# at-cg/PHI

Measured on AMD Instinct MI355X. Metric: read Gbases/s scored (49-hap MHC graph stand-in synMHC-49); reads resident in HBM, parsing and H2D excluded, higher is better.
Workload: dtype u64

## Files before the change

### include/phi_amd.h

```cpp
#ifndef PHI_AMD_H
#define PHI_AMD_H

#include <stddef.h>
#include <stdint.h>

#ifdef __cplusplus
extern "C" {
#endif

typedef struct phi_ctx phi_ctx;

typedef enum {
    PHI_OK = 0,
    PHI_ERR_INVALID = -1,
    PHI_ERR_NOMEM = -2,
    PHI_ERR_DEVICE = -3,
    PHI_ERR_STATE = -4,
    PHI_ERR_UNSUPPORTED = -5,
    PHI_ERR_WALK = -6,
    PHI_ERR_OVERFLOW = -7
} phi_status;

const char *phi_strerror(int status);
const char *phi_last_error(const phi_ctx *ctx);
// ... 44 lines not shown
int phi_panel_stats(phi_ctx *ctx, phi_panel_info *out);
int phi_panel_release(phi_ctx *ctx);
#define PHI_PANEL_KEEP_READS 2u

typedef struct {
    int32_t n_blocks, n_walks;
    int64_t n_classes_flagged;
    int64_t n_nonzero;
    double record_gpu_ms, class_gpu_ms, entry_gpu_ms;
    double walk_sum_gpu_ms;
} phi_scout_info;
int phi_scout_graph(phi_ctx *ctx, int32_t n_vtx, const char *seq_concat, const int64_t *seq_off,
                    const int64_t *adj_off, const int32_t *adj, int32_t n_walks,
                    const int64_t *walk_off, const int32_t *walk_vtx, const int32_t *topo_rank);
int phi_scout_scores(phi_ctx *ctx, int32_t n_blocks, int32_t *scores, phi_scout_info *info);
int phi_scout_choose(phi_ctx *ctx, const uint8_t *always, int32_t n_want, uint8_t *keep, int32_t *round_of);

typedef struct {
    int64_t text_bytes;
    int64_t n_records;
    int32_t n_samples;
    int64_t n_flagged;
    int64_t n_units, n_entries;
    double genotype_gpu_ms, walks_gpu_ms;
} phi_vcf_info;
int phi_vcf_genotypes(phi_ctx *ctx, const char *text, int64_t n_text, const int64_t *text_off, const int32_t *gt_index, int64_t n_records,
                      int32_t n_samples, uint16_t *gt, int32_t *ploidy, uint8_t *flagged);
int phi_vcf_walks(phi_ctx *ctx, const int32_t *unit_first, int64_t n_units, const int32_t *site_backbone, const int32_t *site_allele0,
                  int64_t n_sites, const int32_t *choice, int32_t n_haps, int64_t *walk_off_out);
int phi_vcf_walks_wide(phi_ctx *ctx, const int32_t *unit_first, int64_t n_units, const int32_t *site_backbone, const int32_t *site_allele0,
                       int64_t n_sites, const int32_t *choice, int32_t n_haps, int64_t *walk_off_out);
int phi_vcf_stats(phi_ctx *ctx, phi_vcf_info *out);

int phi_add_reads(phi_ctx *ctx, const char *bases, const int64_t *read_off, int64_t n_reads);
int phi_add_reads_device(phi_ctx *ctx, const void *d_bases, const void *d_read_off, int64_t n_reads,
                         int64_t n_bases);
int phi_reads_text_begin(phi_ctx *ctx, int64_t max_chunk_bytes);
int phi_add_reads_text(phi_ctx *ctx, const char *text, int64_t n_bytes, int32_t *irregular);
int phi_reads_text_end(phi_ctx *ctx, const char **pending, int64_t *n_pending, int64_t *n_taken);
typedef struct phi_text_park phi_text_park;
int phi_text_park_create(int32_t device, phi_text_park **out);
int phi_text_park_pin(phi_text_park *park, void *host, size_t bytes);
int phi_text_park_add(phi_text_park *park, const char *text, int64_t n, int32_t *index);
int phi_text_park_add_async(phi_text_park *park, const char *text, int64_t n, int32_t *index);
int phi_text_park_wait(phi_text_park *park, int32_t index);
int64_t phi_text_park_bytes(phi_text_park *park, int32_t index);
int phi_text_park_fetch(phi_text_park *park, int32_t index, char *out, int64_t cap);
int phi_text_park_release(phi_text_park *park, int32_t index);
void phi_text_park_destroy(phi_text_park *park);
int phi_add_reads_text_parked(phi_ctx *ctx, phi_text_park *park, int32_t index, int32_t *irregular);
int phi_reads_text_last_batch(phi_ctx *ctx, char *bases, int64_t cap_bases, int64_t *off, int64_t cap_reads, int64_t *n_reads,
                              int64_t *n_bases);
int phi_reads_text_detach_carry(phi_ctx *ctx, const char **bytes, int64_t *n);
int phi_reset_reads(phi_ctx *ctx);
int phi_reads_stats(phi_ctx *ctx, int64_t *n_reads, int64_t *n_bases, int64_t *n_emitted, int64_t *n_distinct);

int phi_hits_buffer(phi_ctx *ctx, void **d_hits, int64_t *n);
int phi_read_table(phi_ctx *ctx, void **d_table, int64_t *n_buckets);
int phi_spectrum_export(phi_ctx *ctx, void **d_hashes, int64_t *n);
int phi_spectrum_import(phi_ctx *ctx, const void *d_hashes, int64_t n);
int phi_spectrum_set_size(phi_ctx *ctx, int64_t global_size);

#define PHI_COMM_ID_BYTES 128
int phi_comm_unique_id(void *id_out, size_t cap);
int phi_comm_init(phi_ctx *ctx, const void *id, int32_t rank, int32_t n_ranks);
int phi_comm_info(const phi_ctx *ctx, int32_t *rank, int32_t *n_ranks);
int phi_comm_allreduce_hits(phi_ctx *ctx);
int phi_comm_exchange(phi_ctx *ctx);
int phi_comm_destroy(phi_ctx *ctx);

int phi_peers_create(int32_t n_ranks, void **group);
int phi_peers_join(phi_ctx *ctx, void *group, int32_t rank);
int phi_peers_allreduce_hits(phi_ctx *ctx);
int phi_peers_exchange(phi_ctx *ctx);
int phi_peers_destroy(void *group);

int phi_ipc_unique_id(void *id_out, size_t cap);
int phi_ipc_init(phi_ctx *ctx, const void *id, int32_t rank, int32_t n_ranks);
int phi_ipc_info(const phi_ctx *ctx, int32_t *rank, int32_t *n_ranks);
int phi_ipc_allreduce_hits(phi_ctx *ctx);
int phi_ipc_flush(phi_ctx *ctx);
int phi_ipc_exchange(phi_ctx *ctx);
int phi_ipc_check(phi_ctx *ctx);
int phi_ipc_destroy(phi_ctx *ctx);

typedef struct {
    int64_t objective;
    int64_t upper_bound;
    int32_t optimal;
    int32_t n_dp_runs;
    int64_t n_covered;
    int64_t n_path;
    const int32_t *path_vtx;
    const int32_t *path_hap;
    int32_t recombination_count;
    int32_t n_switches;
    int64_t hap_len;
    int32_t n_walks;
    const int64_t *n_minimizers;
    const int64_t *n_anchors;
    int64_t spectrum_size;
    int64_t filtered;
    int64_t retained;
    int64_t n_in_model;
} phi_result;

int phi_set_solve_budget(phi_ctx *ctx, int64_t max_dp_runs);

int phi_solve(phi_ctx *ctx, phi_result *out);

int phi_path_sequence(phi_ctx *ctx, char *buf, int64_t cap);

int phi_sketch(phi_ctx *ctx, const char *bases, const int64_t *seq_off, int64_t n_seq, int32_t k,
               int32_t w, uint64_t *out_hash, int64_t *out_pos, int32_t *out_seq, int64_t cap,
               int64_t *n_out);
typedef struct {
    int64_t n_entries, walk_bases;
    int64_t n_classes, class_bases, n_class_records;
    int64_t n_walk_minimizers, n_distinct_minimizers;
    double sketch_gpu_ms;
} phi_index_info;
int phi_index_stats(phi_ctx *ctx, phi_index_info *out);

typedef struct {
    int64_t n_dp_anchors, n_events;
    int32_t n_steps, n_blocks, dp_mode, max_classes;
    double mean_classes;
} phi_solve_info;
int phi_solve_stats(phi_ctx *ctx, phi_solve_info *out);

int phi_walk_minimizers(phi_ctx *ctx, int32_t walk, uint64_t *out_hash, int64_t *out_pos,
                        int64_t cap, int64_t *n_out);
int phi_walk_sharing(phi_ctx *ctx, int64_t *hist, int32_t cap, int64_t *n_distinct);

int phi_kept_anchors(phi_ctx *ctx, uint64_t *out_hash, int32_t *out_walk, int32_t *out_t0,
                     int32_t *out_t1, int64_t cap, int64_t *n_out);

int phi_host_register(phi_ctx *ctx, void *p, size_t bytes);
int phi_host_unregister(phi_ctx *ctx, void *p);

int phi_prof_enable(phi_ctx *ctx, int on);
int phi_prof_read(phi_ctx *ctx, int64_t *n_launches, double *total_ms, int64_t *total_bases);

typedef struct { const char *text; int64_t n; } phi_walk_text;
int phi_walk_text_upload(phi_ctx *ctx, const phi_walk_text *walks, int32_t n_walks);
int phi_walk_text_resolve(phi_ctx *ctx, const char *prefix, int32_t prefix_n, const int32_t *num2id, int64_t n_num, int32_t n_seg,
                          int64_t *walk_off_out, uint32_t *irregular);
int phi_walk_entries(phi_ctx *ctx, int32_t *out, int64_t cap, int64_t *n);

int phi_device_synchronize(phi_ctx *ctx);

int phi_prefix_sums(phi_ctx *ctx, int32_t kind, const void *d_in, int64_t n, void *d_out);

int phi_edit_distances(phi_ctx *ctx, const char *a, const int64_t *a_off, const char *b, const int64_t *b_off,
                       int64_t n_pairs, int64_t max_distance, int64_t *out);

int phi_edit_alignments(phi_ctx *ctx, const char *a, const int64_t *a_off, const char *b, const int64_t *b_off,
                        int64_t n_pairs, const int64_t *dist, int64_t *counts, char *cigar, const int64_t *cigar_off);


#define PHI_INFLATE_CHUNK_DEFAULT (64 << 10)
#define PHI_INFLATE_NO_FINDER 1
typedef struct {
    int64_t in_bytes;
    int64_t out_bytes;
    int64_t members;
    int64_t chunks;
    int64_t confirmed;
    int64_t redecoded;
    int64_t marker_bytes;
    double device_ms;
    char detail[192];
} phi_inflate_info;
int phi_inflate(int32_t device, const void *in, int64_t n, void *out, int64_t cap, int64_t chunk_bytes, int32_t flags,
                int64_t *out_size, phi_inflate_info *info);
int phi_inflate_alloc(int32_t device, const void *in, int64_t n, int64_t chunk_bytes, int32_t flags, void **out, int64_t *out_size,
                      phi_inflate_info *info);
void phi_inflate_free(void *p);
int phi_text_park_gzip_begin(phi_text_park *park, int64_t piece_bytes);
int phi_text_park_gzip_add(phi_text_park *park, const void *data, int64_t n);
int phi_text_park_gzip_end(phi_text_park *park, int32_t *first, int32_t *count, phi_inflate_info *info);
int phi_gzip_header(const void *data, int64_t n, int64_t pos, int64_t *deflate_start);
uint32_t phi_crc32_combine(uint32_t crc_a, uint32_t crc_b, int64_t len_b);

typedef struct {
    int64_t text_bytes;
    int64_t host_bytes;
    int64_t walk_bytes;
    int32_t n_walks;
    phi_inflate_info inflate;
} phi_gfa_gzip_info;
int phi_gfa_gzip_split(phi_ctx *ctx, const void *gz, int64_t n, int64_t chunk_bytes, char **host_text, int64_t *host_n,
                       phi_gfa_gzip_info *info);
void phi_gfa_gzip_free(char *host_text);

#define PHI_LADDER_MAX_LEVELS 16
typedef struct {
    int32_t n_levels;
    int32_t one_length;
    int64_t n_reads, n_bases;
    int64_t n_kept_reads, n_kept_bases;
    int64_t band_reads[PHI_LADDER_MAX_LEVELS], band_bases[PHI_LADDER_MAX_LEVELS];
    uint64_t threshold[PHI_LADDER_MAX_LEVELS];
    double count_gpu_ms, scan_gpu_ms, scatter_gpu_ms, copy_gpu_ms;
} phi_ladder_info;
int phi_reads_collect_begin(phi_ctx *ctx, int64_t first_ordinal);
int phi_reads_collect_end(phi_ctx *ctx, int64_t *n_reads, int64_t *n_bases);
int phi_reads_collect_release(phi_ctx *ctx);
int phi_reads_collect_score(phi_ctx *ctx);
int phi_ladder_plan(phi_ctx *ctx, uint64_t seed, const double *fractions, int32_t n_levels, phi_ladder_info *info);
int phi_ladder_advance(phi_ctx *ctx, int32_t level);
int phi_ladder_band(phi_ctx *ctx, int32_t band, int64_t *ordinals_out, int64_t cap, int64_t *n,
                    char *bases_out, int64_t bases_cap, int64_t *offsets_out, int64_t *n_bases);

typedef struct {
    int64_t n_records;
    int64_t n_kept;
    int64_t n_secondary_supplementary;
    int64_t n_empty;
    int64_t n_reverse;
    int64_t n_bases;
    int64_t header_bytes;
    int64_t tiles, tiles_confirmed, tiles_rewalked;
    int64_t batches, batches_without_offsets;
    int32_t n_ref;
    int32_t one_length;
} phi_bam_info;
int phi_reads_bam_begin(phi_ctx *ctx, int64_t max_chunk_bytes, int64_t tile_bytes);
int phi_add_reads_bam(phi_ctx *ctx, const void *bytes, int64_t n);
int phi_add_reads_bam_parked(phi_ctx *ctx, phi_text_park *park, int32_t index);
int phi_reads_bam_end(phi_ctx *ctx, phi_bam_info *info);
int phi_reads_bam_last_batch(phi_ctx *ctx, char *bases, int64_t cap_bases, int64_t *off, int64_t cap_reads, int64_t *n_reads, int64_t *n_bases);

typedef struct {
    int64_t n_calls;
    const int64_t *pos;
    const int64_t *ref_off, *alt_off;
    const char *ref_bytes, *alt_bytes;
    const int32_t *anchor;
    int64_t n_shared, n_query, n_ref;
    int64_t ref_span[2], query_span[2];
    double gpu_ms;
} phi_calls;
typedef struct {
    int64_t n_query, n_ref, n_shared, n_pairs, n_calls;
    int64_t ref_bytes, alt_bytes;
    int64_t ref_bases, query_bases;
    int64_t bytes_moved;
    double table_gpu_ms, shared_gpu_ms, pairs_gpu_ms, fill_gpu_ms, gpu_ms;
} phi_calls_info;
int phi_calls_path(phi_ctx *ctx, int32_t ref_walk, phi_calls *out);
int phi_calls_walk(phi_ctx *ctx, int32_t walk, int32_t ref_walk, phi_calls *out);
int phi_calls_stats(phi_ctx *ctx, phi_calls_info *out);

#ifdef __cplusplus
}
#endif
#endif
```

### phi_amd/_capi.py

```python
import ctypes as C
import os

_HERE = os.path.dirname(os.path.abspath(__file__))
LIB_PATH = os.environ.get("PHI_AMD_LIB") or os.path.join(_HERE, "libphi_amd.so")

PHI_OK = 0
PHI_ERR_INVALID, PHI_ERR_NOMEM, PHI_ERR_DEVICE, PHI_ERR_STATE = -1, -2, -3, -4
PHI_ERR_UNSUPPORTED, PHI_ERR_WALK, PHI_ERR_OVERFLOW = -5, -6, -7
PHI_FLAG_QCLP, PHI_FLAG_MIXED = 1, 2
PHI_COMM_ID_BYTES = 128

SYMBOLS = [
    "phi_strerror", "phi_last_error", "phi_ctx_create", "phi_ctx_destroy", "phi_set_stream", "phi_set_params",
    "phi_set_graph", "phi_add_reads", "phi_add_reads_device", "phi_reset_reads", "phi_reads_stats", "phi_hits_buffer", "phi_read_table",
    "phi_spectrum_export", "phi_spectrum_import", "phi_spectrum_set_size", "phi_solve", "phi_path_sequence",
    "phi_sketch", "phi_walk_minimizers", "phi_walk_sharing", "phi_kept_anchors", "phi_prof_enable", "phi_prof_read",
    "phi_host_register", "phi_host_unregister", "phi_set_solve_budget", "phi_device_synchronize", "phi_walk_text_upload", "phi_walk_text_resolve", "phi_walk_entries",
    "phi_index_stats", "phi_solve_stats", "phi_comm_unique_id", "phi_comm_init", "phi_comm_info", "phi_comm_allreduce_hits", "phi_comm_exchange", "phi_comm_destroy",
    "phi_reads_text_begin", "phi_add_reads_text", "phi_reads_text_end", "phi_reads_text_detach_carry", "phi_reads_text_last_batch",
    "phi_text_park_create", "phi_text_park_pin", "phi_text_park_add", "phi_text_park_add_async", "phi_text_park_wait", "phi_text_park_bytes", "phi_text_park_fetch", "phi_text_park_release", "phi_text_park_destroy",
    "phi_add_reads_text_parked",
    "phi_peers_create", "phi_peers_join", "phi_peers_allreduce_hits", "phi_peers_exchange", "phi_peers_destroy",
    "phi_ipc_unique_id", "phi_ipc_init", "phi_ipc_info", "phi_ipc_allreduce_hits", "phi_ipc_flush", "phi_ipc_exchange", "phi_ipc_check", "phi_ipc_destroy",
    "phi_edit_distances", "phi_edit_alignments",
    "phi_inflate", "phi_inflate_alloc", "phi_inflate_free", "phi_gzip_header", "phi_crc32_combine",
    "phi_text_park_gzip_begin", "phi_text_park_gzip_add", "phi_text_park_gzip_end",
    "phi_gfa_gzip_split", "phi_gfa_gzip_free",
    "phi_set_graph_chopped", "phi_chop_origin", "phi_chop_stats",
    "phi_vcf_genotypes", "phi_vcf_walks", "phi_vcf_stats",
    "phi_reads_collect_begin", "phi_reads_collect_end", "phi_reads_collect_release", "phi_ladder_plan", "phi_ladder_advance", "phi_ladder_band",
    "phi_set_graph_panel", "phi_panel_origin", "phi_panel_walks", "phi_panel_stats", "phi_panel_release",
    "phi_scout_graph", "phi_scout_scores", "phi_scout_choose", "phi_reads_collect_score", "phi_vcf_walks_wide",
    "phi_prefix_sums",
    "phi_reads_bam_begin", "phi_add_reads_bam", "phi_add_reads_bam_parked", "phi_reads_bam_end", "phi_reads_bam_last_batch",
    "phi_calls_path", "phi_calls_walk", "phi_calls_stats",
]
PHI_PANEL_RETAIN = 1
PHI_PANEL_KEEP_READS = 2
PHI_SCOUT_MAX_WALKS = 65535
PHI_LADDER_MAX_LEVELS = 16
PHI_INFLATE_NO_FINDER = 1
PHI_INFLATE_CHUNK_DEFAULT = 64 << 10


class PhiIndexInfo(C.Structure):
    _fields_ = [(n, C.c_int64) for n in ("n_entries", "walk_bases", "n_classes", "class_bases", "n_class_records",
                                         "n_walk_minimizers", "n_distinct_minimizers")] + [("sketch_gpu_ms", C.c_double)]


class PhiSolveInfo(C.Structure):
    _fields_ = [("n_dp_anchors", C.c_int64), ("n_events", C.c_int64), ("n_steps", C.c_int32), ("n_blocks", C.c_int32),
                ("dp_mode", C.c_int32), ("max_classes", C.c_int32), ("mean_classes", C.c_double)]


class PhiChopInfo(C.Structure):
    _fields_ = [("n_vtx_in", C.c_int64), ("n_vtx_out", C.c_int64), ("n_entries_in", C.c_int64), ("n_entries_out", C.c_int64),
                ("max_len", C.c_int32), ("expand_gpu_ms", C.c_double)]


class PhiPanelInfo(C.Structure):
    _fields_ = [("n_walks_in", C.c_int32), ("n_walks_out", C.c_int32), ("n_vtx_in", C.c_int64), ("n_vtx_out", C.c_int64),
                ("n_edges_in", C.c_int64), ("n_edges_out", C.c_int64), ("n_entries_in", C.c_int64), ("n_entries_out", C.c_int64),
                ("mark_gpu_ms", C.c_double), ("scan_gpu_ms", C.c_double), ("remap_gpu_ms", C.c_double),
                ("reduce_host_s", C.c_double), ("kahn_host_s", C.c_double)]


class PhiScoutInfo(C.Structure):
    _fields_ = [("n_blocks", C.c_int32), ("n_walks", C.c_int32), ("n_classes_flagged", C.c_int64), ("n_nonzero", C.c_int64),
                ("record_gpu_ms", C.c_double), ("class_gpu_ms", C.c_double), ("entry_gpu_ms", C.c_double), ("walk_sum_gpu_ms", C.c_double)]


class PhiVcfInfo(C.Structure):
    _fields_ = [("text_bytes", C.c_int64), ("n_records", C.c_int64), ("n_samples", C.c_int32), ("n_flagged", C.c_int64),
                ("n_units", C.c_int64), ("n_entries", C.c_int64), ("genotype_gpu_ms", C.c_double), ("walks_gpu_ms", C.c_double)]


class PhiLadderInfo(C.Structure):
    _fields_ = [("n_levels", C.c_int32), ("one_length", C.c_int32), ("n_reads", C.c_int64), ("n_bases", C.c_int64),
                ("n_kept_reads", C.c_int64), ("n_kept_bases", C.c_int64),
                ("band_reads", C.c_int64 * PHI_LADDER_MAX_LEVELS), ("band_bases", C.c_int64 * PHI_LADDER_MAX_LEVELS),
                ("threshold", C.c_uint64 * PHI_LADDER_MAX_LEVELS),
                ("count_gpu_ms", C.c_double), ("scan_gpu_ms", C.c_double), ("scatter_gpu_ms", C.c_double), ("copy_gpu_ms", C.c_double)]


class PhiBamInfo(C.Structure):
    _fields_ = [(n, C.c_int64) for n in ("n_records", "n_kept", "n_secondary_supplementary", "n_empty", "n_reverse", "n_bases", "header_bytes",
                                         "tiles", "tiles_confirmed", "tiles_rewalked", "batches", "batches_without_offsets")] + [
        ("n_ref", C.c_int32), ("one_length", C.c_int32)]


class PhiCalls(C.Structure):
    _fields_ = [("n_calls", C.c_int64), ("pos", C.POINTER(C.c_int64)), ("ref_off", C.POINTER(C.c_int64)), ("alt_off", C.POINTER(C.c_int64)),
                ("ref_bytes", C.c_void_p), ("alt_bytes", C.c_void_p), ("anchor", C.POINTER(C.c_int32)),
                ("n_shared", C.c_int64), ("n_query", C.c_int64), ("n_ref", C.c_int64),
                ("ref_span", C.c_int64 * 2), ("query_span", C.c_int64 * 2), ("gpu_ms", C.c_double)]


class PhiCallsInfo(C.Structure):
    _fields_ = [(n, C.c_int64) for n in ("n_query", "n_ref", "n_shared", "n_pairs", "n_calls", "ref_bytes", "alt_bytes", "ref_bases", "query_bases", "bytes_moved")] + [
        (n, C.c_double) for n in ("table_gpu_ms", "shared_gpu_ms", "pairs_gpu_ms", "fill_gpu_ms", "gpu_ms")]


class PhiResult(C.Structure):
    _fields_ = [
        ("objective", C.c_int64), ("upper_bound", C.c_int64), ("optimal", C.c_int32), ("n_dp_runs", C.c_int32),
        ("n_covered", C.c_int64),
        ("n_path", C.c_int64), ("path_vtx", C.POINTER(C.c_int32)), ("path_hap", C.POINTER(C.c_int32)),
        ("recombination_count", C.c_int32), ("n_switches", C.c_int32), ("hap_len", C.c_int64),
        ("n_walks", C.c_int32), ("n_minimizers", C.POINTER(C.c_int64)), ("n_anchors", C.POINTER(C.c_int64)),
        ("spectrum_size", C.c_int64), ("filtered", C.c_int64), ("retained", C.c_int64), ("n_in_model", C.c_int64),
    ]


class PhiInflateInfo(C.Structure):
    _fields_ = [(n, C.c_int64) for n in ("in_bytes", "out_bytes", "members", "chunks", "confirmed", "redecoded", "marker_bytes")] + [
        ("device_ms", C.c_double), ("detail", C.c_char * 192)]


class PhiGfaGzipInfo(C.Structure):
    _fields_ = [("text_bytes", C.c_int64), ("host_bytes", C.c_int64), ("walk_bytes", C.c_int64), ("n_walks", C.c_int32),
                ("inflate", PhiInflateInfo)]


_lib = None


def load():
    global _lib
    if _lib is not None:
        return _lib
    if not os.path.exists(LIB_PATH):
        raise RuntimeError(f"{LIB_PATH} is missing: build it with `python -m phi_amd.build` "
                           "(hipcc --offload-arch=gfx950); there is no CPU fallback")
    L = C.CDLL(LIB_PATH)
    vp, i32, i64 = C.c_void_p, C.c_int32, C.c_int64
    L.phi_strerror.restype = C.c_char_p
    L.phi_strerror.argtypes = [C.c_int]
    L.phi_last_error.restype = C.c_char_p
    L.phi_last_error.argtypes = [vp]
    L.phi_ctx_create.argtypes = [C.c_int, C.POINTER(vp)]
    L.phi_ctx_destroy.restype = None
    L.phi_ctx_destroy.argtypes = [vp]
    L.phi_set_stream.argtypes = [vp, vp]
    L.phi_set_params.argtypes = [vp, i32, i32, C.c_float, i32, C.c_uint32]
    L.phi_set_graph.argtypes = [vp, i32, vp, vp, vp, vp, i32, vp, vp, vp]
    L.phi_set_graph_chopped.argtypes = [vp, i32, vp, vp, vp, vp, i32, vp, vp, vp, i32, vp]
    L.phi_chop_origin.argtypes = [vp, vp, i64, vp, vp]
    L.phi_chop_stats.argtypes = [vp, C.POINTER(PhiChopInfo)]
    L.phi_set_graph_panel.argtypes = [vp, i32, vp, vp, vp, vp, i32, vp, vp, vp, i32, C.c_uint32, vp]
    L.phi_panel_origin.argtypes = [vp, vp, i64, vp]
    L.phi_panel_walks.argtypes = [vp, vp, i32, C.POINTER(i32)]
    L.phi_panel_stats.argtypes = [vp, C.POINTER(PhiPanelInfo)]
    L.phi_panel_release.argtypes = [vp]
    L.phi_scout_graph.argtypes = [vp, i32, vp, vp, vp, vp, i32, vp, vp, vp]
    L.phi_scout_scores.argtypes = [vp, i32, vp, C.POINTER(PhiScoutInfo)]
    L.phi_scout_choose.argtypes = [vp, vp, i32, vp, vp]
    L.phi_reads_collect_score.argtypes = [vp]
    L.phi_vcf_walks_wide.argtypes = [vp, vp, i64, vp, vp, i64, vp, i32, vp]
    L.phi_vcf_genotypes.argtypes = [vp, vp, i64, vp, vp, i64, i32, vp, vp, vp]
    L.phi_vcf_walks.argtypes = [vp, vp, i64, vp, vp, i64, vp, i32, vp]
    L.phi_vcf_stats.argtypes = [vp, C.POINTER(PhiVcfInfo)]
    L.phi_reads_collect_begin.argtypes = [vp, i64]
    L.phi_reads_collect_end.argtypes = [vp, C.POINTER(i64), C.POINTER(i64)]
    L.phi_reads_collect_release.argtypes = [vp]
    L.phi_ladder_plan.argtypes = [vp, C.c_uint64, C.POINTER(C.c_double), i32, C.POINTER(PhiLadderInfo)]
    L.phi_ladder_advance.argtypes = [vp, i32]
    L.phi_ladder_band.argtypes = [vp, i32, vp, i64, C.POINTER(i64), vp, i64, vp, C.POINTER(i64)]
    L.phi_add_reads.argtypes = [vp, vp, vp, i64]
    L.phi_add_reads_device.argtypes = [vp, vp, vp, i64, i64]
    L.phi_reset_reads.argtypes = [vp]
    L.phi_reads_text_begin.argtypes = [vp, i64]
    L.phi_add_reads_text.argtypes = [vp, vp, i64, C.POINTER(i32)]
    L.phi_reads_text_end.argtypes = [vp, C.POINTER(vp), C.POINTER(i64), C.POINTER(i64)]
    L.phi_reads_text_detach_carry.argtypes = [vp, C.POINTER(vp), C.POINTER(i64)]
    L.phi_reads_text_last_batch.argtypes = [vp, vp, i64, vp, i64, C.POINTER(i64), C.POINTER(i64)]
    L.phi_text_park_create.argtypes = [i32, C.POINTER(vp)]
    L.phi_text_park_pin.argtypes = [vp, vp, C.c_size_t]
    L.phi_text_park_add.argtypes = [vp, vp, i64, C.POINTER(i32)]
    L.phi_text_park_add_async.argtypes = [vp, vp, i64, C.POINTER(i32)]
    L.phi_text_park_wait.argtypes = [vp, i32]
    L.phi_text_park_bytes.argtypes = [vp, i32]
    L.phi_text_park_bytes.restype = i64
    L.phi_text_park_fetch.argtypes = [vp, i32, vp, i64]
    L.phi_text_park_release.argtypes = [vp, i32]
    L.phi_text_park_destroy.argtypes = [vp]
    L.phi_text_park_destroy.restype = None
    L.phi_add_reads_text_parked.argtypes = [vp, vp, i32, C.POINTER(i32)]
    L.phi_reads_bam_begin.argtypes = [vp, i64, i64]
    L.phi_add_reads_bam.argtypes = [vp, vp, i64]
    L.phi_add_reads_bam_parked.argtypes = [vp, vp, i32]
    L.phi_reads_bam_end.argtypes = [vp, C.POINTER(PhiBamInfo)]
    L.phi_reads_bam_last_batch.argtypes = [vp, vp, i64, vp, i64, C.POINTER(i64), C.POINTER(i64)]
    L.phi_calls_path.argtypes = [vp, i32, C.POINTER(PhiCalls)]
    L.phi_calls_walk.argtypes = [vp, i32, i32, C.POINTER(PhiCalls)]
    L.phi_calls_stats.argtypes = [vp, C.POINTER(PhiCallsInfo)]
    L.phi_reads_stats.argtypes = [vp, C.POINTER(i64), C.POINTER(i64), C.POINTER(i64), C.POINTER(i64)]
    L.phi_hits_buffer.argtypes = [vp, C.POINTER(vp), C.POINTER(i64)]
    L.phi_read_table.argtypes = [vp, C.POINTER(vp), C.POINTER(i64)]
    L.phi_spectrum_export.argtypes = [vp, C.POINTER(vp), C.POINTER(i64)]
    L.phi_spectrum_import.argtypes = [vp, vp, i64]
    L.phi_spectrum_set_size.argtypes = [vp, i64]
    L.phi_solve.argtypes = [vp, C.POINTER(PhiResult)]
    L.phi_set_solve_budget.argtypes = [vp, i64]
    L.phi_index_stats.argtypes = [vp, C.POINTER(PhiIndexInfo)]
    L.phi_solve_stats.argtypes = [vp, C.POINTER(PhiSolveInfo)]
    L.phi_comm_unique_id.argtypes = [vp, C.c_size_t]
    L.phi_comm_init.argtypes = [vp, vp, i32, i32]
    L.phi_comm_info.argtypes = [vp, C.POINTER(i32), C.POINTER(i32)]
    L.phi_comm_allreduce_hits.argtypes = [vp]
    L.phi_comm_exchange.argtypes = [vp]
    L.phi_comm_destroy.argtypes = [vp]
    L.phi_peers_create.argtypes = [i32, C.POINTER(vp)]
    L.phi_peers_join.argtypes = [vp, vp, i32]
    L.phi_peers_allreduce_hits.argtypes = [vp]
    L.phi_peers_exchange.argtypes = [vp]
    L.phi_peers_destroy.argtypes = [vp]
    L.phi_ipc_unique_id.argtypes = [vp, C.c_size_t]
    L.phi_ipc_init.argtypes = [vp, C.c_char_p, i32, i32]
    L.phi_ipc_info.argtypes = [vp, C.POINTER(i32), C.POINTER(i32)]
    L.phi_ipc_allreduce_hits.argtypes = [vp]
    L.phi_ipc_exchange.argtypes = [vp]
    L.phi_ipc_flush.argtypes = [vp]
    L.phi_ipc_check.argtypes = [vp]
    L.phi_ipc_destroy.argtypes = [vp]
    L.phi_path_sequence.argtypes = [vp, vp, i64]
    L.phi_sketch.argtypes = [vp, vp, vp, i64, i32, i32, vp, vp, vp, i64, C.POINTER(i64)]
    L.phi_walk_minimizers.argtypes = [vp, i32, vp, vp, i64, C.POINTER(i64)]
    L.phi_walk_sharing.argtypes = [vp, vp, i32, C.POINTER(i64)]
    L.phi_kept_anchors.argtypes = [vp, vp, vp, vp, vp, i64, C.POINTER(i64)]
    L.phi_prof_enable.argtypes = [vp, C.c_int]
    L.phi_host_register.argtypes = [vp, vp, C.c_size_t]
    L.phi_host_unregister.argtypes = [vp, vp]
    L.phi_prof_read.argtypes = [vp, C.POINTER(i64), C.POINTER(C.c_double), C.POINTER(i64)]
    L.phi_device_synchronize.argtypes = [vp]
    L.phi_prefix_sums.argtypes = [vp, i32, vp, i64, vp]
    L.phi_walk_text_upload.argtypes = [vp, vp, i32]
    L.phi_walk_text_resolve.argtypes = [vp, C.c_char_p, i32, vp, i64, i32, vp, C.POINTER(C.c_uint32)]
    L.phi_walk_entries.argtypes = [vp, vp, i64, C.POINTER(i64)]
    L.phi_edit_distances.argtypes = [vp, vp, vp, vp, vp, i64, i64, vp]
    L.phi_edit_alignments.argtypes = [vp, vp, vp, vp, vp, i64, vp, vp, vp, vp]
    L.phi_inflate.argtypes = [i32, vp, i64, vp, i64, i64, i32, C.POINTER(i64), C.POINTER(PhiInflateInfo)]
    L.phi_inflate_alloc.argtypes = [i32, vp, i64, i64, i32, C.POINTER(vp), C.POINTER(i64), C.POINTER(PhiInflateInfo)]
    L.phi_inflate_free.argtypes = [vp]
    L.phi_inflate_free.restype = None
    L.phi_text_park_gzip_begin.argtypes = [vp, i64]
    L.phi_text_park_gzip_add.argtypes = [vp, vp, i64]
    L.phi_text_park_gzip_end.argtypes = [vp, C.POINTER(i32), C.POINTER(i32), C.POINTER(PhiInflateInfo)]
    L.phi_gzip_header.argtypes = [vp, i64, i64, C.POINTER(i64)]
    L.phi_crc32_combine.argtypes = [C.c_uint32, C.c_uint32, i64]
    L.phi_crc32_combine.restype = C.c_uint32
    L.phi_gfa_gzip_split.argtypes = [vp, vp, i64, i64, C.POINTER(vp), C.POINTER(i64), C.POINTER(PhiGfaGzipInfo)]
    L.phi_gfa_gzip_free.argtypes = [vp]
    L.phi_gfa_gzip_free.restype = None
    for name in SYMBOLS:
        f = getattr(L, name)
        if f.restype is C.c_int and name not in ("phi_strerror", "phi_last_error", "phi_ctx_destroy", "phi_crc32_combine", "phi_inflate_free", "phi_gfa_gzip_free"):
            f.restype = C.c_int
    _lib = L
    return L
```

### phi_amd/context.py

```python
import ctypes as C
from typing import NamedTuple

import numpy as np

from . import _capi


class PhiError(RuntimeError):
    def __init__(self, status, detail):
        self.status = status
        self.detail = detail
        super().__init__(f"{_capi.load().phi_strerror(status).decode()} ({status}): {detail}")


def _ptr(a):
    return a.ctypes.data if a is not None and a.size else None


class Alignments(NamedTuple):
    distance: np.ndarray
    counts: np.ndarray
    cigar: list
    identity: np.ndarray

# ... 487 lines not shown

    def solve(self):
        r = _capi.PhiResult()
        self._chk(self._L.phi_solve(self._h, C.byref(r)))
        nw, npth = r.n_walks, r.n_path
        out = {f: getattr(r, f) for f in ("objective", "upper_bound", "optimal", "n_dp_runs", "n_covered", "n_path",
                                           "recombination_count", "n_switches", "hap_len", "n_walks", "spectrum_size",
                                           "filtered", "retained", "n_in_model")}
        out["path_vtx"] = np.ctypeslib.as_array(r.path_vtx, shape=(npth,)).copy() if npth else np.zeros(0, np.int32)
        out["path_hap"] = np.ctypeslib.as_array(r.path_hap, shape=(npth,)).copy() if npth else np.zeros(0, np.int32)
        out["n_minimizers"] = np.ctypeslib.as_array(r.n_minimizers, shape=(nw,)).copy()
        out["n_anchors"] = np.ctypeslib.as_array(r.n_anchors, shape=(nw,)).copy()
        return out

    def path_sequence(self, hap_len):
        buf = C.create_string_buffer(max(int(hap_len), 1))
        self._chk(self._L.phi_path_sequence(self._h, buf, hap_len))
        return buf.raw[:hap_len]

    def calls(self, ref_walk, walk=None):
        r = _capi.PhiCalls()
        if walk is None:
            self._chk(self._L.phi_calls_path(self._h, int(ref_walk), C.byref(r)))
        else:
            self._chk(self._L.phi_calls_walk(self._h, int(walk), int(ref_walk), C.byref(r)))
        n = r.n_calls
        out = {f: getattr(r, f) for f in ("n_calls", "n_shared", "n_query", "n_ref", "gpu_ms")}
        out["pos"] = np.ctypeslib.as_array(r.pos, shape=(n,)).copy() if n else np.zeros(0, np.int64)
        out["anchor"] = np.ctypeslib.as_array(r.anchor, shape=(n,)).copy() if n else np.zeros(0, np.int32)
        out["ref_off"] = np.ctypeslib.as_array(r.ref_off, shape=(n + 1,)).copy()
        out["alt_off"] = np.ctypeslib.as_array(r.alt_off, shape=(n + 1,)).copy()
        out["ref_bytes"] = C.string_at(r.ref_bytes, int(out["ref_off"][n])) if out["ref_off"][n] else b""
        out["alt_bytes"] = C.string_at(r.alt_bytes, int(out["alt_off"][n])) if out["alt_off"][n] else b""
        out["ref_span"] = (r.ref_span[0], r.ref_span[1])
        out["query_span"] = (r.query_span[0], r.query_span[1])
        return out

    def calls_stats(self):
        r = _capi.PhiCallsInfo()
        self._chk(self._L.phi_calls_stats(self._h, C.byref(r)))
        return {n: getattr(r, n) for n, _ in _capi.PhiCallsInfo._fields_}

    def edit_distances(self, a_list, b_list, max_distance=-1):
        if len(a_list) != len(b_list):
            raise ValueError("a_list and b_list differ in length")
        n = len(a_list)
        a_off, b_off = np.zeros(n + 1, np.int64), np.zeros(n + 1, np.int64)
        np.cumsum([len(s) for s in a_list], out=a_off[1:])
        np.cumsum([len(s) for s in b_list], out=b_off[1:])
        a, b = b"".join(a_list), b"".join(b_list)
        out = np.zeros(n, np.int64)
        self._chk(self._L.phi_edit_distances(self._h, a, _ptr(a_off), b, _ptr(b_off), n, int(max_distance), _ptr(out)))
        return out

    def edit_alignments(self, a_list, b_list, dist=None, cigar=True):
        if len(a_list) != len(b_list):
            raise ValueError("a_list and b_list differ in length")
        n = len(a_list)
        if dist is None:
            dist = self.edit_distances(a_list, b_list)
        dist = np.ascontiguousarray(dist, np.int64)
        if dist.shape != (n,):
            raise ValueError("dist must hold one distance per pair")
        a_off, b_off = np.zeros(n + 1, np.int64), np.zeros(n + 1, np.int64)
        np.cumsum([len(s) for s in a_list], out=a_off[1:])
        np.cumsum([len(s) for s in b_list], out=b_off[1:])
        a, b = b"".join(a_list), b"".join(b_list)
        counts = np.zeros((n, 5), np.int64)
        buf, c_off = None, None
        if cigar:
            c_off = np.zeros(n + 1, np.int64)
            np.cumsum(np.where(dist >= 0, 11 * (2 * dist + 1), 0), out=c_off[1:])
            buf = C.create_string_buffer(max(int(c_off[-1]), 1))
        self._chk(self._L.phi_edit_alignments(self._h, a, _ptr(a_off), b, _ptr(b_off), n, _ptr(dist), _ptr(counts),
                                               buf, _ptr(c_off)))
        cig = None
        if cigar:
            raw = buf.raw
            cig = [raw[c_off[i]:c_off[i] + counts[i, 4]].decode() if dist[i] >= 0 else None for i in range(n)]
        total = counts[:, :4].sum(axis=1)
        with np.errstate(invalid="ignore", divide="ignore"):
            ident = np.where(dist < 0, np.nan, np.where(total > 0, counts[:, 0] * 100.0 / np.maximum(total, 1), 0.0))
        return Alignments(dist, counts[:, :4].copy(), cig, ident)

    def sketch(self, seqs, k, w):
        off = np.zeros(len(seqs) + 1, np.int64)
        np.cumsum([len(s) for s in seqs], out=off[1:])
        concat = np.frombuffer(b"".join(seqs), np.uint8)
        n = C.c_int64()
        self._chk(self._L.phi_sketch(self._h, _ptr(concat), _ptr(off), len(seqs), k, w, None, None, None, 0, C.byref(n)))
        h = np.zeros(n.value, np.uint64)
        p = np.zeros(n.value, np.int64)
        s = np.zeros(n.value, np.int32)
        if n.value:
            self._chk(self._L.phi_sketch(self._h, _ptr(concat), _ptr(off), len(seqs), k, w, _ptr(h), _ptr(p), _ptr(s),
                                         n.value, C.byref(n)))
        return h, p, s

    def walk_minimizers(self, walk):
        n = C.c_int64()
        self._chk(self._L.phi_walk_minimizers(self._h, walk, None, None, 0, C.byref(n)))
        h = np.zeros(n.value, np.uint64)
        p = np.zeros(n.value, np.int64)
        if n.value:
            self._chk(self._L.phi_walk_minimizers(self._h, walk, _ptr(h), _ptr(p), n.value, C.byref(n)))
        return h, p

    def walk_sharing(self, n_walks):
        hist = np.zeros(n_walks + 1, np.int64)
        n = C.c_int64()
        self._chk(self._L.phi_walk_sharing(self._h, _ptr(hist), n_walks + 1, C.byref(n)))
        return hist, n.value

    def kept_anchors(self):
        n = C.c_int64()
        self._chk(self._L.phi_kept_anchors(self._h, None, None, None, None, 0, C.byref(n)))
        h = np.zeros(n.value, np.uint64)
        wk = np.zeros(n.value, np.int32)
        t0 = np.zeros(n.value, np.int32)
        t1 = np.zeros(n.value, np.int32)
        if n.value:
            self._chk(self._L.phi_kept_anchors(self._h, _ptr(h), _ptr(wk), _ptr(t0), _ptr(t1), n.value, C.byref(n)))
        return h, wk, t0, t1

    def walk_entries(self):
        n = C.c_int64()
        self._chk(self._L.phi_walk_entries(self._h, None, 0, C.byref(n)))
        out = np.zeros(n.value, np.int32)
        if n.value:
            self._chk(self._L.phi_walk_entries(self._h, _ptr(out), n.value, C.byref(n)))
        return out

    def gfa_gzip_split(self, data, chunk_bytes=0):
        p, n, info = self._gfa_gzip_split_raw(data, chunk_bytes)
        try:
            return C.string_at(p, n) if n else b"", info
        finally:
            self._L.phi_gfa_gzip_free(p)

    def _gfa_gzip_split_raw(self, data, chunk_bytes=0):
        buf = np.frombuffer(data, np.uint8) if not isinstance(data, np.ndarray) else data
        p, n, info = C.c_void_p(), C.c_int64(), _capi.PhiGfaGzipInfo()
        self._chk(self._L.phi_gfa_gzip_split(self._h, _ptr(buf), len(buf), chunk_bytes, C.byref(p), C.byref(n), C.byref(info)))
        d = {k: getattr(info, k) for k in ("text_bytes", "host_bytes", "walk_bytes", "n_walks")}
        d["inflate"] = _info(info.inflate)
        return p, n.value, d

    def device_synchronize(self):
        self._chk(self._L.phi_device_synchronize(self._h))

    def prefix_sums(self, kind, d_in, n, d_out):
        self._chk(self._L.phi_prefix_sums(self._h, kind, C.c_void_p(d_in), n, C.c_void_p(d_out)))

    def prof_enable(self, on=True):
        self._chk(self._L.phi_prof_enable(self._h, int(on)))

    def prof_read(self):
        n, ms, b = C.c_int64(), C.c_double(), C.c_int64()
        self._chk(self._L.phi_prof_read(self._h, C.byref(n), C.byref(ms), C.byref(b)))
        return n.value, ms.value, b.value


def _parse_reads_tail(text):
    lines = [ln.rstrip(b"\r") for ln in text.split(b"\n")]
    while lines and not lines[-1]:
        lines.pop()
    if not lines:
        return []
    if lines[0][:1] == b"@":
        if len(lines) % 4:
            raise ValueError("the reads text ends inside a FASTQ record")
        return lines[1::4]
    if lines[0][:1] != b">":
        raise ValueError("the reads text is neither FASTA nor FASTQ")
    seqs = []
    for ln in lines:
        if ln[:1] == b">":
            seqs.append([])
        else:
            seqs[-1].append(ln)
    return [b"".join(s) for s in seqs]


def _info(info):
    return {n: getattr(info, n) for n, _ in _capi.PhiInflateInfo._fields_ if n != "detail"}


def inflate(data, device=0, chunk_bytes=0, finder=True, as_array=False):
    L = _capi.load()
    buf = np.frombuffer(data, np.uint8) if not isinstance(data, np.ndarray) else data
    flags = 0 if finder else _capi.PHI_INFLATE_NO_FINDER
    p, size, info = C.c_void_p(), C.c_int64(), _capi.PhiInflateInfo()
    rc = L.phi_inflate_alloc(device, _ptr(buf), len(buf), chunk_bytes, flags, C.byref(p), C.byref(size), C.byref(info))
    if rc:
        raise PhiError(rc, info.detail.decode())
    try:
        out = np.empty(size.value, np.uint8)
        if size.value:
            C.memmove(out.ctypes.data, p, size.value)
    finally:
        L.phi_inflate_free(p)
    return (out if as_array else out.tobytes()), _info(info)


def gzip_header(data, pos=0):
    L = _capi.load()
    buf = np.frombuffer(data, np.uint8) if not isinstance(data, np.ndarray) else data
    q = C.c_int64()
    rc = L.phi_gzip_header(_ptr(buf), len(buf), pos, C.byref(q))
    if rc:
        raise PhiError(rc, "no gzip member header")
    return q.value


def crc32_combine(crc_a, crc_b, len_b):
    return _capi.load().phi_crc32_combine(crc_a, crc_b, len_b)


class TextPark:

    def __init__(self, device=0):
        self._L = _capi.load()
        self._h = C.c_void_p()
        rc = self._L.phi_text_park_create(device, C.byref(self._h))
        if rc:
            raise PhiError(rc, "phi_text_park_create failed")

    def add(self, text):
        buf = np.frombuffer(text, np.uint8) if not isinstance(text, np.ndarray) else text
        idx = C.c_int32()
        rc = self._L.phi_text_park_add(self._h, _ptr(buf), len(buf), C.byref(idx))
        if rc:
            raise PhiError(rc, "phi_text_park_add failed")
        return idx.value

    def add_gzip(self, slices, piece_bytes):
        rc = self._L.phi_text_park_gzip_begin(self._h, piece_bytes)
        if rc:
            raise PhiError(rc, "phi_text_park_gzip_begin failed")
        for sl in slices:
            buf = np.frombuffer(sl, np.uint8) if not isinstance(sl, np.ndarray) else sl
            rc = self._L.phi_text_park_gzip_add(self._h, _ptr(buf), len(buf))
            if rc:
                raise PhiError(rc, "phi_text_park_gzip_add failed")
        first, count, info = C.c_int32(), C.c_int32(), _capi.PhiInflateInfo()
        rc = self._L.phi_text_park_gzip_end(self._h, C.byref(first), C.byref(count), C.byref(info))
        if rc:
            raise PhiError(rc, info.detail.decode())
        return list(range(first.value, first.value + count.value)), _info(info)

    def fetch(self, index):
        n = self._L.phi_text_park_bytes(self._h, index)
        if n < 0:
            raise PhiError(-1, "no such piece")
        out = np.zeros(n, np.uint8)
        rc = self._L.phi_text_park_fetch(self._h, index, _ptr(out), n)
        if rc:
            raise PhiError(rc, "phi_text_park_fetch failed")
        return out.tobytes()

    def release(self, index):
        rc = self._L.phi_text_park_release(self._h, index)
        if rc:
            raise PhiError(rc, "phi_text_park_release failed")

    def close(self):
        if self._h:
            self._L.phi_text_park_destroy(self._h)
            self._h = C.c_void_p()

    def __del__(self):
        try:
            self.close()
        except Exception:
            pass
```

### phi_amd/csrc/phi_abi.hip

```cpp
#include <stdarg.h>
#include <stdio.h>
#include <string.h>
#include <algorithm>
#include <future>
#include "phi_ctx.h"
#include "phi_dev.h"

int phi_fail(phi_ctx *c, int code, const char *fmt, ...)
{
    char buf[512];
    va_list ap;
    va_start(ap, fmt);
    vsnprintf(buf, sizeof buf, fmt, ap);
    va_end(ap);
    if (c) {
        std::lock_guard<std::mutex> g(c->err_mu);
        c->last_error = buf;
    }
    return code;
}

int phi_hip_check(phi_ctx *c, hipError_t e, const char *what)
{
    if (e == hipSuccess) return PHI_OK;
    const int code = (e == hipErrorOutOfMemory) ? PHI_ERR_NOMEM : PHI_ERR_DEVICE;
    return phi_fail(c, code, "%s: %s", what, hipGetErrorString(e));
}

extern "C" {

const char *phi_strerror(int status)
{
    switch (status) {
    case PHI_OK: return "ok";
    case PHI_ERR_INVALID: return "invalid argument";
    case PHI_ERR_NOMEM: return "out of memory";
    case PHI_ERR_DEVICE: return "HIP device error";
    case PHI_ERR_STATE: return "call order violated";
    case PHI_ERR_UNSUPPORTED: return "unsupported input";
    case PHI_ERR_WALK: return "walk does not follow the graph";
    case PHI_ERR_OVERFLOW: return "internal table overflow";
    default: return "unknown status";
    }
}

const char *phi_last_error(const phi_ctx *ctx) { return ctx ? ctx->last_error.c_str() : ""; }

int phi_ctx_create(int device_id, phi_ctx **out)
{
    if (!out) return PHI_ERR_INVALID;
    *out = nullptr;
    PhiStageTimer tm("ctx_create");
    int n_dev = 0;
    if (hipGetDeviceCount(&n_dev) != hipSuccess || n_dev <= 0) return PHI_ERR_DEVICE;
    tm.lap("runtime start (hipInit)");
    if (device_id < 0 || device_id >= n_dev) return PHI_ERR_INVALID;
    if (hipSetDevice(device_id) != hipSuccess) return PHI_ERR_DEVICE;
    phi_ctx *c = new (std::nothrow) phi_ctx();
    if (!c) return PHI_ERR_NOMEM;
    c->device = device_id;
    std::future<hipError_t> aux = std::async(std::launch::async, [c, device_id]() {
        hipError_t e = hipSetDevice(device_id);
        if (e == hipSuccess) e = hipStreamCreateWithFlags(&c->aux_stream, hipStreamNonBlocking);
        if (e != hipSuccess) return e;
        void *d = nullptr;
        std::vector<char> h((size_t)1 << 20, 0);
        if (hipMalloc(&d, h.size()) == hipSuccess) {
            (void)phi_dev_poison(d, h.size());
            (void)hipMemcpyAsync(d, h.data(), h.size(), hipMemcpyHostToDevice, c->aux_stream);
            (void)hipMemcpyAsync(h.data(), d, h.size(), hipMemcpyDeviceToHost, c->aux_stream);
            (void)hipMemcpyAsync(d, h.data(), 64, hipMemcpyHostToDevice, c->aux_stream);
            (void)hipMemcpyAsync(h.data(), d, 64, hipMemcpyDeviceToHost, c->aux_stream);
            (void)hipMemsetAsync(d, 0, 4096, c->aux_stream);
            (void)hipStreamSynchronize(c->aux_stream);
            (void)hipFree(d);
        }
        return hipSuccess;
    });
    auto bail = [&](int code) {
        if (aux.valid()) (void)aux.get();
        if (c->own_stream) (void)hipStreamDestroy(c->own_stream);
        if (c->aux_stream) (void)hipStreamDestroy(c->aux_stream);
        phi_dev_free(c->d_scalars); phi_dev_free(c->d_stripes); phi_dev_free(c->alt.stripes);
        delete c;
        return code;
    };
    if (hipStreamCreateWithFlags(&c->own_stream, hipStreamNonBlocking) != hipSuccess) return bail(PHI_ERR_DEVICE);
    c->stream = c->own_stream;
    tm.lap("stream");
    if (phi_dev_ensure(c, c->d_scalars, S_N * 8) || hipMemsetAsync(c->d_scalars.p, 0, S_N * 8, c->stream) != hipSuccess ||
        phi_dev_ensure(c, c->d_stripes, 2 * STRIPE_BYTES) || hipMemsetAsync(c->d_stripes.p, 0, 2 * STRIPE_BYTES, c->stream) != hipSuccess ||
        phi_dev_ensure(c, c->alt.stripes, 2 * STRIPE_BYTES) || hipMemsetAsync(c->alt.stripes.p, 0, 2 * STRIPE_BYTES, c->stream) != hipSuccess)
        return bail(PHI_ERR_DEVICE);
    if (tm.on && getenv("PHI_TIMING_UNITS")) {
        (void)hipStreamSynchronize(c->stream); tm.lap("  scalars");
        phi_warm_sketch(c->stream); (void)hipStreamSynchronize(c->stream); tm.lap("  code object: sketch");
        phi_warm_table(c->stream); (void)hipStreamSynchronize(c->stream); tm.lap("  code object: table");
        phi_warm_anchors(c->stream); (void)hipStreamSynchronize(c->stream); tm.lap("  code object: anchors");
        phi_warm_contexts(c->stream); (void)hipStreamSynchronize(c->stream); tm.lap("  code object: contexts");
        phi_warm_dp(c->stream); (void)hipStreamSynchronize(c->stream); tm.lap("  code object: dp");
        phi_warm_dp_events(c->stream); (void)hipStreamSynchronize(c->stream); tm.lap("  code object: dp_events");
        phi_warm_solve_dev(c->stream); (void)hipStreamSynchronize(c->stream); tm.lap("  code object: solve_dev");
        phi_warm_reads_text(c->stream); (void)hipStreamSynchronize(c->stream); tm.lap("  code object: reads_text");
        phi_warm_scan(c->stream); (void)hipStreamSynchronize(c->stream); tm.lap("  code object: scan");
    }
    phi_warm_sketch(c->stream); phi_warm_table(c->stream); phi_warm_anchors(c->stream); phi_warm_contexts(c->stream);
    phi_warm_dp(c->stream); phi_warm_dp_events(c->stream); phi_warm_solve_dev(c->stream); phi_warm_reads_text(c->stream);
    phi_warm_walk_text(c->stream); phi_warm_scan(c->stream);
    if (hipStreamSynchronize(c->stream) != hipSuccess) return bail(PHI_ERR_DEVICE);
    tm.lap("scalars + code objects");
    if (aux.get() != hipSuccess) { c->aux_stream = nullptr; return bail(PHI_ERR_DEVICE); }
    c->last_error.clear();
    tm.lap("wait for the second stream + first host copies");
    *out = c;
    return PHI_OK;
}

void phi_ctx_destroy(phi_ctx *c)
{
    if (c && c->pin_future.valid()) c->pin_future.wait();
    if (c && c->dp_alloc_future.valid()) (void)c->dp_alloc_future.get();
    if (c && c->h_pin) { (void)hipSetDevice(c->device); (void)hipHostFree(c->h_pin); c->h_pin = nullptr; }
    if (c) { (void)hipSetDevice(c->device); stage_release(c); }
    if (!c) return;
    (void)phi_comm_destroy(c);
    (void)phi_ipc_destroy(c);
    (void)hipSetDevice(c->device);
    (void)hipStreamSynchronize(c->stream);
    phi_ladder_drop(c);
    DevBuf *all[] = {&c->d_anchors, &c->d_cov_all, &c->d_cov_w, &c->d_slots, &c->d_slots2, &c->d_segs, &c->d_ctr, &c->d_vmax, &c->d_lane_walk, &c->d_walk_lane, &c->d_coff, &c->d_blk_ncls, &c->d_rownew, &c->d_blk_bad, &c->d_seg_lo, &c->d_seg_row, &c->d_seg_S, &c->wtext.d_text, &c->panel.d_full, &c->scout.d_scores, &c->d_sel_off, &c->d_sel_tri, &c->d_blk_lo, &c->d_blk_ev, &c->d_blk_S, &c->d_row_out, &c->d_rowend, &c->d_blk_keys, &c->d_blk_carry, &c->d_cov, &c->d_cov2, &c->d_stepdiff, &c->alt.hit, &c->hit_extra[0], &c->hit_extra[1], &c->alt.stripes, &c->spset.d_sp_cnt, &c->rlog.d_novlog, &c->rlog.d_novcnt, &c->rlog.d_ovlist, &c->d_vlen, &c->d_ent_cls, &c->d_cls_rep, &c->d_cls_left, &c->d_cls_mult, &c->d_cls_base, &c->d_cls_rec_off, &c->d_rec_cls, &c->d_rec_rel, &c->d_u_replist, &c->d_adj_off, &c->d_adj, &c->d_topo_rank, &c->d_cnt_edge, &c->d_walk_err, &c->d_sa_cnt, &c->d_sa_cur, &c->d_sa_off, &c->d_sa_idx, &c->d_seq, &c->d_seq_off, &c->d_walk_vtx, &c->d_walk_off, &c->d_topo, &c->d_in_off,
                     &c->d_in_src, &c->d_e_out, &c->d_st_rec, &c->d_st_mask, &c->d_in_packed, &c->d_word, &c->d_wwords, &c->d_wbad,
                     &c->d_wascii, &c->d_wstarts, &c->d_rec_hash, &c->d_rec_pos, &c->d_rec_slot,
                     &c->d_rec_e0, &c->d_rec_e1, &c->d_u_keys, &c->d_u_rep, &c->d_u_uid, &c->d_rt, &c->d_kt, &c->d_in_s, &c->d_last_walk, &c->d_rowdiag, &c->d_wpre, &c->d_hit, &c->spset.d_sp_keys, &c->d_rbases,
                     &c->d_roff, &c->rlog.d_roff_made, &c->d_peer_send, &c->spset.d_export, &c->d_scalars, &c->d_stripes, &c->d_blk_cnt,
                     &c->d_blk_off, &c->d_flags, &c->d_flags2, &c->d_list, &c->d_list2, &c->d_list3, &c->d_walk_last, &c->d_m_rec, &c->d_m_group,
                     &c->d_g_keys, &c->d_g_rep, &c->d_g_cnt, &c->d_slot_maxcnt, &c->d_slot_multi, &c->d_a_e1,
                     &c->d_g_off, &c->d_g_span, &c->d_a_weight, &c->d_dmax, &c->d_bstart, &c->d_k_rec, &c->d_k_in, &c->d_cvtx, &c->d_ev_e, &c->d_ev_off, &c->d_ev,
                     &c->d_off_end, &c->d_off_start, &c->d_scan_blk, &c->d_scan_blk64, &c->d_scan_blkoff, &c->d_top,
                     &c->d_ent};
    phi_pool_flush(c->device);
    phi_pool_bypass(true);
    struct Bypass { ~Bypass() { phi_pool_bypass(false); } } bypass_guard;
    for (DevBuf *b : all) phi_dev_free(*b);
    for (auto &pr : c->prof_events) { (void)hipEventDestroy(pr.first); (void)hipEventDestroy(pr.second); }
    if (c->h_err) (void)hipHostFree(c->h_err);
    {
        auto &T = c->text;
        for (int i = 0; i < 2; i++) { phi_dev_free(T.text[i]); phi_dev_free(T.bases[i]); phi_dev_free(T.roff[i]); }
        phi_dev_free(T.tile_cnt); phi_dev_free(T.ls); phi_dev_free(T.pre); phi_dev_free(T.blk); phi_dev_free(T.sum);
        if (T.h_sum) (void)hipHostFree(T.h_sum);
        if (T.ev_copy) (void)hipEventDestroy(T.ev_copy);
    }
    phi_bam_drop(c);
    (void)hipStreamDestroy(c->own_stream);
    (void)hipStreamDestroy(c->aux_stream);
    delete c;
}

int phi_set_stream(phi_ctx *c, void *hip_stream)
{
    if (!c) return PHI_ERR_INVALID;
    HIPCHK(hipStreamSynchronize(c->stream));
    c->stream = hip_stream ? (hipStream_t)hip_stream : c->own_stream;
    return PHI_OK;
}

int phi_set_params(phi_ctx *c, int32_t k, int32_t w, float threshold, int32_t recombination, uint32_t flags)
{
    if (!c) return PHI_ERR_INVALID;
    if (c->have_graph) return phi_fail(c, PHI_ERR_STATE, "phi_set_params must precede phi_set_graph");
    if (k < 1 || k > PHI_MAX_K) return phi_fail(c, PHI_ERR_INVALID, "k=%d outside [1,%d]", k, PHI_MAX_K);
    if (w < 1 || w > PHI_MAX_W) return phi_fail(c, PHI_ERR_INVALID, "w=%d outside [1,%d]", w, PHI_MAX_W);
    if (recombination < 0) return phi_fail(c, PHI_ERR_INVALID, "recombination penalty must be >= 0");
    c->k = k; c->w = w; c->threshold = threshold; c->recombination = recombination; c->flags = flags;
    return PHI_OK;
}

}

int sketch_records(phi_ctx *c, const uint64_t *words, const unsigned long long *starts, int64_t n_bases,
                   int32_t k, int32_t w, const uint8_t *ascii_if_bad, DevBuf &out_hash, DevBuf &out_pos,
                   int64_t *n_out)
{
    *n_out = 0;
    const int64_t nb = phi_sketch_num_blocks(n_bases);
    if (nb == 0) return PHI_OK;
    PHICHK(phi_dev_ensure(c, c->d_blk_cnt, (size_t)nb * 4));
    PHICHK(phi_dev_ensure(c, c->d_blk_off, (size_t)(nb + 1) * 8));
    PhiSketchArgs A{};
    A.words = words; A.starts = starts; A.n_bases = n_bases; A.k = k; A.w = w;
    A.ascii = ascii_if_bad; A.allslow = ascii_if_bad ? 1 : 0; A.badbits = nullptr;
    A.block_cnt = c->d_blk_cnt.as<int32_t>();
    A.err = (uint32_t *)scalar(c, S_ERR);
    if (A.allslow) phi_launch_sketch_bytes(c->stream, PHI_MODE_COUNT, A, nullptr);
    else phi_launch_sketch(c->stream, PHI_MODE_COUNT, A);
    PHICHK(phi_scan(c, c->d_blk_cnt.as<int32_t>(), nb, c->d_blk_off.as<int64_t>()));
    int64_t total = 0;
    HIPCHK(hipMemcpyAsync(&total, c->d_blk_off.as<int64_t>() + nb, 8, hipMemcpyDeviceToHost, c->stream));
    HIPCHK(hipStreamSynchronize(c->stream));
    PHICHK(phi_dev_ensure(c, out_hash, (size_t)std::max<int64_t>(total, 1) * 8));
    PHICHK(phi_dev_ensure(c, out_pos, (size_t)std::max<int64_t>(total, 1) * 8));
    A.block_off = c->d_blk_off.as<int64_t>();
    A.out_hash = out_hash.as<uint64_t>();
    A.out_pos = out_pos.as<int64_t>();
    if (A.allslow) phi_launch_sketch_bytes(c->stream, PHI_MODE_WRITE, A, nullptr);
    else phi_launch_sketch(c->stream, PHI_MODE_WRITE, A);
    HIPCHK(hipGetLastError());
    *n_out = total;
    return PHI_OK;
}

extern "C" {

int phi_set_solve_budget(phi_ctx *c, int64_t max_dp_runs)
{
    if (!c) return PHI_ERR_INVALID;
    c->solve_budget = max_dp_runs > 0x7FFFFFFF ? 0x7FFFFFFF : max_dp_runs;
    c->solved = false;
    return PHI_OK;
}

int phi_solve(phi_ctx *c, phi_result *out)
{
    if (!c || !out) return PHI_ERR_INVALID;
    if (!c->have_graph) return phi_fail(c, PHI_ERR_STATE, "phi_solve before phi_set_graph");
    PHICHK(phi_refuse_scout(c, "phi_solve"));
    HIPCHK(hipSetDevice(c->device));
    const int rc = phi_solve_impl(c);
    phi_pool_flush(c->device);
    if (rc) return rc;
    *out = c->result;
    return PHI_OK;
}

int phi_path_sequence(phi_ctx *c, char *buf, int64_t cap)
{
    if (!c || (!buf && cap > 0)) return PHI_ERR_INVALID;
    PHICHK(phi_refuse_scout(c, "phi_path_sequence"));
    if (!c->solved) return phi_fail(c, PHI_ERR_STATE, "phi_path_sequence before phi_solve");
    if (cap < c->result.hap_len) return phi_fail(c, PHI_ERR_INVALID, "buffer too small: need %lld bytes", (long long)c->result.hap_len);
    const int64_t np = (int64_t)c->h_path_vtx.size();
    std::vector<int64_t> at((size_t)np + 1, 0);
    for (int64_t i = 0; i < np; i++) { const int32_t v = c->h_path_vtx[(size_t)i]; at[(size_t)i + 1] = at[(size_t)i] + (c->h_seq_off[v + 1] - c->h_seq_off[v]); }
    phi_parallel_chunks(np, 1 << 15, [&](int64_t lo, int64_t hi, int) {
        for (int64_t i = lo; i < hi; i++) {
            const int32_t v = c->h_path_vtx[(size_t)i];
            memcpy(buf + at[(size_t)i], c->h_seq.data() + c->h_seq_off[v], (size_t)(at[(size_t)i + 1] - at[(size_t)i]));
        }
    });
    return PHI_OK;
}

int phi_sketch(phi_ctx *c, const char *bases, const int64_t *seq_off, int64_t n_seq, int32_t k, int32_t w,
               uint64_t *out_hash, int64_t *out_pos, int32_t *out_seq, int64_t cap, int64_t *n_out)
{
    if (!c || !n_out || n_seq < 0 || (n_seq > 0 && !seq_off)) return PHI_ERR_INVALID;
    if (k < 1 || k > PHI_MAX_K || w < 1 || w > PHI_MAX_W) return phi_fail(c, PHI_ERR_INVALID, "k or w out of range");
    *n_out = 0;
    if (n_seq == 0) return PHI_OK;
    for (int64_t r = 0; r < n_seq; r++)
        if (seq_off[r + 1] < seq_off[r]) return phi_fail(c, PHI_ERR_INVALID, "seq_off not monotone");
    const int64_t n_bases = seq_off[n_seq] - seq_off[0];
    if (n_bases == 0) return PHI_OK;
    if (!bases) return PHI_ERR_INVALID;
    HIPCHK(hipSetDevice(c->device));
    HIPCHK(hipStreamSynchronize(c->stream));
    DevBuf dB, dO, dW, dS, dH, dP;
    int rc = PHI_OK;
    std::vector<int64_t> off(seq_off, seq_off + n_seq + 1);
    for (auto &o : off) o -= seq_off[0];
    do {
        if ((rc = phi_dev_ensure(c, dB, (size_t)n_bases + 64))) break;
        if ((rc = phi_dev_ensure(c, dO, (size_t)(n_seq + 1) * 8))) break;
        const int64_t n_words = (n_bases + 31) / 32;
        if ((rc = phi_dev_ensure(c, dW, (size_t)(n_words + 2) * 8))) break;
        const size_t n_sw = (size_t)(n_bases / 64 + 2);
        if ((rc = phi_dev_ensure(c, dS, n_sw * 8))) break;
        if ((rc = phi_hip_check(c, hipMemcpyAsync(dB.p, bases + seq_off[0], (size_t)n_bases, hipMemcpyHostToDevice, c->stream), "H2D bases"))) break;
        if ((rc = phi_hip_check(c, hipMemcpyAsync(dO.p, off.data(), (size_t)(n_seq + 1) * 8, hipMemcpyHostToDevice, c->stream), "H2D offsets"))) break;
        if ((rc = phi_hip_check(c, hipMemsetAsync(dW.as<uint64_t>() + n_words, 0, 16, c->stream), "memset"))) break;
        if ((rc = phi_hip_check(c, hipMemsetAsync(dS.p, 0, n_sw * 8, c->stream), "memset"))) break;
        if ((rc = phi_hip_check(c, hipMemsetAsync(scalar(c, S_NBAD), 0, 8, c->stream), "memset"))) break;
        phi_launch_mark_starts(c->stream, dO.as<int64_t>(), n_seq, dS.as<unsigned long long>());
        phi_launch_pack_ascii(c->stream, dB.as<uint8_t>(), n_bases, dW.as<uint64_t>(), n_words, nullptr,
                              (unsigned long long *)scalar(c, S_NBAD));
        if ((rc = phi_hip_check(c, hipStreamSynchronize(c->stream), "sync"))) break;
        uint64_t n_bad = 0;
        if ((rc = phi_hip_check(c, phi_copy_sync(c, &n_bad, scalar(c, S_NBAD), 8, hipMemcpyDeviceToHost), "D2H"))) break;
        int64_t total = 0;
        if ((rc = sketch_records(c, dW.as<uint64_t>(), dS.as<unsigned long long>(), n_bases, k, w,
                                 (n_bad || k > PHI_MAX_K_PACKED) ? dB.as<uint8_t>() : nullptr, dH, dP, &total))) break;
        if ((rc = phi_sync_check(c))) break;
        *n_out = total;
        if (cap >= total && total > 0) {
            std::vector<int64_t> gpos((size_t)total);
            if (out_hash && (rc = phi_hip_check(c, phi_copy_sync(c, out_hash, dH.p, (size_t)total * 8, hipMemcpyDeviceToHost), "D2H hash"))) break;
            if ((rc = phi_hip_check(c, phi_copy_sync(c, gpos.data(), dP.p, (size_t)total * 8, hipMemcpyDeviceToHost), "D2H pos"))) break;
            int64_t s = 0;
// ... 198 lines not shown
```

### phi_amd/csrc/phi_ctx.h

```cpp
#pragma once
#include <stdint.h>
#include <stdarg.h>
#include <stdio.h>
#include <stdlib.h>
#include <algorithm>
#include <atomic>
#include <chrono>
#include <future>
#include <mutex>
#include <string>
#include <thread>
#include <vector>
#include <hip/hip_runtime.h>
#include "../../include/phi_amd.h"
#include "phi_kernels.h"
#include "phi_host_par.h"
#include "solve_host.h"
#include "reads_host.h"

struct DevBuf {
    void *p = nullptr;
    size_t cap = 0;
    uint32_t gen = 0;
    template <class T> T *as() const { return reinterpret_cast<T *>(p); }
};

template <class T> struct PhiRawBuf {
    T *p = nullptr;
    size_t n = 0;
    PhiRawBuf() = default;
    PhiRawBuf(const PhiRawBuf &) = delete;
    PhiRawBuf &operator=(const PhiRawBuf &) = delete;
    ~PhiRawBuf() { free(p); }
    bool resize(size_t m)
    {
        free(p);
        p = m ? static_cast<T *>(malloc(m * sizeof(T))) : nullptr;
        n = p ? m : 0;
        return m == 0 || p != nullptr;
    }
    size_t size() const { return n; }
    T *data() const { return p; }
    T &operator[](size_t i) const { return p[i]; }
};

struct PhiComm;
struct PhiIpc;
#define PHI_HIT_RING 4
struct PhiPeers;

struct phi_ctx {
    int device = 0;
    PhiComm *comm = nullptr;
    PhiPeers *peers = nullptr;
    int peer_rank = 0;
    PhiIpc *ipc = nullptr;
    hipStream_t own_stream = nullptr, stream = nullptr;
    hipStream_t aux_stream = nullptr;
    std::string last_error;
    std::mutex err_mu;

    int32_t k = 31, w = 25, recombination = 100;
    float threshold = 1.0f;
    uint32_t flags = PHI_FLAG_QCLP | PHI_FLAG_MIXED;
    int64_t solve_budget = 4096;

    bool have_graph = false;
    int32_t n_vtx = 0, n_walks = 0;
    std::vector<char> h_seq;
    std::vector<int64_t> h_seq_off, h_adj_off, h_walk_off, h_walk_base;
    std::vector<int32_t> h_adj, h_topo_rank, h_topo;
    PhiRawBuf<int32_t> h_walk_vtx;
    int64_t n_entries = 0, walk_bases = 0;

#define WT_TILE 4096
    struct PhiWalkText {
        bool ready = false;
        int32_t n_walks = 0;
        std::vector<int64_t> tile0, t_len;
        std::vector<int32_t> ends;
        DevBuf d_text;
    } wtext;
    bool walks_on_device = false;
    int64_t walks_on_device_n = 0;
    struct PhiChop {
        bool on = false;
        std::vector<int32_t> first;
        phi_chop_info info{};
    } chop;
    struct PhiPanel {
        bool on = false;
        std::vector<int32_t> origin;
        std::vector<int32_t> kept;
        phi_panel_info info{};
        DevBuf d_full;
        std::vector<int64_t> full_off;
    } panel;
    struct PhiScout {
        bool on = false;
        DevBuf d_scores;
        int32_t n_blocks = 0;
    } scout;
    struct PhiVcf {
        bool have = false;
        phi_vcf_info info{};
    } vcf;

    DevBuf d_seq, d_seq_off, d_walk_vtx, d_walk_off, d_topo, d_in_off, d_in_src;
    DevBuf d_e_out, d_st_rec, d_st_mask, d_in_packed;
    int dp_nw = 1;
    DevBuf d_wwords, d_wstarts, d_wbad, d_wascii;
    DevBuf d_vlen;
    DevBuf d_ent_cls;
    DevBuf d_cls_rep, d_cls_left, d_cls_mult, d_cls_base, d_cls_rec_off;
    int64_t n_cls = 0, cls_bases = 0;
    double index_gpu_ms = 0.0;
    DevBuf d_rec_hash, d_rec_pos, d_rec_cls, d_rec_rel, d_rec_slot, d_rec_e0, d_rec_e1;
    int64_t n_rec = 0;
    DevBuf d_u_keys, d_u_rep, d_u_uid, d_u_replist;
    DevBuf d_rt;
    uint64_t rt_buckets = 0, rt_mask = 0;
    DevBuf d_kt;
    uint64_t kt_buckets = 0, kt_mask = 0;
    int64_t kt_max_chunks = 0;
    void *h_stage[2] = {nullptr, nullptr};
    hipEvent_t stage_ev[2] = {nullptr, nullptr};
    DevBuf d_wpre;
    DevBuf d_rowdiag;
    DevBuf d_in_s, d_last_walk;
    int64_t n_unique = 0;
    uint64_t u_cap = 0;
    DevBuf d_hit;
    DevBuf hit_extra[PHI_HIT_RING - 2];
    int hit_n = 2, hit_idx = 0;

    struct PhiSpectrumSet {
        DevBuf d_sp_keys;
        uint64_t sp_cap = 0;
        DevBuf d_sp_cnt;
        DevBuf d_export;
        int64_t sp_set_gen = -1;
        int64_t sp_gen = 0;
        void new_generation() { sp_gen++; }
        void new_graph() { sp_set_gen = -1; }
    } spset;
    struct PhiReadLog {
        DevBuf d_novlog, d_novcnt;
        int32_t nov_shift = 6;
        int64_t log_chunks = 0, log_done = 0;
        int64_t logged_done = 0;
        int64_t last_log_chunks = 0;
        DevBuf d_ovlist;
        int64_t ov_cap = 0, ov_done = 0, ov_bound = 0;
        bool async_batches = false;
        bool next_flag_zeroed = false;
        DevBuf d_roff_made;
        void flushed() { log_chunks = log_done = 0; ov_done = 0; ov_bound = 0; }
        void new_generation() { flushed(); logged_done = 0; last_log_chunks = 0; next_flag_zeroed = false; }
    } rlog;
    int64_t reads_bases = 0, reads_count = 0;
    int64_t spectrum_override = -1;
    DevBuf d_rbases, d_roff, d_peer_send;
    DevBuf d_scalars;
    DevBuf d_stripes;
    struct PhiReadBufs {
        DevBuf hit, stripes;
        bool needs_clean = false;
    } alt;

    uint32_t *h_err = nullptr;
    struct PhiTextStream {
        bool active = false, irregular = false, started = false, detached = false;
        bool carry_stale = false;
        int mode = 0;
        int64_t fed = 0, taken = 0;
        uint32_t carry_cap = 0, chunk_cap = 0, line_cap = 0;
        DevBuf text[2], bases[2], roff[2], tile_cnt, ls, pre, blk, sum;
        int slot = 0;
        uint32_t carry_len = 0, carry_at = 0;
        std::vector<char> h_carry;
        PhiTextSummary *h_sum = nullptr;
        hipEvent_t ev_copy = nullptr;
        int last_slot = -1;
        int64_t last_reads = 0, last_bases = 0;
        bool last_uniform = false;
        int dbg_slot = 0;
        int64_t dbg_reads = 0, dbg_bases = 0;
        uint32_t why = 0, first_bad = 0;
    } text;

    struct PhiBamStream {
        bool active = false, failed = false, header_done = false;
        int32_t n_ref = 0;
        uint32_t tile = 0, list_cap = 0, max_tiles = 0, max_rec = 0;
        uint32_t carry_cap = 0, chunk_cap = 0;
        std::vector<unsigned char> h_hdr;
        int64_t fed = 0;
        DevBuf text[2];
        DevBuf bases, roff, sum;
        DevBuf t_first, t_exit, t_status, t_cnt, t_skip, t_list, t_has, t_has_pre, t_use, t_base;
        DevBuf rec_pos, rec_keep, kidx, klen, kseq, krev;
        int slot = 0;
        uint32_t carry_len = 0, carry_at = 0;
        void *h_sum = nullptr;
        hipEvent_t ev_copy = nullptr;
        int64_t one_len = -1;
        int64_t dbg_reads = 0, dbg_bases = 0;
        phi_bam_info info{};
    } bam;

    struct PhiLadder {
        bool collecting = false, have_store = false, have_plan = false;
        int64_t first_ordinal = 0;
        int64_t n_reads = 0, n_bases = 0;
        int64_t one_len = -1;
        DevBuf d_bases, d_off;
        DevBuf d_pbases, d_poff, d_pidx, d_psrc, d_wg, d_tab;
        int64_t band_read0[PHI_LADDER_MAX_LEVELS + 1] = {0}, band_pos[PHI_LADDER_MAX_LEVELS + 1] = {0};
        int32_t scored = 0;
        phi_ladder_info info{};
    } ladder;

    DevBuf d_blk_cnt, d_blk_off, d_flags, d_flags2, d_list, d_list2, d_list3, d_walk_last;
    DevBuf d_sel_off, d_sel_tri;
    DevBuf d_adj_off, d_adj, d_topo_rank, d_cnt_edge, d_walk_err;
    DevBuf d_sa_cnt, d_sa_cur, d_sa_off, d_sa_idx;

    DevBuf d_m_rec, d_m_group, d_g_keys, d_g_rep, d_g_cnt, d_slot_maxcnt, d_slot_multi;
    DevBuf d_a_e1, d_g_off, d_g_span, d_a_weight;
    DevBuf d_dmax, d_bstart, d_top, d_ent, d_word;
    bool dp_dense_ready = false;
    bool dp_events = false;
    int32_t n_k = 0;
    int64_t n_ev = 0;
    std::vector<int32_t> h_cstep, h_kstep;
    std::vector<int32_t> h_k_cut_ok;
    bool dp_blocks = false;
    int32_t n_blk = 0, blk_ring = 1024, blk_max_len = 0;
    std::vector<int32_t> h_blk_lo;
    DevBuf d_blk_lo, d_blk_ev, d_blk_S, d_row_out, d_rowend, d_blk_keys, d_blk_carry, d_cov, d_cov2, d_stepdiff;
    bool dp_cls = false;
    int32_t blk_cls_target = 16;
    bool blk_no_small = false;
    int32_t blk_ls = 64;
    DevBuf d_lane_walk, d_walk_lane, d_coff, d_blk_ncls, d_rownew, d_blk_bad;
    DevBuf d_seg_lo, d_seg_row, d_seg_S;
    DevBuf d_k_rec, d_k_in, d_cvtx, d_ev_e, d_ev_off, d_ev, d_off_end, d_off_start, d_scan_blk, d_scan_blk64, d_scan_blkoff;
    DevBuf d_anchors, d_cov_all, d_cov_w, d_slots, d_slots2, d_segs, d_ctr, d_vmax;
    int64_t n_kept = 0, n_dp = 0;
    bool anchors_host = false;
    PhiAnchorSpan h_kept, h_dp;
    std::vector<PhiAnchorHost> h_dp_own;
    void *h_pin = nullptr;
    size_t h_pin_cap = 0;
    std::future<void> pin_future;
    std::future<int> dp_alloc_future;
    std::vector<uint64_t> h_kept_hash;
    std::vector<int32_t> h_path_vtx, h_path_hap;
    std::vector<int64_t> h_n_minimizers, h_n_anchors;
    phi_result result{};
    bool solved = false;
    struct PhiPathSeg { int32_t h; int64_t es, ee; };
    std::vector<PhiPathSeg> path_segs;
    struct PhiCalls {
        bool have = false;
        std::vector<int64_t> pos, ref_off, alt_off;
        std::vector<int32_t> anchor;
        std::vector<char> ref_bytes, alt_bytes;
        int64_t span[4] = {0, 0, 0, 0};
        phi_calls_info info{};
    } calls;

    bool prof = false;
    std::vector<std::pair<hipEvent_t, hipEvent_t>> prof_events;
    int prof_period = 1;
    uint64_t prof_seq = 0;
    size_t prof_used = 0;
    int64_t prof_bases = 0;
    double prof_ms_done = 0.0;
    int64_t prof_n_done = 0;
};

struct PhiStageTimer {
    bool on;
    const char *what;
    std::chrono::steady_clock::time_point t0;
    explicit PhiStageTimer(const char *w) : on(getenv("PHI_TIMING") != nullptr), what(w), t0(std::chrono::steady_clock::now()) {}
    void lap(const char *stage)
    {
        if (!on) return;
        const auto t1 = std::chrono::steady_clock::now();
        fprintf(stderr, "[phi timing] %s: %-28s %8.3f ms\n", what, stage, std::chrono::duration<double, std::milli>(t1 - t0).count());
        t0 = t1;
    }
};

static inline hipError_t phi_copy_sync(phi_ctx *c, void *dst, const void *src, size_t n, hipMemcpyKind kind)
{
    const hipError_t e = hipMemcpyAsync(dst, src, n, kind, c->stream);
    return e != hipSuccess ? e : hipStreamSynchronize(c->stream);
}
static inline hipError_t phi_memset_sync(phi_ctx *c, void *dst, int v, size_t n)
{
    const hipError_t e = hipMemsetAsync(dst, v, n, c->stream);
    return e != hipSuccess ? e : hipStreamSynchronize(c->stream);
}

static inline int32_t phi_entry_walk(const phi_ctx *c, int64_t e)
{
    return phi_walk_of_entry(c->h_walk_off.data(), (int32_t)c->h_walk_off.size() - 1, e);
}

int phi_solve_impl(phi_ctx *c);
int phi_add_reads_device_impl(phi_ctx *c, const void *d_bases, const void *d_read_off, int64_t n_reads, int64_t n_bases, bool replay);
int replay_if_full(phi_ctx *c, uint32_t err, const void *d_bases, const void *d_off, int64_t n_reads, int64_t n_bases);
int phi_fail(phi_ctx *c, int code, const char *fmt, ...);
#define HIPCHK(call) do { int rc_ = phi_hip_check(c, (call), #call); if (rc_) return rc_; } while (0)
#define PHICHK(call) do { int rc_ = (call); if (rc_) return rc_; } while (0)
int phi_dev_ensure(phi_ctx *c, DevBuf &b, size_t bytes);
int phi_dev_grow_keep(phi_ctx *c, DevBuf &b, size_t bytes, size_t keep);
void phi_dev_free(DevBuf &b);
static inline void phi_scout_end(phi_ctx *c)
{
    c->scout.on = false; c->scout.n_blocks = 0;
    phi_dev_free(c->scout.d_scores);
}
struct PhiDevGuard {
    std::vector<DevBuf *> b;
    ~PhiDevGuard() { for (DevBuf *x : b) phi_dev_free(*x); }
};
enum { S_ERR = 0, S_NBAD = 1, S_BATCHBAD = 2, S_NEMIT = 3, S_FILTERED = 4, S_INMODEL = 5, S_EXPORT = 6, S_BATCHBAD2 = 7,
       S_OVCNT = 8 , S_N = 11 };
static inline uint64_t *scalar(phi_ctx *c, int i) { return c->d_scalars.as<uint64_t>() + i; }
#define STRIPE_BYTES ((size_t)PHI_STRIPES * 8 * 8)
int phi_upload_bytes(phi_ctx *c, DevBuf &b, const void *src, size_t bytes, hipStream_t st);
template <class T> static inline int upload(phi_ctx *c, DevBuf &b, const T *src, size_t n, hipStream_t st = nullptr)
{
    return phi_upload_bytes(c, b, src, n * sizeof(T), st);
}
void stage_release(phi_ctx *c);
int sketch_records(phi_ctx *c, const uint64_t *words, const unsigned long long *starts, int64_t n_bases, int32_t k, int32_t w,
                   const uint8_t *ascii_if_bad, DevBuf &out_hash, DevBuf &out_pos, int64_t *n_out);
int set_graph_check_args(phi_ctx *c, int32_t n_vtx, const char *seq_concat, const int64_t *seq_off, const int64_t *adj_off,
                         const int32_t *adj, int32_t n_walks, const int64_t *walk_off, const int32_t *walk_vtx, const int32_t *topo_rank);
int set_graph_check_offsets(phi_ctx *c, int32_t n_vtx, const int64_t *seq_off, const int64_t *adj_off, int32_t n_walks, const int64_t *walk_off);
int set_graph_impl(phi_ctx *c, int32_t n_vtx, const char *seq_concat, const int64_t *seq_off, const int64_t *adj_off,
                   const int32_t *adj, int32_t n_walks, const int64_t *walk_off, const int32_t *walk_vtx, const int32_t *topo_rank);
int chop_expand_entries(phi_ctx *c, const int32_t *d_in, int64_t n_in, const int32_t *first, int32_t n_vtx, const int64_t *walk_off,
                        int32_t n_walks, int32_t max_len, DevBuf &d_out, std::vector<int64_t> &walk_off2, std::vector<int32_t> &ends,
                        int64_t *n_out_p, double *gpu_ms);
extern const int phi_device_poison;
int phi_dev_poison_fill(void *p, size_t bytes);
static inline int phi_dev_poison(void *p, size_t bytes) { return phi_device_poison < 0 ? 0 : phi_dev_poison_fill(p, bytes); }
void phi_bam_drop(phi_ctx *c);
int phi_text_park_piece_dev(phi_text_park *p, int32_t index, int device, const void **d, int64_t *n, char *first = nullptr);
int phi_ladder_collect(phi_ctx *c, const void *d_bases, const void *d_read_off, int64_t n_reads, int64_t n_bases);
void phi_ladder_drop(phi_ctx *c);
void phi_ladder_detach(phi_ctx *c, phi_ctx::PhiLadder &out);
void phi_ladder_attach(phi_ctx *c, phi_ctx::PhiLadder &in);
int phi_score_resident_batch(phi_ctx *c, const void *d_bases, const void *d_read_off, int64_t n_reads, int64_t n_bases);
void phi_pool_bypass(bool on);
void phi_pool_flush(int device);
int phi_hip_check(phi_ctx *c, hipError_t e, const char *what);
int phi_sync_check(phi_ctx *c);
static inline int phi_refuse_scout(phi_ctx *c, const char *what)
{
    return c->scout.on ? phi_fail(c, PHI_ERR_STATE, "%s on a scout graph (phi_scout_graph builds the index without the DP: phi_set_graph_panel sets the chosen panel)", what) : PHI_OK;
}
int phi_pin_ensure(phi_ctx *c, size_t bytes);
int phi_host_anchors(phi_ctx *c);
int phi_ipc_wait_pending(phi_ctx *c);
int phi_ipc_before_generation(phi_ctx *c, int64_t gen);
void phi_ipc_launch_args(phi_ctx *c, PhiSketchArgs &A);
int phi_read_counts(phi_ctx *c, uint64_t *n_logged, uint64_t *n_emitted);
int phi_spectrum_count(phi_ctx *c, uint64_t *n_distinct);
int phi_scan(phi_ctx *c, const uint8_t *cnt, int64_t n, int32_t *off);
int phi_scan(phi_ctx *c, const int32_t *cnt, int64_t n, int32_t *off);
int phi_scan(phi_ctx *c, const int32_t *cnt, int64_t n, int64_t *off);
int phi_compact(phi_ctx *c, const uint8_t *flags, int64_t n, DevBuf &out, int64_t *n_out);
```

### phi_amd/csrc/phi_kernels.h

```cpp
#pragma once
#include <stdint.h>
#include <hip/hip_runtime.h>
#include "phi_dp_flags.h"

#ifndef PHI_TPB
#define PHI_TPB 256

#endif
#define PHI_WCH 512
#define PHI_MAX_W 256
#define PHI_MAX_K 64
#define PHI_MAX_K_PACKED 32
#define PHI_MAX_PROBE 4096
#define PHI_RT_OVERFLOWED 1u
static inline int phi_nov_shift(int w)
{
    const int want = (3 * 2 * PHI_WCH) / (2 * (w + 1));
    int sh = 4;
    while ((1 << sh) < want && sh < 9) sh++;
    return sh;
}
#define PHI_STRIPES 256

typedef uint32_t phi_ent_t;
#define PHI_MAX_ENTRIES (((int64_t)1 << 32) - 64)

enum { PHI_MODE_COUNT = 0, PHI_MODE_WRITE = 1, PHI_MODE_PROBE = 2 };

#define PHI_MB_ERR 8
#define PHI_MB_SCORED 16
#define PHI_MB_GATHERED 17
#define PHI_MB_BLOCKS 18

#define PHI_KERR_SENTINEL 1u
#define PHI_KERR_TABLE_FULL 2u
#define PHI_KERR_WALK_EDGE 4u
#define PHI_KERR_CSR_ID 32u
#define PHI_KERR_DP_QUEUE 16u
#define PHI_KERR_DP_CLASSES 64u
#define PHI_KERR_HASH_COLLISION 128u

struct PhiSketchArgs {
    const uint64_t *words;
    const unsigned long long *starts;
    int64_t n_bases;
    int32_t k, w;
    const unsigned long long *badbits;
    const uint8_t *ascii;
    int32_t allslow;
    int32_t *block_cnt;
    const int64_t *block_off;
    uint64_t *out_hash;
    int64_t *out_pos;
    unsigned long long *n_logged;
    unsigned long long *n_emitted;
    const uint64_t *u_rt; uint64_t u_bmask;
    uint8_t *hit;
    uint32_t *err;
    uint64_t *nov_log; uint16_t *nov_cnt; int64_t log_base; int32_t nov_shift;
    uint64_t *ov_list; unsigned long long *ov_count; int64_t ov_cap;
    const int64_t *read_off; int64_t n_reads;
    uint32_t reads_per_base_q32;
    int32_t uniform_len;
    double inv_len;
    uint32_t inv_len_q32;
    int32_t wave_stride;
    int32_t q_clean;
    int32_t win_reads;
    unsigned long long *ov_zero;
    unsigned long long *ipc_mb; unsigned long long ipc_scored, ipc_need;
    uint64_t *q_hit_words; int64_t q_n_hit_words; uint64_t *q_stripes; int64_t q_n_stripe_words;
    const uint64_t *k_rt; uint64_t k_bmask;
};
#define PHI_NOV_KMERS 0x8000u

void phi_launch_pack_ascii(hipStream_t st, const uint8_t *bases, int64_t n, uint64_t *words, int64_t n_words,
                           uint32_t *badbits, unsigned long long *n_bad);
void phi_launch_mark_starts(hipStream_t st, const int64_t *seq_off, int64_t n_seq, unsigned long long *starts);

void phi_launch_sketch_bytes(hipStream_t st, int mode, const PhiSketchArgs &A, const unsigned long long *batch_bad);
void phi_launch_reset_reads(hipStream_t st, uint64_t *hit_words, int64_t n_hit_words, uint64_t *stripes, int64_t n_stripe_words);
int64_t phi_sketch_num_blocks(int64_t n_bases);
int phi_sketch_win_reads(int k, int w, int64_t uniform_len, int64_t n_reads, int64_t n_bases);
int64_t phi_sketch_read_chunks(int k, int w, int64_t uniform_len, int64_t n_reads, int64_t n_bases);
void phi_launch_sketch(hipStream_t st, int mode, const PhiSketchArgs &A, hipEvent_t t0 = nullptr, hipEvent_t t1 = nullptr);

void phi_launch_table_build(hipStream_t st, const uint64_t *rec_hash, int64_t n_rec, uint64_t *u_keys,
                            uint32_t *u_rep, uint64_t u_mask, uint32_t *rec_slot, uint32_t *err);
void phi_launch_rep_flags(hipStream_t st, const uint32_t *rec_slot, int64_t n_rec, const uint32_t *u_rep,
                          uint8_t *flags);
void phi_launch_table_compact(hipStream_t st, const int32_t *rep_list, int64_t n_unique, const uint64_t *rec_hash, int64_t n_rec,
                              uint64_t *keys, uint32_t *uid, uint64_t mask, uint32_t *rec_slot, uint32_t *err);
void phi_launch_share_hist(hipStream_t st, const uint64_t *keys, int64_t cap, const int32_t *n_walks_of, unsigned long long *hist);
void phi_launch_slot_uid(hipStream_t st, const int32_t *rep_list, int64_t n_unique, const uint32_t *rec_slot,
                         uint32_t *u_uid);
void phi_launch_read_table(hipStream_t st, const uint64_t *keys, const uint32_t *uid, int64_t cap, uint64_t *rt,
                           int64_t n_buckets, uint32_t *err);
void phi_launch_fill_u64(hipStream_t st, uint64_t *p, int64_t n, uint64_t v);
void phi_launch_fill_u32(hipStream_t st, uint32_t *p, int64_t n, uint32_t v);
void phi_launch_iota_i64(hipStream_t st, int64_t *p, int64_t n, int64_t step);
void phi_launch_spectrum_insert(hipStream_t st, const uint64_t *hashes, int64_t n, uint64_t *sp_keys,
                                uint64_t sp_mask, unsigned long long *sp_count, const uint64_t *u_keys, uint64_t u_mask,
                                const uint32_t *u_uid, uint8_t *hit, uint32_t *err);
void phi_launch_spectrum_flush(hipStream_t st, const uint64_t *nov_log, const uint16_t *nov_cnt, int64_t c_lo, int64_t c_hi, int32_t shift,
                               uint64_t *sp_keys, uint64_t sp_mask, unsigned long long *sp_count, int32_t k, const uint64_t *u_keys,
                               uint64_t u_mask, uint32_t *err);
void phi_launch_kmer_keys(hipStream_t st, const int32_t *rec_cls, const int32_t *rec_rel, const uint64_t *rec_hash, const uint32_t *rec_slot,
                          int64_t n_rec, const int64_t *cls_base, const uint8_t *cls_left, const uint64_t *words, const uint32_t *badbits,
                          int32_t k, uint64_t *kkeys, unsigned long long *ctr);
void phi_launch_rt_overflowed(hipStream_t st, const uint64_t *rt, int64_t n_buckets, unsigned long long *n_out);
void phi_launch_count_flags(hipStream_t st, const uint8_t *flags, int64_t n, unsigned long long *n_out);
void phi_launch_spectrum_export(hipStream_t st, const uint64_t *sp_keys, int64_t cap, uint64_t *out,
                                unsigned long long *n_out);

struct PhiClassArgs {
    const int32_t *walk_vtx; const int64_t *walk_off; int32_t n_walks; int64_t n_entries;
    const int32_t *vlen; const uint8_t *seq; const int64_t *seq_off;
    int32_t tail_need;
    uint64_t seed;
    uint64_t *t_keys; uint32_t *t_rep; uint32_t *t_mult; uint64_t t_mask;
    uint32_t *ent_slot;
    uint32_t *err;
};
struct PhiExpandArgs {
    const int32_t *ent_cls; int64_t e_lo, e_hi;
    const int32_t *cls_rec_off; const phi_ent_t *cls_rep;
    const uint8_t *sel; const int32_t *sel_cnt;
    int32_t *block_cnt; const int64_t *block_off;
    const uint64_t *rec_hash; const int32_t *rec_rel; const int64_t *ent_base; uint64_t *out_hash; int64_t *out_pos;
    const uint32_t *rec_slot; const uint32_t *u_uid; const phi_ent_t *rec_e0; const phi_ent_t *rec_e1; uint32_t *out_tri;
};
void phi_launch_vlen(hipStream_t st, const int64_t *seq_off, int64_t n_vtx, int32_t *vlen);
void phi_launch_walk_bases(hipStream_t st, const int32_t *walk_vtx, const int32_t *vlen, const int64_t *walk_off, int32_t n_walks,
                           int64_t n_entries, unsigned long long *out);
void phi_launch_walk_rec_counts(hipStream_t st, const int32_t *ent_cls, const int32_t *cls_rec_off, const int64_t *walk_off,
                                int32_t n_walks, int64_t n_entries, unsigned long long *out);
void phi_launch_class_insert(hipStream_t st, const PhiClassArgs &A);
void phi_launch_class_verify(hipStream_t st, const PhiClassArgs &A, uint8_t *is_rep);
void phi_launch_class_ids(hipStream_t st, const phi_ent_t *cls_rep, int64_t n_cls, const uint32_t *ent_slot, int64_t n_entries,
                          const uint32_t *t_mult, uint32_t *t_cid, int32_t *cls_mult, int32_t *ent_cls);
void phi_launch_class_len(hipStream_t st, const PhiClassArgs &A, const phi_ent_t *cls_rep, int64_t n_cls, int32_t *cls_len, uint8_t *cls_left);
void phi_launch_pack_classes(hipStream_t st, const uint8_t *seq, const int64_t *seq_off, const int32_t *walk_vtx, const int32_t *vlen,
                             const phi_ent_t *cls_rep, const uint8_t *cls_left, const int64_t *cls_base, int64_t n_cls, uint64_t *words,
                             int64_t n_words, uint32_t *badbits, uint8_t *ascii, unsigned long long *n_bad);
void phi_launch_class_rec(hipStream_t st, const int64_t *raw_pos, int64_t n_raw, const int64_t *cls_base, int64_t n_cls,
                          const phi_ent_t *cls_rep, const uint8_t *cls_left, const int32_t *walk_vtx, const int32_t *vlen, int32_t k,
                          uint8_t *keep, int32_t *r_cls, int32_t *r_rel, phi_ent_t *r_e0, phi_ent_t *r_e1);
void phi_launch_class_rec_gather(hipStream_t st, const int32_t *idx, int64_t n, const uint64_t *raw_hash, const int32_t *r_cls,
                                 const int32_t *r_rel, const phi_ent_t *r_e0, const phi_ent_t *r_e1, uint64_t *o_hash, int32_t *o_cls,
                                 int32_t *o_rel, phi_ent_t *o_e0, phi_ent_t *o_e1);
void phi_launch_class_rec_off(hipStream_t st, const int32_t *rec_cls, int64_t n_rec, int64_t n_cls, int32_t *off);
int64_t phi_expand_num_blocks(int64_t n_entries);
void phi_launch_expand_count(hipStream_t st, const PhiExpandArgs &A);
void phi_launch_expand_write(hipStream_t st, const PhiExpandArgs &A, int kind);
void phi_launch_class_sel_count(hipStream_t st, const uint8_t *sel, const int32_t *cls_rec_off, int64_t n_cls, int32_t *sel_cnt);
void phi_launch_class_sel_tri(hipStream_t st, const uint8_t *sel, const int32_t *cls_rec_off, int64_t n_cls, const int32_t *sel_off, const phi_ent_t *cls_rep,
                              const uint32_t *rec_slot, const uint32_t *u_uid, const phi_ent_t *rec_e0, const phi_ent_t *rec_e1, int32_t *sel_tri);
void phi_launch_expand_tri(hipStream_t st, const int32_t *ent_cls, int64_t e_lo, int64_t e_hi, const int32_t *sel_off, const int32_t *sel_tri,
                           const int64_t *block_off, uint32_t *out_tri, phi_ent_t *a_e1, uint8_t *a_span, const int64_t *walk_off, int32_t n_walks,
                           unsigned long long *walk_cnt, unsigned long long *prep, int64_t n_anchors);
void phi_launch_mark_list(hipStream_t st, const int32_t *list, const int32_t *through, int64_t n, uint8_t *sel);
void phi_launch_share_count_cls(hipStream_t st, const int32_t *ent_cls, int64_t e_lo, int64_t e_hi, const int32_t *cls_rec_off,
                                const uint32_t *rec_slot, int32_t walk, int32_t *last_walk, int32_t *n_walks_of);
void phi_launch_entry_len_range(hipStream_t st, const int32_t *walk_vtx, const int32_t *vlen, int64_t e_lo, int64_t n, int32_t *lens);

#define PHI_KERR_FP_COLLISION 8u
void phi_launch_walk_edges(hipStream_t st, const int32_t *walk_vtx, const int64_t *walk_off, int32_t n_walks, int64_t n_entries, int32_t n_vtx,
                           const int64_t *adj_off, const int32_t *adj, const int64_t *seq_off, const int32_t *topo_rank,
                           uint8_t *e_out, int32_t *cnt_edge, unsigned long long *st_mask, int32_t nw64, int32_t *err);
void phi_launch_csr_count(hipStream_t st, const uint32_t *triples, int64_t n, int64_t n_ids, int32_t *cnt, uint32_t *err);
void phi_launch_csr_scatter(hipStream_t st, const uint32_t *triples, int64_t n, int64_t n_ids, const int32_t *off, int32_t *cur,
                            int32_t *idx);
void phi_launch_csr_sort(hipStream_t st, const int32_t *off, int64_t n_ids, int32_t *idx);
void phi_launch_match_flags(hipStream_t st, const uint32_t *rec_slot, int64_t n_rec, const uint32_t *u_uid,
                            const uint8_t *hit, uint8_t *flags);

struct PhiFilterArgs {
    const uint32_t *rec_slot; const phi_ent_t *rec_e0; const phi_ent_t *rec_e1;
    const int32_t *walk_vtx;
    const int32_t *rec_cls; const int32_t *cls_mult;
    const int32_t *m_rec;
    uint64_t *g_keys; int32_t *g_rep; uint32_t *g_cnt; uint64_t g_mask; uint64_t seed;
    int32_t *m_group;
    const uint32_t *u_uid;
    uint32_t *slot_maxcnt;
    uint8_t *slot_multi;
    float limit;
    unsigned long long *counters;
    uint32_t *err;
};
void phi_launch_group_insert(hipStream_t st, const PhiFilterArgs &A, int64_t n_matched);
void phi_launch_group_count(hipStream_t st, const PhiFilterArgs &A, int64_t n_matched);
void phi_launch_group_max(hipStream_t st, const PhiFilterArgs &A, int64_t n_matched);
void phi_launch_slot_count(hipStream_t st, const PhiFilterArgs &A, int64_t u_cap);
void phi_launch_kept_flags(hipStream_t st, const PhiFilterArgs &A, int64_t n_matched, uint8_t *kept, uint8_t *dp);
void phi_launch_gather_i32(hipStream_t st, const int32_t *src, const uint32_t *idx, int64_t n, int32_t *out);
void phi_launch_gather_u64(hipStream_t st, const uint64_t *src, const int32_t *idx, int64_t n, uint64_t *out);
void phi_launch_entry_csr(hipStream_t st, const phi_ent_t *a_e1, int64_t n_a, int64_t n_entries, int64_t *g_off);

#define PHI_DP_CHUNK 128
#define PHI_DP_RING 2048
#define PHI_SCOUT_MAX_WALKS 65535
#define PHI_DP_MAX_WALKS 1022

struct PhiDpArgs {
    int32_t n_vtx, n_walks;
    const int32_t *st_rec;
    const unsigned long long *st_mask;
    const int32_t *in_packed;
    const int64_t *walk_off;
    const uint64_t *word;
    const int64_t *g_off; const uint8_t *g_span; const uint8_t *a_weight;
    int32_t cost;
    int32_t *dmax;
    int32_t *bstart;
    int32_t *tops;
    int32_t *ent_src, *ent_h;
};
void phi_launch_dp(hipStream_t st, const PhiDpArgs &A);

#define PHI_DP_EVENT_MAX_WALKS 256
#define PHI_DP_EVENT_SAFE_WALKS 128
struct PhiDpEventArgs {
    int32_t n_k, n_walks;
    int64_t n_ev;
    const int32_t *k_rec;
    const int32_t *k_in_packed;
    const int64_t *walk_off;
    const phi_ent_t *ev_e;
    const int64_t *ev_off;
    void *ev;
    const int64_t *g_off; const uint8_t *g_span; const uint8_t *a_weight;
    int32_t cost;
    int32_t *dmax, *bstart;
    int32_t *tops;
    int32_t *ent_src, *ent_h;
    uint32_t *err;
    int32_t q_limit;
    int32_t n_blk, blk_ring;
    int32_t blk_max_len;
    int32_t lane_stride;
    const int32_t *lane_walk;
    int32_t *rownew_out;
    int32_t *rowdiag_out;
    const int32_t *blk_lo;
    const int32_t *blk_ev;
    const int32_t *blk_S;
    int32_t *row_out; int32_t *rowend_out;
    int32_t *blk_keys_out; int32_t *blk_carry;
};
void phi_launch_dp_events(hipStream_t st, const PhiDpEventArgs &A);
void phi_launch_dp_block_rows(hipStream_t st, const PhiDpEventArgs &A);
void phi_launch_dp_block_paths(hipStream_t st, const PhiDpEventArgs &A);
void phi_launch_anchor_prep(hipStream_t st, const uint32_t *tri, int64_t n, const int64_t *walk_off, int32_t n_walks, phi_ent_t *a_e1, uint8_t *a_span,
                            unsigned long long *walk_cnt, unsigned long long *out);
void phi_launch_vertex_most(hipStream_t st, const int64_t *g_off, int64_t n_entries, const int32_t *walk_vtx, int32_t *vmax);
void phi_launch_sum_i32(hipStream_t st, const int32_t *v, int64_t n, unsigned long long *out);
void phi_launch_repeat_walk(hipStream_t st, const uint32_t *tri, int64_t lo, int64_t hi, int32_t walk, int32_t *last, uint8_t *flags);
void phi_launch_weights(hipStream_t st, const uint32_t *tri, int64_t n, const uint8_t *in_s, uint8_t *wgt);
void phi_launch_path_cover(hipStream_t st, bool clear, const phi_ent_t *segs, int32_t n_seg, const int64_t *g_off, const uint32_t *tri, const uint8_t *wgt,
                           int32_t *cov_all, int32_t *cov_w, unsigned long long *ctr, uint32_t *twice, int64_t twice_cap);
void phi_launch_uncovered_slots(hipStream_t st, const uint32_t *slots, int64_t n, const int32_t *cov_all, unsigned long long *ctr, uint32_t *out);
struct PhiBlkClassArgs {
    int32_t n_blk, n_walks, lane_stride;
// ... 87 lines not shown
```

### phi_amd/csrc/phi_solve.hip

```cpp
#include <stdio.h>
#include <string.h>
#include <algorithm>
#include <map>
#include <set>
#include <unordered_map>
#include "phi_ctx.h"
#include "phi_dev.h"

static bool have_host_walks(const phi_ctx *c) { return (int64_t)c->h_walk_vtx.size() == c->n_entries; }
static int walk_vtx_at(phi_ctx *c, int64_t e, int32_t *v)
{
    if (have_host_walks(c)) { *v = c->h_walk_vtx[(size_t)e]; return PHI_OK; }
    return phi_hip_check(c, phi_copy_sync(c, v, c->d_walk_vtx.as<int32_t>() + e, 4, hipMemcpyDeviceToHost), "walk entry D2H");
}
static int walk_vtx_range(phi_ctx *c, int64_t es, int64_t n, int32_t *dst)
{
    if (have_host_walks(c)) { memcpy(dst, c->h_walk_vtx.data() + es, (size_t)n * 4); return PHI_OK; }
    return phi_hip_check(c, phi_copy_sync(c, dst, c->d_walk_vtx.as<int32_t>() + es, (size_t)n * 4, hipMemcpyDeviceToHost), "walk entries D2H");
}
static int ensure_host_walks(phi_ctx *c)
{
    if (have_host_walks(c)) return PHI_OK;
    if (!c->h_walk_vtx.resize((size_t)c->n_entries)) return phi_fail(c, PHI_ERR_NOMEM, "host allocation failed");
    return phi_hip_check(c, phi_copy_sync(c, c->h_walk_vtx.data(), c->d_walk_vtx.p, (size_t)c->n_entries * 4, hipMemcpyDeviceToHost), "walk entries D2H");
// ... 319 lines not shown
    }
    *e_ = -1;
    if (lo < c->h_walk_off[h + 1]) {
        int32_t vl = 0;
        PHICHK(walk_vtx_at(c, lo, &vl));
        if (vl == u) *e_ = lo;
    }
    return PHI_OK;
}

static int dp_backtrack(phi_ctx *c, const DpOut &O, bool events, DpHost &H, int32_t h, std::vector<Seg> *segs)
{
    bool bulk = false;
    auto fetch_bulk = [&]() -> int {
        H.bstart.resize(c->n_entries); H.ent_u.resize(O.n_ent); H.ent_h.resize(O.n_ent);
        HIPCHK(hipMemcpyAsync(H.bstart.data(), O.bstart, (size_t)c->n_entries * 4, hipMemcpyDeviceToHost, c->stream));
        HIPCHK(hipMemcpyAsync(H.ent_u.data(), O.ent_src, (size_t)O.n_ent * 4, hipMemcpyDeviceToHost, c->stream));
        HIPCHK(hipMemcpyAsync(H.ent_h.data(), O.ent_h, (size_t)O.n_ent * 4, hipMemcpyDeviceToHost, c->stream));
        HIPCHK(hipStreamSynchronize(c->stream));
        bulk = true;
        return PHI_OK;
    };
    segs->clear();
    int64_t e = c->h_walk_off[h + 1] - 1;
    for (int64_t guard = 0; guard <= (int64_t)c->n_vtx; guard++) {
        if (!bulk && guard == 64) PHICHK(fetch_bulk());
        int32_t bs = 0;
        if (bulk) bs = H.bstart[e];
        else HIPCHK(phi_copy_sync(c, &bs, O.bstart + e, 4, hipMemcpyDeviceToHost));
        if (bs < 0 && c->dp_blocks && events) {
            int32_t vq = 0;
            PHICHK(walk_vtx_at(c, e, &vq));
            const int32_t kq = c->h_cstep[c->h_topo_rank[vq]];
            int32_t b = (int32_t)(std::upper_bound(c->h_blk_lo.begin(), c->h_blk_lo.end(), kq) - c->h_blk_lo.begin()) - 1;
            if (c->dp_cls) {
                int32_t out[2] = {-1, -1};
                phi_launch_carry_resolve(c->stream, c->d_blk_carry.as<int32_t>(), c->blk_ls, b, h, c->d_blk_bad.as<int32_t>() + 2);
                HIPCHK(hipMemcpyAsync(out, c->d_blk_bad.as<int32_t>() + 2, 8, hipMemcpyDeviceToHost, c->stream));
                HIPCHK(hipStreamSynchronize(c->stream));
                bs = out[1];
            } else {
                while (bs < 0 && --b >= 0) bs = H.carry[(size_t)b * 64 + h];
            }
            if (bs < 0) return phi_fail(c, PHI_ERR_DEVICE, "DP backtrack: a carried run has no beginning (internal error)");
        }
        const int64_t es = c->h_walk_off[h] + bs;
        if (es < c->h_walk_off[h] || es > e) return phi_fail(c, PHI_ERR_DEVICE, "DP backtrack left the walk (internal error)");
        segs->push_back(Seg{h, es, e});
        if (es == c->h_walk_off[h]) break;
        int32_t v = 0;
        PHICHK(walk_vtx_at(c, es, &v));
        const int32_t step = events ? c->h_cstep[c->h_topo_rank[v]] : c->h_topo_rank[v];
        if (step < 0) return phi_fail(c, PHI_ERR_DEVICE, "DP backtrack: run begins on a vertex without events (internal error)");
        int32_t src, h2;
        if (bulk) { src = H.ent_u[step]; h2 = H.ent_h[step]; }
        else {
            HIPCHK(phi_copy_sync(c, &src, O.ent_src + step, 4, hipMemcpyDeviceToHost));
            HIPCHK(phi_copy_sync(c, &h2, O.ent_h + step, 4, hipMemcpyDeviceToHost));
        }
        if (events && src >= 0) src = c->h_kstep[src];
        const int32_t u = src >= 0 ? c->h_topo[src] : -1;
        if (u < 0 || h2 < 0) return phi_fail(c, PHI_ERR_DEVICE, "DP backtrack hit a vertex without an entry (internal error)");
        int64_t e2 = -1;
        PHICHK(entry_on_vertex(c, h2, src, u, &e2));
        if (e2 < 0) return phi_fail(c, PHI_ERR_DEVICE, "DP backtrack: walk %d is not on vertex %d (internal error)", h2, u);
        h = h2; e = e2;
    }
    std::reverse(segs->begin(), segs->end());
    return PHI_OK;
}

static int run_dp(phi_ctx *c, const std::vector<uint8_t> *wgt, DpHost &H, int64_t *value, std::vector<Seg> *segs)
{
    for (DpRetry want = DP_DONE;;) {
        switch (want) {
        case DP_DONE: break;
        case DP_HALVE_CLASS_TARGET: c->blk_cls_target /= 2; PHICHK(dp_prepare_blocks(c, c->n_dp)); break;
        case DP_NO_SMALL_BLOCKS: c->blk_no_small = true; PHICHK(dp_prepare_blocks(c, c->n_dp)); break;
        case DP_GIVE_UP_BLOCKS: c->dp_blocks = false; c->dp_cls = false; break;
        case DP_DENSE: c->dp_events = false; break;
        }
        want = DP_DONE;
        const bool events = c->dp_events;
        const DpOut O = dp_out(c);
        PhiStageTimer tr("dp run");
        if (c->n_dp && wgt) HIPCHK(hipMemcpyAsync(c->d_a_weight.p, wgt->data(), (size_t)c->n_dp, hipMemcpyHostToDevice, c->stream));
        if (events) {
            PhiDpEventArgs A{};
            PHICHK(dp_event_records(c, O, A, tr));
            if (c->dp_blocks && c->dp_cls) PHICHK(dp_blocks_on_class_lanes(c, A, tr, &want));
            else if (c->dp_blocks) PHICHK(dp_blocks_on_walk_lanes(c, A, H, tr, &want));
            else phi_launch_dp_events(c->stream, A);
            if (want != DP_DONE) continue;
        } else {
            PHICHK(dp_dense(c, O));
        }
        HIPCHK(hipGetLastError());
        PHICHK(dp_fetch_ends(c, O, events, H, tr, &want));
        if (want != DP_DONE) continue;
        int32_t bh = -1;
        PHICHK(dp_pick_end(c, H, &bh, value));
        PHICHK(dp_backtrack(c, O, events, H, bh, segs));
        tr.lap("backtrack");
        return PHI_OK;
    }
}

template <class F> static void for_covered(const phi_ctx *c, const std::vector<Seg> &segs, F f)
{
    const PhiAnchorSpan &A = c->h_dp;
    for (const Seg &s : segs) {
        auto lo = std::lower_bound(A.begin(), A.end(), s.es, [](const PhiAnchorHost &a, int64_t e) { return (int64_t)a.e1 < e; });
        for (auto it = lo; it != A.end() && (int64_t)it->e1 <= s.ee; ++it)
            if ((int64_t)it->e0 >= s.es) f((int64_t)(it - A.begin()));
    }
}

struct Node {
    std::vector<std::pair<uint32_t, int32_t>> assign;
    int64_t ub = INT64_MAX;
};

struct Search {
    std::vector<Node> stack;
    std::vector<int64_t> open_ub;
    int64_t incumbent = INT64_MIN, global_ub = INT64_MIN, best_cov = 0;
    int n_runs = 0;
    bool exhausted = false;
};

struct Solve {
    phi_ctx *const c;
    PhiStageTimer tm{"solve"};
    int64_t n_matched = 0, n_kept_rec = 0, n_kept = 0, n_dp = 0;
    int64_t filtered = 0, in_model = 0, spectrum = 0;
    bool anchors_prepped = false;
    bool dev = false;
    PhiAnchorArrays arr;
    std::vector<int32_t> sa_off, sa_idx;
    std::vector<uint8_t> wgt;
    std::vector<int32_t> cov_all, cov_w;
    std::vector<uint32_t> touched;
    std::set<uint32_t> S0;
    DpHost H;
    Search bb;
    std::vector<Seg> best_segs;
    explicit Solve(phi_ctx *c_) : c(c_) {}
};

static int read_spectrum(Solve &S)
{
    phi_ctx *c = S.c;
    if (c->dp_alloc_future.valid()) PHICHK(c->dp_alloc_future.get());
    PHICHK(phi_sync_check(c));
    S.tm = PhiStageTimer("solve");
    uint64_t sc[S_N];
    HIPCHK(phi_copy_sync(c, sc, c->d_scalars.p, sizeof sc, hipMemcpyDeviceToHost));
    uint64_t n_distinct = 0;
    PHICHK(phi_spectrum_count(c, &n_distinct));
    S.tm.lap("read spectrum (set from the log)");
    S.spectrum = c->spectrum_override >= 0 ? c->spectrum_override : (int64_t)n_distinct;
    return PHI_OK;
}

static int match_and_compact(Solve &S)
{
    phi_ctx *c = S.c;
    const int64_t n_rec = c->n_rec;
    PHICHK(phi_dev_ensure(c, c->d_flags, (size_t)std::max<int64_t>(n_rec, 1)));
    phi_launch_match_flags(c->stream, c->d_rec_slot.as<uint32_t>(), n_rec, c->d_u_uid.as<uint32_t>(),
                           c->d_hit.as<uint8_t>(), c->d_flags.as<uint8_t>());
    PHICHK(phi_compact(c, c->d_flags.as<uint8_t>(), n_rec, c->d_m_rec, &S.n_matched));
    S.tm.lap("match + compact");
    return PHI_OK;
}

static int filter_shared_anchors(Solve &S)
{
    phi_ctx *c = S.c;
    const int64_t n_rec = c->n_rec, n_matched = S.n_matched;
    PhiFilterArgs F{};
    F.rec_slot = c->d_rec_slot.as<uint32_t>(); F.rec_e0 = c->d_rec_e0.as<phi_ent_t>(); F.rec_e1 = c->d_rec_e1.as<phi_ent_t>();
    F.walk_vtx = c->d_walk_vtx.as<int32_t>();
    F.rec_cls = c->d_rec_cls.as<int32_t>(); F.cls_mult = c->d_cls_mult.as<int32_t>();
    F.m_rec = c->d_m_rec.as<int32_t>();
    const uint64_t g_cap = pow2_at_least(std::max<uint64_t>(1024, 2 * (uint64_t)n_matched));
    PHICHK(phi_dev_ensure(c, c->d_g_keys, g_cap * 8));
    PHICHK(phi_dev_ensure(c, c->d_g_rep, g_cap * 4));
    PHICHK(phi_dev_ensure(c, c->d_g_cnt, g_cap * 4));
    PHICHK(phi_dev_ensure(c, c->d_m_group, (size_t)std::max<int64_t>(n_matched, 1) * 4));
    const size_t n_slot_ids = (size_t)std::max<int64_t>(c->n_unique, 1);
    PHICHK(phi_dev_ensure(c, c->d_slot_maxcnt, n_slot_ids * 4));
    PHICHK(phi_dev_ensure(c, c->d_slot_multi, n_slot_ids));
    F.g_keys = c->d_g_keys.as<uint64_t>(); F.g_rep = c->d_g_rep.as<int32_t>(); F.g_cnt = c->d_g_cnt.as<uint32_t>();
    F.g_mask = g_cap - 1;
    F.m_group = c->d_m_group.as<int32_t>();
    F.u_uid = c->d_u_uid.as<uint32_t>();
    F.slot_maxcnt = c->d_slot_maxcnt.as<uint32_t>(); F.slot_multi = c->d_slot_multi.as<uint8_t>();
    F.limit = c->threshold * (float)(uint32_t)c->n_walks;
    F.counters = (unsigned long long *)scalar(c, S_FILTERED);
    F.err = (uint32_t *)scalar(c, S_ERR);
    for (int attempt = 0;; attempt++) {
        F.seed = 0x243F6A8885A308D3ull + 0x9E3779B97F4A7C15ull * (uint64_t)attempt;
        phi_launch_fill_u64(c->stream, F.g_keys, (int64_t)g_cap, PHI_EMPTY_KEY);
        phi_launch_fill_u32(c->stream, (uint32_t *)F.g_rep, (int64_t)g_cap, 0xFFFFFFFFu);
        HIPCHK(hipMemsetAsync(F.g_cnt, 0, g_cap * 4, c->stream));
        phi_launch_group_insert(c->stream, F, n_matched);
        phi_launch_group_count(c->stream, F, n_matched);
        HIPCHK(hipStreamSynchronize(c->stream));
        uint32_t err = 0;
        HIPCHK(phi_copy_sync(c, &err, scalar(c, S_ERR), 4, hipMemcpyDeviceToHost));
        if (err & PHI_KERR_TABLE_FULL) return phi_fail(c, PHI_ERR_OVERFLOW, "anchor group table overflow");
        if (!(err & PHI_KERR_FP_COLLISION)) break;
        if (attempt == 7) return phi_fail(c, PHI_ERR_DEVICE, "anchor fingerprints collide under 8 seeds (internal error)");
        HIPCHK(phi_memset_sync(c, scalar(c, S_ERR), 0, 4));
    }
    HIPCHK(hipMemsetAsync(F.slot_maxcnt, 0, n_slot_ids * 4, c->stream));
    HIPCHK(hipMemsetAsync(F.slot_multi, 0, n_slot_ids, c->stream));
    HIPCHK(hipMemsetAsync(scalar(c, S_FILTERED), 0, 16, c->stream));
    phi_launch_group_max(c->stream, F, n_matched);
    phi_launch_slot_count(c->stream, F, c->n_unique);
    PHICHK(phi_dev_ensure(c, c->d_flags, (size_t)std::max<int64_t>(std::max(n_matched, n_rec), 1)));
    PHICHK(phi_dev_ensure(c, c->d_flags2, (size_t)std::max<int64_t>(n_matched, 1)));
    phi_launch_kept_flags(c->stream, F, n_matched, c->d_flags.as<uint8_t>(), c->d_flags2.as<uint8_t>());
    PHICHK(phi_compact(c, c->d_flags.as<uint8_t>(), n_matched, c->d_list, &S.n_kept_rec));
    S.tm.lap("filter kernels");
    return PHI_OK;
}

static int expand_kept_records(Solve &S)
{
    phi_ctx *c = S.c;
    const int64_t n_rec = c->n_rec, n_matched = S.n_matched, n_kept_rec = S.n_kept_rec;
    const int32_t nw = c->n_walks;
    const int64_t nr = std::max<int64_t>(n_rec, 1);
    PHICHK(phi_dev_ensure(c, c->d_flags2, (size_t)std::max<int64_t>(nr, n_matched)));
    HIPCHK(hipMemsetAsync(c->d_flags2.p, 0, (size_t)nr, c->stream));
    phi_launch_mark_list(c->stream, c->d_list.as<int32_t>(), c->d_m_rec.as<int32_t>(), n_kept_rec, c->d_flags2.as<uint8_t>());
    PHICHK(phi_dev_ensure(c, c->d_list3, (size_t)std::max<int64_t>(c->n_cls, (int64_t)nw) * 4));
    phi_launch_class_sel_count(c->stream, c->d_flags2.as<uint8_t>(), c->d_cls_rec_off.as<int32_t>(), c->n_cls, c->d_list3.as<int32_t>());
    PhiExpandArgs X{};
    X.ent_cls = c->d_ent_cls.as<int32_t>(); X.e_lo = 0; X.e_hi = c->n_entries;
    X.cls_rec_off = c->d_cls_rec_off.as<int32_t>(); X.cls_rep = c->d_cls_rep.as<phi_ent_t>();
    X.sel = c->d_flags2.as<uint8_t>(); X.sel_cnt = c->d_list3.as<int32_t>();
    X.rec_slot = c->d_rec_slot.as<uint32_t>(); X.u_uid = c->d_u_uid.as<uint32_t>();
    X.rec_e0 = c->d_rec_e0.as<phi_ent_t>(); X.rec_e1 = c->d_rec_e1.as<phi_ent_t>();
    const int64_t nb = phi_expand_num_blocks(c->n_entries);
    PHICHK(phi_dev_ensure(c, c->d_blk_cnt, (size_t)nb * 4));
    PHICHK(phi_dev_ensure(c, c->d_blk_off, (size_t)(nb + 1) * 8));
    X.block_cnt = c->d_blk_cnt.as<int32_t>(); X.block_off = c->d_blk_off.as<int64_t>();
    phi_launch_expand_count(c->stream, X);
    PHICHK(phi_scan(c, c->d_blk_cnt.as<int32_t>(), nb, c->d_blk_off.as<int64_t>()));
    int64_t n_kept = 0;
    HIPCHK(hipMemcpyAsync(&n_kept, c->d_blk_off.as<int64_t>() + nb, 8, hipMemcpyDeviceToHost, c->stream));
    HIPCHK(hipStreamSynchronize(c->stream));
    if (n_kept >= (int64_t)1 << 31) return phi_fail(c, PHI_ERR_UNSUPPORTED, "more than 2^31 anchors in the model");
    S.n_kept = n_kept;
    c->h_kept = PhiAnchorSpan{}; c->h_dp = PhiAnchorSpan{}; c->anchors_host = false;
    c->n_kept = n_kept; c->n_dp = 0;
    c->h_kept_hash.clear();
    PHICHK(phi_dev_ensure(c, c->d_anchors, (size_t)std::max<int64_t>(n_kept, 1) * 12));
    static_assert(sizeof(PhiAnchorHost) == 12, "PhiAnchorHost is the device triple");
    PHICHK(phi_dev_ensure(c, c->d_a_e1, (size_t)std::max<int64_t>(n_kept, 1) * 4));
    PHICHK(phi_dev_ensure(c, c->d_g_span, (size_t)std::max<int64_t>(n_kept, 1)));
    PHICHK(phi_dev_ensure(c, c->d_ctr, (size_t)(nw + 8) * 8));
    HIPCHK(hipMemsetAsync(c->d_ctr.p, 0, (size_t)(nw + 8) * 8, c->stream));
    if (n_kept && getenv("PHI_EXPAND_GENERIC")) {
        X.out_tri = c->d_anchors.as<uint32_t>();
        phi_launch_expand_write(c->stream, X, 1);
    } else if (n_kept) {
        PHICHK(phi_dev_ensure(c, c->d_sel_off, (size_t)(c->n_cls + 1) * 4));
        PHICHK(phi_dev_ensure(c, c->d_sel_tri, (size_t)std::max<int64_t>(n_kept_rec, 1) * 12));
        PHICHK(phi_scan(c, c->d_list3.as<int32_t>(), c->n_cls, c->d_sel_off.as<int32_t>()));
        phi_launch_class_sel_tri(c->stream, c->d_flags2.as<uint8_t>(), c->d_cls_rec_off.as<int32_t>(), c->n_cls, c->d_sel_off.as<int32_t>(), c->d_cls_rep.as<phi_ent_t>(),
                                 c->d_rec_slot.as<uint32_t>(), c->d_u_uid.as<uint32_t>(), c->d_rec_e0.as<phi_ent_t>(), c->d_rec_e1.as<phi_ent_t>(), c->d_sel_tri.as<int32_t>());
        unsigned long long *d_ctr = c->d_ctr.as<unsigned long long>();
        phi_launch_expand_tri(c->stream, c->d_ent_cls.as<int32_t>(), 0, c->n_entries, c->d_sel_off.as<int32_t>(), c->d_sel_tri.as<int32_t>(),
                              c->d_blk_off.as<int64_t>(), c->d_anchors.as<uint32_t>(), c->d_a_e1.as<phi_ent_t>(), c->d_g_span.as<uint8_t>(),
                              c->d_walk_off.as<int64_t>(), nw, d_ctr + 8, d_ctr, n_kept);
        S.anchors_prepped = true;
    }
    return PHI_OK;
}

static int check_anchors_choose_mode(Solve &S)
{
    phi_ctx *c = S.c;
    const int32_t nw = c->n_walks;
    const int64_t n_kept = S.n_kept;
    unsigned long long *d_ctr = c->d_ctr.as<unsigned long long>();
    if (!S.anchors_prepped)
        phi_launch_anchor_prep(c->stream, c->d_anchors.as<uint32_t>(), n_kept, c->d_walk_off.as<int64_t>(), nw, c->d_a_e1.as<phi_ent_t>(), c->d_g_span.as<uint8_t>(), d_ctr + 8, d_ctr);
    std::vector<unsigned long long> hc((size_t)nw + 8);
    HIPCHK(hipMemcpyAsync(hc.data(), d_ctr, hc.size() * 8, hipMemcpyDeviceToHost, c->stream));
    HIPCHK(hipStreamSynchronize(c->stream));
    if (hc[1] & 1) return phi_fail(c, PHI_ERR_DEVICE, "dp anchors not sorted by last entry (internal error)");
    if (hc[1] & 2)
        return phi_fail(c, c->k > PHI_RCAP ? PHI_ERR_UNSUPPORTED : PHI_ERR_DEVICE, "an anchor spans %d edges or more%s", PHI_RCAP,
                        c->k > PHI_RCAP ? ": with k > 32 the graph's vertices must be long enough for a k-mer to cover at most 32 of them" : " (internal error)");
    c->h_n_anchors.assign(nw, 0);
    for (int32_t h = 0; h < nw; h++) c->h_n_anchors[h] = (int64_t)hc[(size_t)h + 8];
    int64_t dev_min = (int64_t)1 << 16;
    if (const char *e = getenv("PHI_SOLVE_DEVICE")) dev_min = atoi(e) ? 0 : INT64_MAX;
    S.dev = hc[0] == 0 && n_kept >= dev_min && n_kept > 0;
    uint64_t sc[S_N];
    HIPCHK(phi_copy_sync(c, sc, c->d_scalars.p, sizeof sc, hipMemcpyDeviceToHost));
    S.filtered = (int64_t)sc[S_FILTERED]; S.in_model = (int64_t)sc[S_INMODEL];
    return PHI_OK;
}

// ... 487 lines not shown
```

### phi_amd/csrc/read_batches.hip

```cpp
#include <string.h>
#include "phi_ctx.h"
#include "phi_dev.h"

static unsigned long long *logged_stripes(phi_ctx *c) { return c->d_stripes.as<unsigned long long>(); }
static unsigned long long *emit_stripes(phi_ctx *c) { return c->d_stripes.as<unsigned long long>() + PHI_STRIPES * 8; }

int phi_flush_reset(phi_ctx *c) { return c && c->ipc ? phi_ipc_wait_pending(c) : PHI_OK; }

static void swap_read_bufs(phi_ctx *c)
{
    if (c->hit_n == PHI_HIT_RING) {
        const DevBuf old = c->d_hit;
        c->d_hit = c->alt.hit; c->alt.hit = c->hit_extra[0]; c->hit_extra[0] = c->hit_extra[1]; c->hit_extra[1] = old;
        c->hit_idx = (c->hit_idx + 1) % PHI_HIT_RING;
    } else {
        std::swap(c->d_hit, c->alt.hit);
    }
    std::swap(c->d_stripes, c->alt.stripes);
}

static int sum_stripes(phi_ctx *c, const void *d, int n_sets, uint64_t *out)
{
    std::vector<uint64_t> h((size_t)n_sets * PHI_STRIPES * 8);
    int rc = phi_hip_check(c, phi_copy_sync(c, h.data(), d, (size_t)n_sets * STRIPE_BYTES, hipMemcpyDeviceToHost), "D2H counters");
    if (rc) return rc;
    for (int s_ = 0; s_ < n_sets; s_++) {
        uint64_t a = 0;
        for (int i = 0; i < PHI_STRIPES; i++) a += h[((size_t)s_ * PHI_STRIPES + i) * 8];
        out[s_] = a;
    }
    return PHI_OK;
}

int phi_read_counts(phi_ctx *c, uint64_t *n_logged, uint64_t *n_emitted)
{
    int frc = phi_flush_reset(c);
    if (frc) return frc;
    if (hipStreamSynchronize(c->stream) != hipSuccess) return phi_fail(c, PHI_ERR_DEVICE, "stream synchronize failed");
    uint64_t v[2];
    int rc = sum_stripes(c, c->d_stripes.p, 2, v);
    if (rc) return rc;
    if (n_logged) *n_logged = v[0];
    if (n_emitted) *n_emitted = v[1];
    return PHI_OK;
}

static int sp_set_size(phi_ctx *c, uint64_t *n)
{
    auto &S = c->spset;
    *n = 0;
    if (S.sp_cap == 0 || S.sp_set_gen != S.sp_gen) return PHI_OK;
    return sum_stripes(c, S.d_sp_cnt.p, 1, n);
}

static int sp_clear(phi_ctx *c, uint64_t cap)
{
    auto &S = c->spset;
    if (cap != S.sp_cap || !S.d_sp_keys.p) {
        phi_dev_free(S.d_sp_keys);
        S.sp_cap = 0;
        PHICHK(phi_dev_ensure(c, S.d_sp_keys, cap * 8));
        S.sp_cap = cap;
    }
    PHICHK(phi_dev_ensure(c, S.d_sp_cnt, STRIPE_BYTES));
    phi_launch_fill_u64(c->stream, S.d_sp_keys.as<uint64_t>(), (int64_t)cap, PHI_EMPTY_KEY);
    HIPCHK(hipMemsetAsync(S.d_sp_cnt.p, 0, STRIPE_BYTES, c->stream));
    return PHI_OK;
}

static int sp_reserve(phi_ctx *c, uint64_t in_set, uint64_t more)
{
    auto &S = c->spset;
    const uint64_t need = phi_set_capacity(in_set, more);
    if (S.sp_set_gen != S.sp_gen) {
        PHICHK(sp_clear(c, phi_set_reusable(S.sp_cap, need) ? S.sp_cap : need));
        S.sp_set_gen = S.sp_gen;
        return PHI_OK;
    }
    if (need <= S.sp_cap) return PHI_OK;
    PHICHK(phi_dev_ensure(c, S.d_export, (size_t)std::max<uint64_t>(in_set, 1) * 8));
    HIPCHK(hipMemsetAsync(scalar(c, S_EXPORT), 0, 8, c->stream));
    phi_launch_spectrum_export(c->stream, S.d_sp_keys.as<uint64_t>(), (int64_t)S.sp_cap, S.d_export.as<uint64_t>(),
                               (unsigned long long *)scalar(c, S_EXPORT));
    HIPCHK(hipStreamSynchronize(c->stream));
    PHICHK(sp_clear(c, need));
    phi_launch_spectrum_insert(c->stream, S.d_export.as<uint64_t>(), (int64_t)in_set, S.d_sp_keys.as<uint64_t>(), S.sp_cap - 1,
                               S.d_sp_cnt.as<unsigned long long>(), nullptr, 0, nullptr, nullptr, (uint32_t *)scalar(c, S_ERR));
    return PHI_OK;
}

int phi_sp_flush(phi_ctx *c, uint64_t *n_in_set)
{
    auto &S = c->spset;
    auto &L = c->rlog;
    PHICHK(phi_sync_check(c));
    L.async_batches = false;
    uint64_t logged = 0, in_set = 0;
    PHICHK(phi_read_counts(c, &logged, nullptr));
    unsigned long long ov_now = 0;
    HIPCHK(phi_copy_sync(c, &ov_now, scalar(c, S_OVCNT + (int)(S.sp_gen % 3)), 8, hipMemcpyDeviceToHost));
    if ((int64_t)ov_now > L.ov_cap) ov_now = (unsigned long long)L.ov_cap;
    const bool pending = L.log_chunks > L.log_done || (int64_t)ov_now > L.ov_done;
    PHICHK(sp_set_size(c, &in_set));
    if (pending) {
        const uint64_t more = logged > (uint64_t)L.logged_done ? logged - (uint64_t)L.logged_done : 0;
        PHICHK(sp_reserve(c, in_set, more));
        if (L.log_chunks > L.log_done)
            phi_launch_spectrum_flush(c->stream, L.d_novlog.as<uint64_t>(), L.d_novcnt.as<uint16_t>(), L.log_done, L.log_chunks, L.nov_shift,
                                      S.d_sp_keys.as<uint64_t>(), S.sp_cap - 1, S.d_sp_cnt.as<unsigned long long>(), c->k, c->d_u_keys.as<uint64_t>(),
                                      c->u_cap - 1, (uint32_t *)scalar(c, S_ERR));
        if ((int64_t)ov_now > L.ov_done)
            phi_launch_spectrum_insert(c->stream, L.d_ovlist.as<uint64_t>() + L.ov_done, (int64_t)ov_now - L.ov_done, S.d_sp_keys.as<uint64_t>(),
                                       S.sp_cap - 1, S.d_sp_cnt.as<unsigned long long>(), nullptr, 0, nullptr, nullptr, (uint32_t *)scalar(c, S_ERR));
        HIPCHK(hipGetLastError());
        L.log_done = L.log_chunks; L.ov_done = (int64_t)ov_now; L.logged_done = (int64_t)logged;
        PHICHK(phi_sync_check(c));
        PHICHK(sp_set_size(c, &in_set));
    }
    if (n_in_set) *n_in_set = in_set;
    return PHI_OK;
}

int phi_spectrum_count(phi_ctx *c, uint64_t *n_distinct)
{
    uint64_t in_set = 0, flagged = 0;
    PHICHK(phi_sp_flush(c, &in_set));
    if (c->n_unique > 0) {
        HIPCHK(hipMemsetAsync(scalar(c, S_EXPORT), 0, 8, c->stream));
        phi_launch_count_flags(c->stream, c->d_hit.as<uint8_t>(), c->n_unique, (unsigned long long *)scalar(c, S_EXPORT));
        HIPCHK(hipMemcpyAsync(&flagged, scalar(c, S_EXPORT), 8, hipMemcpyDeviceToHost, c->stream));
        HIPCHK(hipStreamSynchronize(c->stream));
    }
    *n_distinct = in_set + flagged;
    return PHI_OK;
}

int phi_sync_check(phi_ctx *c)
{
    PHICHK(phi_flush_reset(c));
    HIPCHK(hipStreamSynchronize(c->stream));
    uint64_t s[S_N];
    HIPCHK(phi_copy_sync(c, s, c->d_scalars.p, sizeof s, hipMemcpyDeviceToHost));
    const uint32_t err = (uint32_t)s[S_ERR];
    if (err & PHI_KERR_TABLE_FULL) return phi_fail(c, PHI_ERR_OVERFLOW, "open-addressed table overflow (probe bound %d), or the overflow list of novel read hashes ran full under a batch handed over with phi_add_reads_device", PHI_MAX_PROBE);
    if (err & PHI_KERR_SENTINEL) return phi_fail(c, PHI_ERR_UNSUPPORTED, "a minimiser hashes to UINT64_MAX (table sentinel)");
    if (err & PHI_KERR_HASH_COLLISION) return phi_fail(c, PHI_ERR_UNSUPPORTED, "two different k-mers of the reads and walks share a MurmurHash3 value: the k-mer route cannot reproduce the reference's result for this read set (set PHI_SKETCH_KMER_KEYS=0 and run again)");
    return PHI_OK;
}

extern "C" {

int phi_add_reads_device(phi_ctx *c, const void *d_bases, const void *d_read_off, int64_t n_reads, int64_t n_bases)
{
    const int rc = phi_add_reads_device_impl(c, d_bases, d_read_off, n_reads, n_bases, false);
    if (c && rc == PHI_OK) c->rlog.async_batches = true;
    return rc;
}

}

int phi_add_reads_device_impl(phi_ctx *c, const void *d_bases, const void *d_read_off, int64_t n_reads, int64_t n_bases, bool replay)
{
    if (!c) return PHI_ERR_INVALID;
    if (!c->have_graph) return phi_fail(c, PHI_ERR_STATE, "phi_add_reads before phi_set_graph");
    if (n_reads < 0 || n_bases < 0 || (n_bases > 0 && !d_bases)) return phi_fail(c, PHI_ERR_INVALID, "phi_add_reads: bad arguments");
    if (__builtin_expect(c->ladder.collecting, 0)) return phi_ladder_collect(c, d_bases, d_read_off, n_reads, n_bases);
    auto &L = c->rlog;
    int64_t uniform_len = 0;
    if (!d_read_off && n_reads > 0 && n_bases > 0) {
        if (n_bases % n_reads) return phi_fail(c, PHI_ERR_INVALID, "phi_add_reads_device without offsets: %lld bases are not %lld reads of one length", (long long)n_bases, (long long)n_reads);
        const PhiOneLength one = phi_device_one_length(n_reads, n_bases);
        if (one.make_offsets) {
            PHICHK(phi_dev_ensure(c, L.d_roff_made, (size_t)(n_reads + 1) * 8));
            phi_launch_iota_i64(c->stream, L.d_roff_made.as<int64_t>(), n_reads + 1, one.step);
            d_read_off = L.d_roff_made.p;
        }
        uniform_len = one.uniform_len;
    }
    if (n_reads == 0 || n_bases == 0) { if (!replay) c->reads_count += n_reads; return PHI_OK; }
    HIPCHK(hipSetDevice(c->device));
    c->solved = false;
    const int64_t n_log_chunks = phi_sketch_read_chunks(c->k, c->w, uniform_len, n_reads, n_bases);
    {
        size_t budget = (size_t)1 << 30;
        if (const char *e = getenv("PHI_NOVLOG_BUDGET")) budget = (size_t)std::max<long long>(atoll(e), 1);
        const PhiLogPlan P = phi_log_plan(L.log_chunks, L.last_log_chunks, replay, n_log_chunks, L.nov_shift, L.d_novlog.cap, L.d_novcnt.cap, budget);
        L.log_chunks = P.base;
        if (P.flush_first) {
            PHICHK(phi_sp_flush(c, nullptr));
            L.flushed();
            HIPCHK(hipMemsetAsync(scalar(c, S_OVCNT + (int)(c->spset.sp_gen % 3)), 0, 8, c->stream));
        }
        if (P.log_bytes) {
            PHICHK(phi_dev_grow_keep(c, L.d_novlog, P.log_bytes, P.keep_log));
            PHICHK(phi_dev_grow_keep(c, L.d_novcnt, P.cnt_bytes, P.keep_cnt));
        }
        if (!replay) {
            L.ov_bound += phi_ov_batch_bound(n_bases, c->w);
            const char *e = getenv("PHI_OVLIST_CAP");
            if (e && !L.d_ovlist.p) {
                L.ov_cap = std::max<long long>(atoll(e), 1);
                PHICHK(phi_dev_ensure(c, L.d_ovlist, (size_t)L.ov_cap * 8));
            } else if (const int64_t cap = phi_ov_capacity(L.ov_bound, L.ov_cap); !e && cap != L.ov_cap) {
                PHICHK(phi_dev_grow_keep(c, L.d_ovlist, (size_t)cap * 8, (size_t)L.ov_cap * 8));
                L.ov_cap = cap;
            }
        }
    }
    PhiSketchArgs A{};
    A.ascii = (const uint8_t *)d_bases;
    A.read_off = (const int64_t *)d_read_off; A.n_reads = n_reads;
    A.uniform_len = (int32_t)uniform_len; A.inv_len = uniform_len ? 1.0 / (double)uniform_len : 0.0;
    A.inv_len_q32 = phi_inv_len_q32(uniform_len); A.reads_per_base_q32 = phi_reads_per_base_q32(n_reads, n_bases);
    A.allslow = c->k > PHI_MAX_K_PACKED;
    A.n_bases = n_bases; A.k = c->k; A.w = c->w;
    A.n_logged = replay ? nullptr : logged_stripes(c);
    A.n_emitted = replay ? nullptr : emit_stripes(c);
    A.u_rt = c->d_rt.as<uint64_t>(); A.u_bmask = c->rt_mask;
    A.hit = c->d_hit.as<uint8_t>();
    A.err = (uint32_t *)scalar(c, S_ERR);
    if (c->kt_mask) {
        const char *e = getenv("PHI_SKETCH_KMER_KEYS");
        const int mode = e ? atoi(e) : 1;
        if (mode >= 2 || (mode == 1 && n_log_chunks <= c->kt_max_chunks)) { A.k_rt = c->d_kt.as<uint64_t>(); A.k_bmask = c->kt_mask; }
    }
    A.nov_log = L.d_novlog.as<uint64_t>(); A.nov_cnt = L.d_novcnt.as<uint16_t>(); A.log_base = L.log_chunks; A.nov_shift = L.nov_shift;
    A.ov_list = L.d_ovlist.as<uint64_t>(); A.ov_cap = L.ov_cap;
    A.ov_count = (unsigned long long *)scalar(c, S_OVCNT + (int)(c->spset.sp_gen % 3));
    L.log_chunks += n_log_chunks; L.last_log_chunks = n_log_chunks;
    if (c->alt.needs_clean) {
        A.q_clean = 1;
        A.ov_zero = (unsigned long long *)scalar(c, S_OVCNT + (int)((c->spset.sp_gen + 1) % 3));
        A.q_hit_words = c->alt.hit.as<uint64_t>(); A.q_n_hit_words = c->n_unique / 8 + 1;
        A.q_stripes = c->alt.stripes.as<uint64_t>(); A.q_n_stripe_words = 2 * PHI_STRIPES * 8;
        c->alt.needs_clean = false;
        L.next_flag_zeroed = true;
    }
    phi_ipc_launch_args(c, A);
    hipEvent_t t0 = nullptr, t1 = nullptr;
    if (c->prof && c->prof_period > 0 && (c->prof_seq++ % c->prof_period) == 0) {
        if (c->prof_used == c->prof_events.size()) {
            hipEvent_t a, b;
            HIPCHK(hipEventCreate(&a));
            HIPCHK(hipEventCreate(&b));
            c->prof_events.emplace_back(a, b);
        }
        t0 = c->prof_events[c->prof_used].first; t1 = c->prof_events[c->prof_used].second;
        c->prof_used++;
        c->prof_bases += n_bases;
    }
    phi_launch_sketch(c->stream, PHI_MODE_PROBE, A, t0, t1);
    HIPCHK(hipGetLastError());
    if (!replay) { c->reads_bases += n_bases; c->reads_count += n_reads; }
    return PHI_OK;
}


int replay_if_full(phi_ctx *c, uint32_t err, const void *d_bases, const void *d_off, int64_t n_reads, int64_t n_bases)
{
    for (int attempt = 0; attempt < 8 && (err & PHI_KERR_TABLE_FULL); attempt++) {
        unsigned long long *cnt = (unsigned long long *)scalar(c, S_OVCNT + (int)(c->spset.sp_gen % 3));
        unsigned long long wanted = 0;
        HIPCHK(phi_copy_sync(c, &wanted, cnt, 8, hipMemcpyDeviceToHost));
        const PhiOvReplay R = phi_ov_replay(wanted, c->rlog.ov_cap);
        PHICHK(phi_dev_grow_keep(c, c->rlog.d_ovlist, (size_t)R.cap * 8, (size_t)R.valid * 8));
        c->rlog.ov_cap = R.cap;
        HIPCHK(phi_copy_sync(c, cnt, &R.valid, 8, hipMemcpyHostToDevice));
        err &= ~PHI_KERR_TABLE_FULL;
        HIPCHK(phi_copy_sync(c, scalar(c, S_ERR), &err, 4, hipMemcpyHostToDevice));
        PHICHK(phi_add_reads_device_impl(c, d_bases, d_off, n_reads, n_bases, true));
        HIPCHK(phi_copy_sync(c, &err, scalar(c, S_ERR), 4, hipMemcpyDeviceToHost));
    }
    return PHI_OK;
}

static int score_wait_replay(phi_ctx *c, const void *d_bases, const void *d_read_off, int64_t n_reads, int64_t n_bases, PhiStageTimer *tm)
{
    PHICHK(phi_add_reads_device_impl(c, d_bases, d_read_off, n_reads, n_bases, false));
    HIPCHK(hipMemcpyAsync(c->h_err, scalar(c, S_ERR), 4, hipMemcpyDeviceToHost, c->stream));
    HIPCHK(hipStreamSynchronize(c->stream));
    if (tm) tm->lap("H2D + sketch + probe");
    if (*c->h_err & PHI_KERR_TABLE_FULL) {
        PHICHK(replay_if_full(c, *c->h_err, d_bases, d_read_off, n_reads, n_bases));
        if (tm) tm->lap("overflow list grown, batch replayed");
    }
    return PHI_OK;
}

int phi_score_resident_batch(phi_ctx *c, const void *d_bases, const void *d_read_off, int64_t n_reads, int64_t n_bases)
{
    if (c->rlog.async_batches) { PHICHK(phi_sync_check(c)); c->rlog.async_batches = false; }
    if (!c->h_err) HIPCHK(hipHostMalloc((void **)&c->h_err, 64, hipHostMallocDefault));
    return score_wait_replay(c, d_bases, d_read_off, n_reads, n_bases, nullptr);
}

extern "C" {

int phi_add_reads(phi_ctx *c, const char *bases, const int64_t *read_off, int64_t n_reads)
{
    if (!c) return PHI_ERR_INVALID;
    if (!c->have_graph) return phi_fail(c, PHI_ERR_STATE, "phi_add_reads before phi_set_graph");
    if (n_reads < 0 || (n_reads > 0 && !read_off)) return phi_fail(c, PHI_ERR_INVALID, "phi_add_reads: bad arguments");
    if (n_reads == 0) return PHI_OK;
    if (read_off[0] != 0) return phi_fail(c, PHI_ERR_INVALID, "read_off must start at 0");
    const int64_t first_bad = phi_offsets_first_bad(read_off, n_reads, false, 0);
    if (first_bad >= 0) return phi_fail(c, PHI_ERR_INVALID, "read_off not monotone at read %lld", (long long)first_bad);
    const int64_t n_bases = read_off[n_reads];
    if (n_bases > 0 && !bases) return phi_fail(c, PHI_ERR_INVALID, "phi_add_reads: bases is null");
    const bool uniform = phi_reads_one_length(read_off, n_reads);
    HIPCHK(hipSetDevice(c->device));
    PhiStageTimer tm("add_reads");
    if (c->rlog.async_batches) { PHICHK(phi_sync_check(c)); c->rlog.async_batches = false; }
    PHICHK(phi_dev_ensure(c, c->d_roff, (size_t)(n_reads + 1) * 8));
    if (!c->h_err) HIPCHK(hipHostMalloc((void **)&c->h_err, 64, hipHostMallocDefault));
    tm.lap("buffers");
    PHICHK(phi_dev_ensure(c, c->d_rbases, (size_t)std::max<int64_t>(n_bases, 1)));
    if (!uniform) HIPCHK(hipMemcpyAsync(c->d_roff.p, read_off, (size_t)(n_reads + 1) * 8, hipMemcpyHostToDevice, c->stream));
    if (n_bases) HIPCHK(hipMemcpyAsync(c->d_rbases.p, bases, (size_t)n_bases, hipMemcpyHostToDevice, c->stream));
    return score_wait_replay(c, c->d_rbases.p, uniform ? nullptr : c->d_roff.p, n_reads, n_bases, &tm);
}

int phi_reset_reads(phi_ctx *c)
{
    if (!c) return PHI_ERR_INVALID;
    if (!c->have_graph) return phi_fail(c, PHI_ERR_STATE, "phi_reset_reads before phi_set_graph");
    HIPCHK(hipSetDevice(c->device));
    const bool front_dirty = c->alt.needs_clean;
    swap_read_bufs(c);
    c->alt.needs_clean = true;
    if (front_dirty) {
        PHICHK(phi_ipc_before_generation(c, c->spset.sp_gen + 1));
        phi_launch_reset_reads(c->stream, c->d_hit.as<uint64_t>(), c->d_hit.p ? c->n_unique / 8 + 1 : 0, c->d_stripes.as<uint64_t>(), 2 * PHI_STRIPES * 8);
        HIPCHK(hipGetLastError());
    }
    c->spset.new_generation();
    if (!c->rlog.next_flag_zeroed) HIPCHK(hipMemsetAsync(scalar(c, S_OVCNT + (int)(c->spset.sp_gen % 3)), 0, 8, c->stream));
    c->rlog.new_generation();
    c->reads_bases = 0; c->reads_count = 0; c->spectrum_override = -1;
    c->solved = false;
    c->ladder.scored = 0;
    return PHI_OK;
}

int phi_reads_stats(phi_ctx *c, int64_t *n_reads, int64_t *n_bases, int64_t *n_emitted, int64_t *n_distinct)
{
    if (!c) return PHI_ERR_INVALID;
    if (!c->have_graph) return phi_fail(c, PHI_ERR_STATE, "phi_reads_stats before phi_set_graph");
    HIPCHK(hipSetDevice(c->device));
    PHICHK(phi_sync_check(c));
    uint64_t nd = 0, ne = 0;
    PHICHK(phi_read_counts(c, nullptr, &ne));
    PHICHK(phi_spectrum_count(c, &nd));
    if (n_reads) *n_reads = c->reads_count;
    if (n_bases) *n_bases = c->reads_bases;
    if (n_emitted) *n_emitted = (int64_t)ne;
    if (n_distinct) *n_distinct = (int64_t)nd;
    return PHI_OK;
}

int phi_hits_buffer(phi_ctx *c, void **d_hits, int64_t *n)
{
    if (!c || !d_hits || !n) return PHI_ERR_INVALID;
    if (!c->have_graph) return phi_fail(c, PHI_ERR_STATE, "phi_hits_buffer before phi_set_graph");
    HIPCHK(hipSetDevice(c->device));
    PHICHK(phi_flush_reset(c));
    *d_hits = c->d_hit.p;
    *n = c->n_unique;
    return PHI_OK;
}

int phi_read_table(phi_ctx *c, void **d_table, int64_t *n_buckets)
{
    if (!c || !d_table || !n_buckets) return PHI_ERR_INVALID;
    if (!c->have_graph) return phi_fail(c, PHI_ERR_STATE, "phi_read_table before phi_set_graph");
    *d_table = c->d_rt.p;
    *n_buckets = (int64_t)c->rt_buckets;
    return PHI_OK;
}

int phi_spectrum_export(phi_ctx *c, void **d_hashes, int64_t *n)
{
    if (!c || !d_hashes || !n) return PHI_ERR_INVALID;
    if (!c->have_graph) return phi_fail(c, PHI_ERR_STATE, "phi_spectrum_export before phi_set_graph");
    HIPCHK(hipSetDevice(c->device));
    *d_hashes = nullptr; *n = 0;
    uint64_t cnt = 0;
    PHICHK(phi_sp_flush(c, &cnt));
    PHICHK(phi_dev_ensure(c, c->spset.d_export, (size_t)std::max<uint64_t>(cnt, 1) * 8));
    if (cnt) {
        HIPCHK(hipMemsetAsync(scalar(c, S_EXPORT), 0, 8, c->stream));
        phi_launch_spectrum_export(c->stream, c->spset.d_sp_keys.as<uint64_t>(), (int64_t)c->spset.sp_cap, c->spset.d_export.as<uint64_t>(),
                                   (unsigned long long *)scalar(c, S_EXPORT));
        HIPCHK(hipStreamSynchronize(c->stream));
    }
    *d_hashes = c->spset.d_export.p;
    *n = (int64_t)cnt;
    return PHI_OK;
}

int phi_spectrum_import(phi_ctx *c, const void *d_hashes, int64_t n)
{
    if (!c || n < 0 || (n > 0 && !d_hashes)) return PHI_ERR_INVALID;
    if (!c->have_graph) return phi_fail(c, PHI_ERR_STATE, "phi_spectrum_import before phi_set_graph");
    if (n == 0) return PHI_OK;
    HIPCHK(hipSetDevice(c->device));
    if (d_hashes == c->spset.d_export.p) return phi_fail(c, PHI_ERR_INVALID, "phi_spectrum_import: pass a copy, not the export buffer");
    uint64_t in_set = 0;
    PHICHK(phi_sp_flush(c, &in_set));
    PHICHK(sp_reserve(c, in_set, (uint64_t)n));
    phi_launch_spectrum_insert(c->stream, (const uint64_t *)d_hashes, n, c->spset.d_sp_keys.as<uint64_t>(), c->spset.sp_cap - 1,
                               c->spset.d_sp_cnt.as<unsigned long long>(), c->d_u_keys.as<uint64_t>(), c->u_cap - 1, c->d_u_uid.as<uint32_t>(),
                               c->d_hit.as<uint8_t>(), (uint32_t *)scalar(c, S_ERR));
    HIPCHK(hipGetLastError());
    c->solved = false;
    return PHI_OK;
}

int phi_spectrum_set_size(phi_ctx *c, int64_t global_size)
{
    if (!c || global_size < 0) return PHI_ERR_INVALID;
    c->spectrum_override = global_size;
    return PHI_OK;
}

}
```

### phi_amd/csrc/reads_host.h

```cpp
#pragma once
#include <stddef.h>
#include <string.h>
#include "phi_host_par.h"

static inline uint64_t pow2_at_least(uint64_t x) { uint64_t p = 1; while (p < x) p <<= 1; return p; }

struct PhiLogPlan {
    int64_t base;
    bool flush_first;
    size_t log_bytes, cnt_bytes;
    size_t keep_log, keep_cnt;
};
static inline PhiLogPlan phi_log_plan(int64_t log_chunks, int64_t last_log_chunks, bool replay, int64_t batch_chunks, int32_t nov_shift,
                                      size_t log_cap, size_t cnt_cap, size_t budget)
{
    PhiLogPlan P{};
    P.base = replay ? log_chunks - last_log_chunks : log_chunks;
    const size_t ent = (size_t)8 << nov_shift;
    size_t chunks = (size_t)P.base, need = (chunks + (size_t)batch_chunks) * ent;
    const auto full = [&]() { return need > log_cap || (chunks + (size_t)batch_chunks) * 2 > cnt_cap; };
    if (!full()) return P;
    if (chunks > 0 && need > budget) {
        P.flush_first = true;
        chunks = 0;
        need = (size_t)batch_chunks * ent;
    }
    if (full()) {
        const size_t want = std::max(need, std::min(2 * log_cap, budget));
        P.log_bytes = want; P.cnt_bytes = want / ent * 2 + 64;
        P.keep_log = chunks * ent; P.keep_cnt = chunks * 2;
    }
    return P;
}

static inline int64_t phi_ov_batch_bound(int64_t n_bases, int32_t w)
{
    return (int64_t)((double)n_bases * std::min(1.0, 3.0 / (w + 1))) + 16;
}
static inline int64_t phi_ov_capacity(int64_t bound, int64_t cap)
{
    return bound > cap ? std::max<int64_t>(std::max<int64_t>(bound, 2 * cap), 1 << 16) : cap;
}
struct PhiOvReplay { unsigned long long valid; int64_t cap; };
static inline PhiOvReplay phi_ov_replay(unsigned long long wanted, int64_t cap)
{
    PhiOvReplay R;
    R.valid = std::min<unsigned long long>(wanted, (unsigned long long)cap);
    R.cap = (int64_t)std::max<unsigned long long>(4ull * (unsigned long long)cap, 2 * wanted);
    return R;
}

static inline uint64_t phi_set_capacity(uint64_t in_set, uint64_t more)
{
    return pow2_at_least(std::max<uint64_t>(1u << 16, 2 * (in_set + more)));
}
static inline bool phi_set_reusable(uint64_t cap, uint64_t need) { return cap >= need && cap <= 4 * need; }

template <bool ONE> static inline int phi_offsets_span_bad(const int64_t *off, int64_t lo, int64_t hi, int64_t len)
{
    int bad = 0;
    for (int64_t r = lo; r < hi; r++) bad |= ONE ? (uint64_t)off[r + 1] - (uint64_t)off[r] != (uint64_t)len : off[r + 1] < off[r];
    return bad;
}
static inline int64_t phi_offsets_first_bad(const int64_t *off, int64_t n, bool one_length, int64_t len)
{
    const auto span = [=](int64_t lo, int64_t hi) { return one_length ? phi_offsets_span_bad<true>(off, lo, hi, len) : phi_offsets_span_bad<false>(off, lo, hi, len); };
    int64_t from = 0, to = n;
    if (n < (1 << 20)) {
        if (!span(0, n)) return -1;
    } else {
        std::atomic<int64_t> first{INT64_MAX};
        phi_parallel_chunks(n, (int64_t)1 << 20, [&](int64_t lo, int64_t hi, int) {
            if (!span(lo, hi)) return;
            int64_t seen = first.load();
            while (lo < seen && !first.compare_exchange_weak(seen, lo)) {}
        });
        if (first.load() == INT64_MAX) return -1;
        from = first.load(); to = std::min(n, from + ((int64_t)1 << 20));
    }
    for (int64_t r = from; r < to; r++)
        if (span(r, r + 1)) return r;
    return -1;
}
static inline bool phi_reads_one_length(const int64_t *off, int64_t n_reads)
{
    const int64_t n_bases = off[n_reads], len0 = off[1];
    int64_t all = 0;
    return n_bases > 0 && len0 >= 32 && !__builtin_mul_overflow(len0, n_reads, &all) && all == n_bases &&
           phi_offsets_first_bad(off, n_reads, true, len0) < 0;
}
struct PhiOneLength { int64_t uniform_len; bool make_offsets; int64_t step; };
static inline PhiOneLength phi_device_one_length(int64_t n_reads, int64_t n_bases)
{
    PhiOneLength L;
    L.step = n_bases / n_reads;
    L.make_offsets = L.step < 32 || L.step > 0x7FFFFFFF;
    L.uniform_len = L.make_offsets ? 0 : L.step;
    return L;
}

static inline uint32_t phi_inv_len_q32(int64_t uniform_len)
{
    return uniform_len ? (uint32_t)(((uint64_t)1 << 32) / (uint64_t)uniform_len) : 0u;
}
static inline uint32_t phi_reads_per_base_q32(int64_t n_reads, int64_t n_bases)
{
    const double q = (double)n_reads / (double)n_bases * 4294967296.0;
    return q >= 2147483648.0 ? 0x80000000u : (uint32_t)q;
}

static inline int phi_pool_best_fit(const size_t *cap, int n, size_t want)
{
    int best = -1;
    for (int i = 0; i < n; i++)
        if (cap[i] >= want && cap[i] <= want + want / 8 && (best < 0 || cap[i] < cap[best])) best = i;
    return best;
}

struct PhiTextSizes { uint32_t chunk, carry, line_cap; };
static inline PhiTextSizes phi_text_sizes(int64_t max_chunk_bytes, const char *carry_env)
{
    PhiTextSizes Z;
    Z.chunk = (uint32_t)std::min<int64_t>(std::max<int64_t>(max_chunk_bytes, 64), (int64_t)1 << 28);
    Z.carry = carry_env ? (uint32_t)std::max<long long>(64, atoll(carry_env)) & ~15u : std::max<uint32_t>(Z.chunk / 2, 1u << 24);
    Z.line_cap = (Z.carry + Z.chunk) / 16 + 1024;
    return Z;
}
static inline void phi_text_carry_update(std::vector<char> &carry, const char *p, uint32_t m, uint32_t tail)
{
    if (tail == 0) carry.clear();
    else if (tail <= m) carry.assign(p + m - tail, p + m);
    else {
        const size_t keep = tail - m;
        carry.erase(carry.begin(), carry.end() - (ptrdiff_t)keep);
        carry.insert(carry.end(), p, p + m);
    }
}
```

### phi_amd/csrc/table.hip

```cpp
#include <hip/hip_runtime.h>
#include "phi_dev.h"
#include "phi_kernels.h"
#include "phi_wave.h"

__global__ void phi_fill_u64_kernel(uint64_t *p, int64_t n, uint64_t v)
{
    for (int64_t i = (int64_t)blockIdx.x * blockDim.x + threadIdx.x; i < n; i += (int64_t)gridDim.x * blockDim.x)
        p[i] = v;
}
__global__ void phi_fill_u32_kernel(uint32_t *p, int64_t n, uint32_t v)
{
    for (int64_t i = (int64_t)blockIdx.x * blockDim.x + threadIdx.x; i < n; i += (int64_t)gridDim.x * blockDim.x)
        p[i] = v;
}

static inline unsigned grid_for(int64_t n, int tpb)
{
    int64_t nb = (n + tpb - 1) / tpb;
    if (nb > 256 * 16) nb = 256 * 16;
    if (nb < 1) nb = 1;
    return (unsigned)nb;
}

__global__ void __launch_bounds__(256) phi_read_table_clear_kernel(ulonglong2 *__restrict__ rt, int64_t n_slots)
// ... 182 lines not shown
    int n_new = 0;
    for (int64_t i = (int64_t)blockIdx.x * blockDim.x + threadIdx.x; i < n; i += (int64_t)gridDim.x * blockDim.x) {
        const uint64_t h = hashes[i];
        if (h == PHI_EMPTY_KEY) continue;
        if (u_keys) {
            bool found = false;
            uint64_t su = h & u_mask;
            for (int probes = 0; probes <= PHI_MAX_PROBE; probes++) {
                const uint64_t key = u_keys[su];
                if (key == h) { hit[u_uid[su]] = 1; found = true; break; }
                if (key == PHI_EMPTY_KEY) break;
                su = (su + 1) & u_mask;
            }
            if (found) continue;
        }
        uint64_t slot = h & sp_mask;
        int probes = 0;
        for (;;) {
            const unsigned long long prev = atomicCAS((unsigned long long *)&sp_keys[slot], PHI_EMPTY_KEY, h);
            if (prev == PHI_EMPTY_KEY) { n_new++; break; }
            if (prev == h) break;
            slot = (slot + 1) & sp_mask;
            if (++probes > PHI_MAX_PROBE) { atomicOr(err, PHI_KERR_TABLE_FULL); break; }
        }
    }
    n_new = phi_wave_sum(n_new);
    if ((threadIdx.x & 63) == 0 && n_new)
        atomicAdd(sp_count + (size_t)((blockIdx.x * 4 + (threadIdx.x >> 6)) & (PHI_STRIPES - 1)) * 8, (unsigned long long)n_new);
}

void phi_launch_spectrum_insert(hipStream_t st, const uint64_t *hashes, int64_t n, uint64_t *sp_keys,
                                uint64_t sp_mask, unsigned long long *sp_count, const uint64_t *u_keys, uint64_t u_mask,
                                const uint32_t *u_uid, uint8_t *hit, uint32_t *err)
{
    if (n > 0)
        hipLaunchKernelGGL(phi_spectrum_insert_kernel, dim3(grid_for(n, 256)), dim3(256), 0, st, hashes, n, sp_keys,
                           sp_mask, sp_count, u_keys, u_mask, u_uid, hit, err);
}

__global__ void __launch_bounds__(256) phi_spectrum_flush_kernel(const uint64_t *__restrict__ nov_log, const uint16_t *__restrict__ nov_cnt,
                                                                 int64_t c_lo, int64_t n_ent, int32_t shift,
                                                                 uint64_t *__restrict__ sp_keys, uint64_t sp_mask,
                                                                 unsigned long long *__restrict__ sp_count, int32_t k,
                                                                 const uint64_t *__restrict__ u_keys, uint64_t u_mask, uint32_t *__restrict__ err)
{
    int n_new = 0;
    const int lane = threadIdx.x & 63;
    for (int64_t t0 = (int64_t)blockIdx.x * blockDim.x + (threadIdx.x & ~63); t0 < n_ent; t0 += (int64_t)gridDim.x * blockDim.x) {
        const int64_t t = t0 + lane;
        bool have = false, kmers = false;
        int i = 0;
        int64_t c = 0;
        uint64_t h = 0, v = 0;
        if (t < n_ent) {
            c = c_lo + (t >> shift);
            i = (int)(t & ((1 << shift) - 1));
            const uint32_t cnt = nov_cnt[c];
            kmers = (cnt & PHI_NOV_KMERS) != 0;
            have = i < (int)(cnt & (PHI_NOV_KMERS - 1));
            if (have) {
                h = __builtin_nontemporal_load(&nov_log[(c << shift) + i]);
                if (kmers) { v = h; h = phi_kmer_hash(v, k); }
            }
        }
        uint64_t hp = __shfl_up(h, 1, 64), vp = __shfl_up(v, 1, 64);
        if (have && kmers) {
            if (lane == 0 && i > 0) { vp = nov_log[(c << shift) + i - 1]; hp = phi_kmer_hash(vp, k); }
            bool in_walks = false;
            if (h != PHI_EMPTY_KEY) {
                uint64_t su = h & u_mask;
                for (int probes = 0; probes <= PHI_MAX_PROBE; probes++) {
                    const uint64_t key = u_keys[su];
                    if (key == h) { in_walks = true; break; }
                    if (key == PHI_EMPTY_KEY) break;
                    su = (su + 1) & u_mask;
                }
            }
            const uint32_t e = phi_kmer_flush_rule(h, v, i > 0, hp, vp, in_walks);
            if (e) { atomicOr(err, e); have = false; }
        }
        if (!have) continue;
        uint64_t slot = h & sp_mask;
        int probes = 0;
        for (;;) {
            const unsigned long long prev = atomicCAS((unsigned long long *)&sp_keys[slot], PHI_EMPTY_KEY, h);
            if (prev == PHI_EMPTY_KEY) { n_new++; break; }
            if (prev == h) break;
            slot = (slot + 1) & sp_mask;
            if (++probes > PHI_MAX_PROBE) { atomicOr(err, PHI_KERR_TABLE_FULL); break; }
        }
    }
    n_new = phi_wave_sum(n_new);
    if ((threadIdx.x & 63) == 0 && n_new)
        atomicAdd(sp_count + (size_t)((blockIdx.x * 4 + (threadIdx.x >> 6)) & (PHI_STRIPES - 1)) * 8, (unsigned long long)n_new);
}

void phi_launch_spectrum_flush(hipStream_t st, const uint64_t *nov_log, const uint16_t *nov_cnt, int64_t c_lo, int64_t c_hi, int32_t shift,
                               uint64_t *sp_keys, uint64_t sp_mask, unsigned long long *sp_count, int32_t k, const uint64_t *u_keys,
                               uint64_t u_mask, uint32_t *err)
{
    const int64_t n_ent = (c_hi - c_lo) << shift;
    if (n_ent > 0)
        hipLaunchKernelGGL(phi_spectrum_flush_kernel, dim3(grid_for(n_ent, 256)), dim3(256), 0, st, nov_log, nov_cnt, c_lo, n_ent, shift,
                           sp_keys, sp_mask, sp_count, k, u_keys, u_mask, err);
}

__global__ void __launch_bounds__(256) phi_kmer_keys_kernel(const int32_t *__restrict__ rec_cls, const int32_t *__restrict__ rec_rel,
                                                            const uint64_t *__restrict__ rec_hash, const uint32_t *__restrict__ rec_slot,
                                                            int64_t n_rec, const int64_t *__restrict__ cls_base, const uint8_t *__restrict__ cls_left,
                                                            const uint64_t *__restrict__ words, const uint32_t *__restrict__ badbits, int32_t k,
                                                            uint64_t *__restrict__ kkeys, unsigned long long *__restrict__ ctr)
{
    for (int64_t i = (int64_t)blockIdx.x * blockDim.x + threadIdx.x; i < n_rec; i += (int64_t)gridDim.x * blockDim.x) {
        const int32_t c = rec_cls[i];
        const int64_t p = cls_base[c] + cls_left[c] + rec_rel[i];
        const int64_t wi = p >> 5;
        const int s = (int)(p & 31);
        const uint64_t bad = (((uint64_t)badbits[wi + 1] << 32) | badbits[wi]) >> s;
        if (bad & ((1ull << k) - 1)) { atomicAdd(&ctr[0], 1ull); continue; }
        const uint64_t f = phi_extract64(words, p) >> (64 - 2 * k), r = phi_revcomp(f, k);
        const uint64_t v = f < r ? f : r;
        if (phi_kmer_hash(v, k) != rec_hash[i]) { atomicAdd(&ctr[1], 1ull); continue; }
        const uint64_t key = phi_kmer_mix(v);
        unsigned long long *slot = (unsigned long long *)&kkeys[rec_slot[i]];
        unsigned long long prev = __builtin_nontemporal_load(slot);
        if (prev == PHI_EMPTY_KEY) prev = atomicCAS(slot, PHI_EMPTY_KEY, key);
        if (prev != PHI_EMPTY_KEY && prev != key) atomicAdd(&ctr[2], 1ull);
    }
}
void phi_launch_kmer_keys(hipStream_t st, const int32_t *rec_cls, const int32_t *rec_rel, const uint64_t *rec_hash, const uint32_t *rec_slot,
                          int64_t n_rec, const int64_t *cls_base, const uint8_t *cls_left, const uint64_t *words, const uint32_t *badbits,
                          int32_t k, uint64_t *kkeys, unsigned long long *ctr)
{
    if (n_rec > 0)
        hipLaunchKernelGGL(phi_kmer_keys_kernel, dim3(grid_for(n_rec, 256)), dim3(256), 0, st, rec_cls, rec_rel, rec_hash, rec_slot, n_rec,
                           cls_base, cls_left, words, badbits, k, kkeys, ctr);
}

__global__ void __launch_bounds__(256) phi_rt_overflowed_kernel(const uint64_t *__restrict__ rt, int64_t n_buckets,
                                                                unsigned long long *__restrict__ n_out)
{
    int cnt = 0;
    for (int64_t b = (int64_t)blockIdx.x * blockDim.x + threadIdx.x; b < n_buckets; b += (int64_t)gridDim.x * blockDim.x)
        cnt += (int)((rt[4 * b + 1] >> 32) & PHI_RT_OVERFLOWED);
    cnt = phi_wave_sum(cnt);
    if ((threadIdx.x & 63) == 0 && cnt) atomicAdd(n_out, (unsigned long long)cnt);
}
void phi_launch_rt_overflowed(hipStream_t st, const uint64_t *rt, int64_t n_buckets, unsigned long long *n_out)
{
    if (n_buckets > 0)
        hipLaunchKernelGGL(phi_rt_overflowed_kernel, dim3(grid_for(n_buckets, 256)), dim3(256), 0, st, rt, n_buckets, n_out);
}

__global__ void __launch_bounds__(256) phi_count_flags_kernel(const uint8_t *__restrict__ flags, int64_t n,
                                                              unsigned long long *__restrict__ n_out)
{
    int cnt = 0;
    for (int64_t i = (int64_t)blockIdx.x * blockDim.x + threadIdx.x; i < n; i += (int64_t)gridDim.x * blockDim.x)
        cnt += flags[i] != 0;
    cnt = phi_wave_sum(cnt);
    if ((threadIdx.x & 63) == 0 && cnt) atomicAdd(n_out, (unsigned long long)cnt);
}

void phi_launch_count_flags(hipStream_t st, const uint8_t *flags, int64_t n, unsigned long long *n_out)
{
    if (n > 0) hipLaunchKernelGGL(phi_count_flags_kernel, dim3(grid_for(n, 256)), dim3(256), 0, st, flags, n, n_out);
}

__global__ void __launch_bounds__(256) phi_spectrum_export_kernel(const uint64_t *__restrict__ sp_keys, int64_t cap,
                                                                  uint64_t *__restrict__ out,
                                                                  unsigned long long *__restrict__ n_out)
{
    for (int64_t i0 = (int64_t)blockIdx.x * blockDim.x; i0 < cap; i0 += (int64_t)gridDim.x * blockDim.x) {
        const int64_t i = i0 + threadIdx.x;
        const uint64_t key = i < cap ? sp_keys[i] : PHI_EMPTY_KEY;
        const bool occ = key != PHI_EMPTY_KEY;
        const unsigned long long bal = __ballot(occ);
        const int lane = threadIdx.x & 63;
        unsigned long long base = 0;
        if (lane == 0 && bal) base = atomicAdd(n_out, (unsigned long long)__popcll(bal));
        base = __shfl(base, 0, 64);
        if (occ) out[base + __popcll(bal & ((1ull << lane) - 1))] = key;
    }
}

void phi_launch_spectrum_export(hipStream_t st, const uint64_t *sp_keys, int64_t cap, uint64_t *out,
                                unsigned long long *n_out)
{
    if (cap > 0)
        hipLaunchKernelGGL(phi_spectrum_export_kernel, dim3(grid_for(cap, 256)), dim3(256), 0, st, sp_keys, cap, out,
                           n_out);
}

__global__ void phi_warm_table_kernel() {}
void phi_warm_table(hipStream_t st) { hipLaunchKernelGGL(phi_warm_table_kernel, dim3(1), dim3(64), 0, st); }
```

Measured before the change: 481.0.

## Collapse host round trips into one device totals block read per spectrum step

Adds a single-block totals kernel that reduces the scalar slots, stripe counters, spectrum counts and a nonzero-byte count into one 128-byte block, copied to pinned host memory in one transfer. Solve and stats then make one synchronised round trip instead of several separate copy-and-wait steps. Host error/totals buffers now come from a shared pinned slab, and a wait counter plus a planning helper with a selftest are added. The old path stays available behind the PHI_SPECTRUM_TRIPS=0 environment variable; the new path adds small extra kernel launches.

Result: slower. 466.7 (-3.0%).

```diff
diff --git a/include/phi_amd.h b/include/phi_amd.h
--- a/include/phi_amd.h
+++ b/include/phi_amd.h
@@ -220,6 +220,10 @@
 
 int phi_prefix_sums(phi_ctx *ctx, int32_t kind, const void *d_in, int64_t n, void *d_out);
 
+int phi_count_nonzero_bytes(phi_ctx *ctx, const void *d_bytes, int64_t n, int64_t *count);
+
+int phi_host_waits(phi_ctx *ctx, int64_t *n_waits);
+
 int phi_edit_distances(phi_ctx *ctx, const char *a, const int64_t *a_off, const char *b, const int64_t *b_off,
                        int64_t n_pairs, int64_t max_distance, int64_t *out);
 
diff --git a/phi_amd/_capi.py b/phi_amd/_capi.py
--- a/phi_amd/_capi.py
+++ b/phi_amd/_capi.py
@@ -31,7 +31,7 @@
     "phi_reads_collect_begin", "phi_reads_collect_end", "phi_reads_collect_release", "phi_ladder_plan", "phi_ladder_advance", "phi_ladder_band",
     "phi_set_graph_panel", "phi_panel_origin", "phi_panel_walks", "phi_panel_stats", "phi_panel_release",
     "phi_scout_graph", "phi_scout_scores", "phi_scout_choose", "phi_reads_collect_score", "phi_vcf_walks_wide",
-    "phi_prefix_sums",
+    "phi_prefix_sums", "phi_count_nonzero_bytes", "phi_host_waits",
     "phi_reads_bam_begin", "phi_add_reads_bam", "phi_add_reads_bam_parked", "phi_reads_bam_end", "phi_reads_bam_last_batch",
     "phi_calls_path", "phi_calls_walk", "phi_calls_stats",
 ]
@@ -234,6 +234,8 @@
     L.phi_prof_read.argtypes = [vp, C.POINTER(i64), C.POINTER(C.c_double), C.POINTER(i64)]
     L.phi_device_synchronize.argtypes = [vp]
     L.phi_prefix_sums.argtypes = [vp, i32, vp, i64, vp]
+    L.phi_count_nonzero_bytes.argtypes = [vp, vp, i64, C.POINTER(i64)]
+    L.phi_host_waits.argtypes = [vp, C.POINTER(i64)]
     L.phi_walk_text_upload.argtypes = [vp, vp, i32]
     L.phi_walk_text_resolve.argtypes = [vp, C.c_char_p, i32, vp, i64, i32, vp, C.POINTER(C.c_uint32)]
     L.phi_walk_entries.argtypes = [vp, vp, i64, C.POINTER(i64)]
diff --git a/phi_amd/context.py b/phi_amd/context.py
--- a/phi_amd/context.py
+++ b/phi_amd/context.py
@@ -663,6 +663,16 @@
     def prefix_sums(self, kind, d_in, n, d_out):
         self._chk(self._L.phi_prefix_sums(self._h, kind, C.c_void_p(d_in), n, C.c_void_p(d_out)))
 
+    def count_nonzero_bytes(self, d_bytes, n):
+        cnt = C.c_int64()
+        self._chk(self._L.phi_count_nonzero_bytes(self._h, C.c_void_p(d_bytes), n, C.byref(cnt)))
+        return cnt.value
+
+    def host_waits(self):
+        n = C.c_int64()
+        self._chk(self._L.phi_host_waits(self._h, C.byref(n)))
+        return n.value
+
     def prof_enable(self, on=True):
         self._chk(self._L.phi_prof_enable(self._h, int(on)))
 
diff --git a/phi_amd/csrc/host/spectrum_plan_selftest.cpp b/phi_amd/csrc/host/spectrum_plan_selftest.cpp
--- /dev/null
+++ b/phi_amd/csrc/host/spectrum_plan_selftest.cpp
@@ -0,0 +1,92 @@
+#include <stdio.h>
+#include <stdlib.h>
+#include <string.h>
+#include <vector>
+#include "../reads_host.h"
+
+namespace {
+
+typedef unsigned __int128 u128;
+
+uint64_t ref_need(uint64_t kept, uint64_t more)
+{
+    u128 want = 2 * ((u128)kept + more), p = 65536;
+    while (p < want) p *= 2;
+    return (uint64_t)p;
+}
+
+struct Pending { const char *name; int64_t log_chunks, log_done; uint64_t ov_now; int64_t ov_done, ov_cap; };
+const Pending PENDING[] = {
+    {"nothing_pending", 0, 0, 0, 0, 0},
+    {"nothing_pending_all_done", 10, 10, 5, 5, 100},
+    {"log_only", 10, 3, 5, 5, 100},
+    {"log_only_no_list", 7, 0, 0, 0, 0},
+    {"overflow_only", 10, 10, 50, 5, 100},
+    {"both", 12, 3, 50, 5, 100},
+    {"counter_past_the_list", 10, 10, 500, 5, 100},
+    {"counter_past_the_list_all_done", 10, 10, 500, 100, 100},
+    {"counter_below_done", 10, 10, 3, 5, 100},
+    {"log_below_done", 3, 10, 0, 0, 0},
+};
+
+bool check(const Pending &W, bool current, uint64_t in_set, uint64_t logged, int64_t logged_done, uint64_t sp_cap, std::vector<char> &why)
+{
+    const PhiSetPlan P = phi_set_plan(W.log_chunks, W.log_done, W.ov_now, W.ov_done, W.ov_cap, logged, logged_done, in_set, sp_cap, current);
+    const auto fail = [&](const char *m) { why.assign(m, m + strlen(m) + 1); return false; };
+    const int64_t ov_end = (int64_t)(W.ov_now < (uint64_t)W.ov_cap ? W.ov_now : (uint64_t)W.ov_cap);
+    const bool log_p = W.log_chunks > W.log_done, ov_p = ov_end > W.ov_done;
+    if (P.pending != (log_p || ov_p)) return fail("pending");
+    if (P.chunk_lo != W.log_done || P.chunk_hi < P.chunk_lo || P.ov_lo != W.ov_done || P.ov_hi < P.ov_lo) return fail("a range is reversed or starts elsewhere");
+    if ((P.chunk_hi > P.chunk_lo) != log_p || (log_p && P.chunk_hi != W.log_chunks)) return fail("chunk range");
+    if ((P.ov_hi > P.ov_lo) != ov_p || (ov_p && P.ov_hi != ov_end)) return fail("overflow range");
+    if (P.ov_hi > P.ov_lo && P.ov_hi > W.ov_cap) return fail("overflow range past the list");
+    if (!P.pending) {
+        if (P.room.clear || P.room.grow || P.room.cap != sp_cap) return fail("touched with nothing pending");
+        return true;
+    }
+    const uint64_t more = logged > (uint64_t)logged_done ? logged - (uint64_t)logged_done : 0;
+    if (P.more != more) return fail("more (underflow?)");
+    const bool mine = current && sp_cap > 0;
+    const uint64_t need = ref_need(mine ? in_set : 0, more);
+    if (need != phi_set_capacity(mine ? in_set : 0, more)) return fail("phi_set_capacity");
+    if (P.room.cap < need) return fail("capacity below need");
+    if (P.room.grow && !(mine && sp_cap < need && P.room.clear && P.room.cap == need)) return fail("grow");
+    if (mine) {
+        if (sp_cap >= need && (P.room.clear || P.room.cap != sp_cap)) return fail("a set with room was touched");
+        if (sp_cap < need && !P.room.grow) return fail("a set without room did not grow");
+    } else {
+        if (!P.room.clear || P.room.grow) return fail("another generation's set");
+        const bool reusable = sp_cap >= need && (u128)sp_cap <= 4 * (u128)need;
+        if (P.room.cap != (reusable ? sp_cap : need)) return fail("reuse");
+    }
+    return true;
+}
+
+}
+
+int main()
+{
+    const uint64_t IN_SET[] = {0, 1, 1000, 32768, 40000, 1u << 20, (uint64_t)3 << 31};
+    const int64_t LOGGED_DONE[] = {0, 500, 1000000};
+    const uint64_t LOGGED[] = {0, 100, 500, 70000, 3000000, (uint64_t)1 << 33};
+    int bad_total = 0;
+    for (const Pending &W : PENDING) {
+        long n = 0, bad = 0;
+        std::vector<char> why, first;
+        for (int current = 0; current < 2; current++)
+            for (uint64_t in_set : IN_SET)
+                for (int64_t logged_done : LOGGED_DONE)
+                    for (uint64_t logged : LOGGED) {
+                        const uint64_t more = logged > (uint64_t)logged_done ? logged - (uint64_t)logged_done : 0;
+                        const uint64_t need = ref_need(in_set, more), need0 = ref_need(0, more);
+                        const uint64_t CAPS[] = {0, need, 2 * need, 4 * need, 8 * need, need / 2, 65536, need0, 4 * need0, 8 * need0};
+                        for (uint64_t cap : CAPS) {
+                            n++;
+                            if (!check(W, current != 0, in_set, logged, logged_done, cap, why)) { if (!bad++) first = why; }
+                        }
+                    }
+        printf("%s %s plans=%ld bad=%ld%s%s\n", W.name, bad ? "FAILED" : "ok", n, bad, bad ? " first=" : "", bad ? first.data() : "");
+        bad_total += bad != 0;
+    }
+    return bad_total ? 1 : 0;
+}
diff --git a/phi_amd/csrc/phi_abi.hip b/phi_amd/csrc/phi_abi.hip
--- a/phi_amd/csrc/phi_abi.hip
+++ b/phi_amd/csrc/phi_abi.hip
@@ -63,6 +63,7 @@
         hipError_t e = hipSetDevice(device_id);
         if (e == hipSuccess) e = hipStreamCreateWithFlags(&c->aux_stream, hipStreamNonBlocking);
         if (e != hipSuccess) return e;
+        (void)phi_host_block(c);
         void *d = nullptr;
         std::vector<char> h((size_t)1 << 20, 0);
         if (hipMalloc(&d, h.size()) == hipSuccess) {
@@ -81,6 +82,7 @@
         if (aux.valid()) (void)aux.get();
         if (c->own_stream) (void)hipStreamDestroy(c->own_stream);
         if (c->aux_stream) (void)hipStreamDestroy(c->aux_stream);
+        phi_host_block_release(c);
         phi_dev_free(c->d_scalars); phi_dev_free(c->d_stripes); phi_dev_free(c->alt.stripes);
         delete c;
         return code;
@@ -88,7 +90,8 @@
     if (hipStreamCreateWithFlags(&c->own_stream, hipStreamNonBlocking) != hipSuccess) return bail(PHI_ERR_DEVICE);
     c->stream = c->own_stream;
     tm.lap("stream");
-    if (phi_dev_ensure(c, c->d_scalars, S_N * 8) || hipMemsetAsync(c->d_scalars.p, 0, S_N * 8, c->stream) != hipSuccess ||
+    if (const char *e = getenv("PHI_SPECTRUM_TRIPS")) c->sp_trips = atoi(e) != 0;
+    if (phi_dev_ensure(c, c->d_scalars, SCALARS_BYTES) || hipMemsetAsync(c->d_scalars.p, 0, SCALARS_BYTES, c->stream) != hipSuccess ||
         phi_dev_ensure(c, c->d_stripes, 2 * STRIPE_BYTES) || hipMemsetAsync(c->d_stripes.p, 0, 2 * STRIPE_BYTES, c->stream) != hipSuccess ||
         phi_dev_ensure(c, c->alt.stripes, 2 * STRIPE_BYTES) || hipMemsetAsync(c->alt.stripes.p, 0, 2 * STRIPE_BYTES, c->stream) != hipSuccess)
         return bail(PHI_ERR_DEVICE);
@@ -143,7 +146,7 @@
     struct Bypass { ~Bypass() { phi_pool_bypass(false); } } bypass_guard;
     for (DevBuf *b : all) phi_dev_free(*b);
     for (auto &pr : c->prof_events) { (void)hipEventDestroy(pr.first); (void)hipEventDestroy(pr.second); }
-    if (c->h_err) (void)hipHostFree(c->h_err);
+    phi_host_block_release(c);
     {
         auto &T = c->text;
         for (int i = 0; i < 2; i++) { phi_dev_free(T.text[i]); phi_dev_free(T.bases[i]); phi_dev_free(T.roff[i]); }
diff --git a/phi_amd/csrc/phi_ctx.h b/phi_amd/csrc/phi_ctx.h
--- a/phi_amd/csrc/phi_ctx.h
+++ b/phi_amd/csrc/phi_ctx.h
@@ -154,9 +154,10 @@
         int64_t ov_cap = 0, ov_done = 0, ov_bound = 0;
         bool async_batches = false;
         bool next_flag_zeroed = false;
+        bool maybe_pending = true;
         DevBuf d_roff_made;
         void flushed() { log_chunks = log_done = 0; ov_done = 0; ov_bound = 0; }
-        void new_generation() { flushed(); logged_done = 0; last_log_chunks = 0; next_flag_zeroed = false; }
+        void new_generation() { flushed(); logged_done = 0; last_log_chunks = 0; next_flag_zeroed = false; maybe_pending = true; }
     } rlog;
     int64_t reads_bases = 0, reads_count = 0;
     int64_t spectrum_override = -1;
@@ -169,6 +170,9 @@
     } alt;
 
     uint32_t *h_err = nullptr;
+    int h_err_slot = -1;
+    bool sp_trips = true;
+    int64_t n_waits = 0;
     struct PhiTextStream {
         bool active = false, irregular = false, started = false, detached = false;
         bool carry_stale = false;
@@ -295,15 +299,16 @@
     }
 };
 
+static inline hipError_t phi_stream_wait(phi_ctx *c) { c->n_waits++; return hipStreamSynchronize(c->stream); }
 static inline hipError_t phi_copy_sync(phi_ctx *c, void *dst, const void *src, size_t n, hipMemcpyKind kind)
 {
     const hipError_t e = hipMemcpyAsync(dst, src, n, kind, c->stream);
-    return e != hipSuccess ? e : hipStreamSynchronize(c->stream);
+    return e != hipSuccess ? e : phi_stream_wait(c);
 }
 static inline hipError_t phi_memset_sync(phi_ctx *c, void *dst, int v, size_t n)
 {
     const hipError_t e = hipMemsetAsync(dst, v, n, c->stream);
-    return e != hipSuccess ? e : hipStreamSynchronize(c->stream);
+    return e != hipSuccess ? e : phi_stream_wait(c);
 }
 
 static inline int32_t phi_entry_walk(const phi_ctx *c, int64_t e)
@@ -333,6 +338,13 @@
        S_OVCNT = 8 , S_N = 11 };
 static inline uint64_t *scalar(phi_ctx *c, int i) { return c->d_scalars.as<uint64_t>() + i; }
 #define STRIPE_BYTES ((size_t)PHI_STRIPES * 8 * 8)
+static_assert(S_N <= PHI_TOT_LOGGED && PHI_TOT_N * 8 == 128, "the block of totals holds every scalar in front of its sums");
+#define SCALARS_BYTES ((size_t)256 + STRIPE_BYTES)
+static inline uint64_t *totals_block(phi_ctx *c) { return c->d_scalars.as<uint64_t>() + 16; }
+static inline unsigned long long *byte_count_stripes(phi_ctx *c) { return c->d_scalars.as<unsigned long long>() + 32; }
+#define H_ERR_BYTES 192
+int phi_host_block(phi_ctx *c);
+void phi_host_block_release(phi_ctx *c);
 int phi_upload_bytes(phi_ctx *c, DevBuf &b, const void *src, size_t bytes, hipStream_t st);
 template <class T> static inline int upload(phi_ctx *c, DevBuf &b, const T *src, size_t n, hipStream_t st = nullptr)
 {
@@ -372,7 +384,6 @@
 int phi_ipc_wait_pending(phi_ctx *c);
 int phi_ipc_before_generation(phi_ctx *c, int64_t gen);
 void phi_ipc_launch_args(phi_ctx *c, PhiSketchArgs &A);
-int phi_read_counts(phi_ctx *c, uint64_t *n_logged, uint64_t *n_emitted);
 int phi_spectrum_count(phi_ctx *c, uint64_t *n_distinct);
 int phi_scan(phi_ctx *c, const uint8_t *cnt, int64_t n, int32_t *off);
 int phi_scan(phi_ctx *c, const int32_t *cnt, int64_t n, int32_t *off);
diff --git a/phi_amd/csrc/phi_kernels.h b/phi_amd/csrc/phi_kernels.h
--- a/phi_amd/csrc/phi_kernels.h
+++ b/phi_amd/csrc/phi_kernels.h
@@ -110,6 +110,10 @@
                           int32_t k, uint64_t *kkeys, unsigned long long *ctr);
 void phi_launch_rt_overflowed(hipStream_t st, const uint64_t *rt, int64_t n_buckets, unsigned long long *n_out);
 void phi_launch_count_flags(hipStream_t st, const uint8_t *flags, int64_t n, unsigned long long *n_out);
+void phi_launch_count_nonzero(hipStream_t st, const uint8_t *p, int64_t n, unsigned long long *stripes);
+enum { PHI_TOT_LOGGED = 11, PHI_TOT_EMITTED = 12, PHI_TOT_IN_SET = 13, PHI_TOT_FLAGGED = 14, PHI_TOT_OV = 15, PHI_TOT_N = 16 };
+void phi_launch_totals(hipStream_t st, const uint64_t *scalars, int n_scalars, int ov_slot, const unsigned long long *stripes,
+                       const unsigned long long *sp_cnt, unsigned long long *byte_cnt, uint64_t *out);
 void phi_launch_spectrum_export(hipStream_t st, const uint64_t *sp_keys, int64_t cap, uint64_t *out,
                                 unsigned long long *n_out);
 
diff --git a/phi_amd/csrc/phi_solve.hip b/phi_amd/csrc/phi_solve.hip
--- a/phi_amd/csrc/phi_solve.hip
+++ b/phi_amd/csrc/phi_solve.hip
@@ -495,10 +495,12 @@
 {
     phi_ctx *c = S.c;
     if (c->dp_alloc_future.valid()) PHICHK(c->dp_alloc_future.get());
-    PHICHK(phi_sync_check(c));
+    if (!c->sp_trips) {
+        PHICHK(phi_sync_check(c));
+        uint64_t sc[S_N];
+        HIPCHK(phi_copy_sync(c, sc, c->d_scalars.p, sizeof sc, hipMemcpyDeviceToHost));
+    }
     S.tm = PhiStageTimer("solve");
-    uint64_t sc[S_N];
-    HIPCHK(phi_copy_sync(c, sc, c->d_scalars.p, sizeof sc, hipMemcpyDeviceToHost));
     uint64_t n_distinct = 0;
     PHICHK(phi_spectrum_count(c, &n_distinct));
     S.tm.lap("read spectrum (set from the log)");
diff --git a/phi_amd/csrc/read_batches.hip b/phi_amd/csrc/read_batches.hip
--- a/phi_amd/csrc/read_batches.hip
+++ b/phi_amd/csrc/read_batches.hip
@@ -17,6 +17,145 @@
         std::swap(c->d_hit, c->alt.hit);
     }
     std::swap(c->d_stripes, c->alt.stripes);
+}
+
+namespace {
+constexpr int SLAB_SLOTS = 64;
+constexpr size_t SLOT_BYTES = 256;
+static_assert(H_ERR_BYTES <= SLOT_BYTES, "a slot holds the error word and the block of totals");
+std::mutex slab_mu;
+char *slab = nullptr;
+uint64_t slab_used = 0;
+}
+int phi_host_block(phi_ctx *c)
+{
+    if (c->h_err) return PHI_OK;
+    {
+        std::lock_guard<std::mutex> g(slab_mu);
+        if (!slab && hipHostMalloc((void **)&slab, SLAB_SLOTS * SLOT_BYTES, hipHostMallocPortable) != hipSuccess) slab = nullptr;
+        for (int i = 0; slab && i < SLAB_SLOTS; i++)
+            if (!((slab_used >> i) & 1)) {
+                slab_used |= 1ull << i;
+                c->h_err = (uint32_t *)(slab + (size_t)i * SLOT_BYTES); c->h_err_slot = i;
+                return PHI_OK;
+            }
+    }
+    HIPCHK(hipHostMalloc((void **)&c->h_err, H_ERR_BYTES, hipHostMallocDefault));
+    c->h_err_slot = -1;
+    return PHI_OK;
+}
+void phi_host_block_release(phi_ctx *c)
+{
+    if (!c->h_err) return;
+    if (c->h_err_slot < 0) (void)hipHostFree(c->h_err);
+    else { std::lock_guard<std::mutex> g(slab_mu); slab_used &= ~(1ull << c->h_err_slot); }
+    c->h_err = nullptr;
+}
+static const uint64_t *host_totals(phi_ctx *c) { return (const uint64_t *)(c->h_err + 16); }
+
+static int report_kernel_errors(phi_ctx *c, uint32_t err)
+{
+    if (err & PHI_KERR_TABLE_FULL) return phi_fail(c, PHI_ERR_OVERFLOW, "open-addressed table overflow (probe bound %d), or the overflow list of novel read hashes ran full under a batch handed over with phi_add_reads_device", PHI_MAX_PROBE);
+    if (err & PHI_KERR_SENTINEL) return phi_fail(c, PHI_ERR_UNSUPPORTED, "a minimiser hashes to UINT64_MAX (table sentinel)");
+    if (err & PHI_KERR_HASH_COLLISION) return phi_fail(c, PHI_ERR_UNSUPPORTED, "two different k-mers of the reads and walks share a MurmurHash3 value: the k-mer route cannot reproduce the reference's result for this read set (set PHI_SKETCH_KMER_KEYS=0 and run again)");
+    return PHI_OK;
+}
+
+static bool sp_set_current(const phi_ctx *c) { return c->spset.sp_cap > 0 && c->spset.sp_set_gen == c->spset.sp_gen && c->spset.d_sp_cnt.p; }
+
+static int totals_round_trip(phi_ctx *c, bool count_flags)
+{
+    PHICHK(phi_host_block(c));
+    if (count_flags) phi_launch_count_nonzero(c->stream, c->d_hit.as<uint8_t>(), c->n_unique, byte_count_stripes(c));
+    phi_launch_totals(c->stream, c->d_scalars.as<uint64_t>(), S_N, S_OVCNT + (int)(c->spset.sp_gen % 3), c->d_stripes.as<unsigned long long>(),
+                      sp_set_current(c) ? c->spset.d_sp_cnt.as<unsigned long long>() : nullptr, byte_count_stripes(c), totals_block(c));
+    HIPCHK(hipGetLastError());
+    HIPCHK(hipMemcpyAsync(c->h_err + 16, totals_block(c), PHI_TOT_N * 8, hipMemcpyDeviceToHost, c->stream));
+    HIPCHK(phi_stream_wait(c));
+    return report_kernel_errors(c, (uint32_t)host_totals(c)[S_ERR]);
+}
+
+static int sp_clear(phi_ctx *c, uint64_t cap)
+{
+    auto &S = c->spset;
+    if (cap != S.sp_cap || !S.d_sp_keys.p) {
+        phi_dev_free(S.d_sp_keys);
+        S.sp_cap = 0;
+        PHICHK(phi_dev_ensure(c, S.d_sp_keys, cap * 8));
+        S.sp_cap = cap;
+    }
+    PHICHK(phi_dev_ensure(c, S.d_sp_cnt, STRIPE_BYTES));
+    phi_launch_fill_u64(c->stream, S.d_sp_keys.as<uint64_t>(), (int64_t)cap, PHI_EMPTY_KEY);
+    HIPCHK(hipMemsetAsync(S.d_sp_cnt.p, 0, STRIPE_BYTES, c->stream));
+    return PHI_OK;
+}
+
+static int sp_make_room(phi_ctx *c, const PhiSetRoom &R, uint64_t in_set)
+{
+    auto &S = c->spset;
+    if (!R.clear) return PHI_OK;
+    if (!R.grow) {
+        PHICHK(sp_clear(c, R.cap));
+        S.sp_set_gen = S.sp_gen;
+        return PHI_OK;
+    }
+    PHICHK(phi_dev_ensure(c, S.d_export, (size_t)std::max<uint64_t>(in_set, 1) * 8));
+    HIPCHK(hipMemsetAsync(scalar(c, S_EXPORT), 0, 8, c->stream));
+    phi_launch_spectrum_export(c->stream, S.d_sp_keys.as<uint64_t>(), (int64_t)S.sp_cap, S.d_export.as<uint64_t>(),
+                               (unsigned long long *)scalar(c, S_EXPORT));
+    HIPCHK(phi_stream_wait(c));
+    PHICHK(sp_clear(c, R.cap));
+    phi_launch_spectrum_insert(c->stream, S.d_export.as<uint64_t>(), (int64_t)in_set, S.d_sp_keys.as<uint64_t>(), S.sp_cap - 1,
+                               S.d_sp_cnt.as<unsigned long long>(), nullptr, 0, nullptr, nullptr, (uint32_t *)scalar(c, S_ERR));
+    return PHI_OK;
+}
+static int sp_reserve(phi_ctx *c, uint64_t in_set, uint64_t more)
+{
+    return sp_make_room(c, phi_set_room(in_set, more, c->spset.sp_cap, sp_set_current(c)), in_set);
+}
+
+static int sp_issue(phi_ctx *c, const PhiSetPlan &P, uint64_t in_set, uint64_t logged)
+{
+    auto &S = c->spset;
+    auto &L = c->rlog;
+    PHICHK(sp_make_room(c, P.room, in_set));
+    if (P.chunk_hi > P.chunk_lo)
+        phi_launch_spectrum_flush(c->stream, L.d_novlog.as<uint64_t>(), L.d_novcnt.as<uint16_t>(), P.chunk_lo, P.chunk_hi, L.nov_shift,
+                                  S.d_sp_keys.as<uint64_t>(), S.sp_cap - 1, S.d_sp_cnt.as<unsigned long long>(), c->k, c->d_u_keys.as<uint64_t>(),
+                                  c->u_cap - 1, (uint32_t *)scalar(c, S_ERR));
+    if (P.ov_hi > P.ov_lo)
+        phi_launch_spectrum_insert(c->stream, L.d_ovlist.as<uint64_t>() + P.ov_lo, P.ov_hi - P.ov_lo, S.d_sp_keys.as<uint64_t>(),
+                                   S.sp_cap - 1, S.d_sp_cnt.as<unsigned long long>(), nullptr, 0, nullptr, nullptr, (uint32_t *)scalar(c, S_ERR));
+    HIPCHK(hipGetLastError());
+    L.log_done = P.chunk_hi; L.ov_done = P.ov_hi; L.logged_done = (int64_t)logged;
+    return PHI_OK;
+}
+
+struct PhiSpectrumNow { uint64_t in_set = 0, flagged = 0, emitted = 0; };
+static int sp_make_current(phi_ctx *c, bool want_flags, PhiSpectrumNow *now)
+{
+    auto &L = c->rlog;
+    PHICHK(phi_flush_reset(c));
+    L.async_batches = false;
+    want_flags = want_flags && c->n_unique > 0;
+    bool counted = false;
+    if (L.maybe_pending) {
+        PHICHK(totals_round_trip(c, want_flags));
+        const uint64_t *T = host_totals(c);
+        const uint64_t in_set = T[PHI_TOT_IN_SET], logged = T[PHI_TOT_LOGGED];
+        now->in_set = in_set; now->flagged = T[PHI_TOT_FLAGGED]; now->emitted = T[PHI_TOT_EMITTED];
+        counted = true;
+        const PhiSetPlan P = phi_set_plan(L.log_chunks, L.log_done, T[PHI_TOT_OV], L.ov_done, L.ov_cap, logged, L.logged_done, in_set,
+                                          c->spset.sp_cap, sp_set_current(c));
+        L.maybe_pending = false;
+        if (!P.pending) return PHI_OK;
+        PHICHK(sp_issue(c, P, in_set, logged));
+    }
+    PHICHK(totals_round_trip(c, want_flags && !counted));
+    const uint64_t *T = host_totals(c);
+    now->in_set = T[PHI_TOT_IN_SET]; now->emitted = T[PHI_TOT_EMITTED];
+    if (!counted) now->flagged = T[PHI_TOT_FLAGGED];
+    return PHI_OK;
 }
 
 static int sum_stripes(phi_ctx *c, const void *d, int n_sets, uint64_t *out)
@@ -32,11 +171,11 @@
     return PHI_OK;
 }
 
-int phi_read_counts(phi_ctx *c, uint64_t *n_logged, uint64_t *n_emitted)
+static int read_counts_trips0(phi_ctx *c, uint64_t *n_logged, uint64_t *n_emitted)
 {
     int frc = phi_flush_reset(c);
     if (frc) return frc;
-    if (hipStreamSynchronize(c->stream) != hipSuccess) return phi_fail(c, PHI_ERR_DEVICE, "stream synchronize failed");
+    if (phi_stream_wait(c) != hipSuccess) return phi_fail(c, PHI_ERR_DEVICE, "stream synchronize failed");
     uint64_t v[2];
     int rc = sum_stripes(c, c->d_stripes.p, 2, v);
     if (rc) return rc;
@@ -45,7 +184,7 @@
     return PHI_OK;
 }
 
-static int sp_set_size(phi_ctx *c, uint64_t *n)
+static int sp_set_size_trips0(phi_ctx *c, uint64_t *n)
 {
     auto &S = c->spset;
     *n = 0;
@@ -53,99 +192,72 @@
     return sum_stripes(c, S.d_sp_cnt.p, 1, n);
 }
 
-static int sp_clear(phi_ctx *c, uint64_t cap)
-{
-    auto &S = c->spset;
-    if (cap != S.sp_cap || !S.d_sp_keys.p) {
-        phi_dev_free(S.d_sp_keys);
-        S.sp_cap = 0;
-        PHICHK(phi_dev_ensure(c, S.d_sp_keys, cap * 8));
-        S.sp_cap = cap;
-    }
-    PHICHK(phi_dev_ensure(c, S.d_sp_cnt, STRIPE_BYTES));
-    phi_launch_fill_u64(c->stream, S.d_sp_keys.as<uint64_t>(), (int64_t)cap, PHI_EMPTY_KEY);
-    HIPCHK(hipMemsetAsync(S.d_sp_cnt.p, 0, STRIPE_BYTES, c->stream));
-    return PHI_OK;
-}
-
-static int sp_reserve(phi_ctx *c, uint64_t in_set, uint64_t more)
-{
-    auto &S = c->spset;
-    const uint64_t need = phi_set_capacity(in_set, more);
-    if (S.sp_set_gen != S.sp_gen) {
-        PHICHK(sp_clear(c, phi_set_reusable(S.sp_cap, need) ? S.sp_cap : need));
-        S.sp_set_gen = S.sp_gen;
-        return PHI_OK;
-    }
-    if (need <= S.sp_cap) return PHI_OK;
-    PHICHK(phi_dev_ensure(c, S.d_export, (size_t)std::max<uint64_t>(in_set, 1) * 8));
-    HIPCHK(hipMemsetAsync(scalar(c, S_EXPORT), 0, 8, c->stream));
-    phi_launch_spectrum_export(c->stream, S.d_sp_keys.as<uint64_t>(), (int64_t)S.sp_cap, S.d_export.as<uint64_t>(),
-                               (unsigned long long *)scalar(c, S_EXPORT));
-    HIPCHK(hipStreamSynchronize(c->stream));
-    PHICHK(sp_clear(c, need));
-    phi_launch_spectrum_insert(c->stream, S.d_export.as<uint64_t>(), (int64_t)in_set, S.d_sp_keys.as<uint64_t>(), S.sp_cap - 1,
-                               S.d_sp_cnt.as<unsigned long long>(), nullptr, 0, nullptr, nullptr, (uint32_t *)scalar(c, S_ERR));
-    return PHI_OK;
-}
-
-int phi_sp_flush(phi_ctx *c, uint64_t *n_in_set)
-{
-    auto &S = c->spset;
+static int sp_flush_trips0(phi_ctx *c, uint64_t *n_in_set)
+{
     auto &L = c->rlog;
     PHICHK(phi_sync_check(c));
     L.async_batches = false;
+    L.maybe_pending = false;
     uint64_t logged = 0, in_set = 0;
-    PHICHK(phi_read_counts(c, &logged, nullptr));
+    PHICHK(read_counts_trips0(c, &logged, nullptr));
     unsigned long long ov_now = 0;
-    HIPCHK(phi_copy_sync(c, &ov_now, scalar(c, S_OVCNT + (int)(S.sp_gen % 3)), 8, hipMemcpyDeviceToHost));
-    if ((int64_t)ov_now > L.ov_cap) ov_now = (unsigned long long)L.ov_cap;
-    const bool pending = L.log_chunks > L.log_done || (int64_t)ov_now > L.ov_done;
-    PHICHK(sp_set_size(c, &in_set));
-    if (pending) {
-        const uint64_t more = logged > (uint64_t)L.logged_done ? logged - (uint64_t)L.logged_done : 0;
-        PHICHK(sp_reserve(c, in_set, more));
-        if (L.log_chunks > L.log_done)
-            phi_launch_spectrum_flush(c->stream, L.d_novlog.as<uint64_t>(), L.d_novcnt.as<uint16_t>(), L.log_done, L.log_chunks, L.nov_shift,
-                                      S.d_sp_keys.as<uint64_t>(), S.sp_cap - 1, S.d_sp_cnt.as<unsigned long long>(), c->k, c->d_u_keys.as<uint64_t>(),
-                                      c->u_cap - 1, (uint32_t *)scalar(c, S_ERR));
-        if ((int64_t)ov_now > L.ov_done)
-            phi_launch_spectrum_insert(c->stream, L.d_ovlist.as<uint64_t>() + L.ov_done, (int64_t)ov_now - L.ov_done, S.d_sp_keys.as<uint64_t>(),
-                                       S.sp_cap - 1, S.d_sp_cnt.as<unsigned long long>(), nullptr, 0, nullptr, nullptr, (uint32_t *)scalar(c, S_ERR));
-        HIPCHK(hipGetLastError());
-        L.log_done = L.log_chunks; L.ov_done = (int64_t)ov_now; L.logged_done = (int64_t)logged;
+    HIPCHK(phi_copy_sync(c, &ov_now, scalar(c, S_OVCNT + (int)(c->spset.sp_gen % 3)), 8, hipMemcpyDeviceToHost));
+    PHICHK(sp_set_size_trips0(c, &in_set));
+    const PhiSetPlan P = phi_set_plan(L.log_chunks, L.log_done, ov_now, L.ov_done, L.ov_cap, logged, L.logged_done, in_set, c->spset.sp_cap, sp_set_current(c));
+    if (P.pending) {
+        PHICHK(sp_issue(c, P, in_set, logged));
         PHICHK(phi_sync_check(c));
-        PHICHK(sp_set_size(c, &in_set));
+        PHICHK(sp_set_size_trips0(c, &in_set));
     }
     if (n_in_set) *n_in_set = in_set;
     return PHI_OK;
 }
 
-int phi_spectrum_count(phi_ctx *c, uint64_t *n_distinct)
+static int spectrum_count_trips0(phi_ctx *c, uint64_t *n_distinct)
 {
     uint64_t in_set = 0, flagged = 0;
-    PHICHK(phi_sp_flush(c, &in_set));
+    PHICHK(sp_flush_trips0(c, &in_set));
     if (c->n_unique > 0) {
         HIPCHK(hipMemsetAsync(scalar(c, S_EXPORT), 0, 8, c->stream));
         phi_launch_count_flags(c->stream, c->d_hit.as<uint8_t>(), c->n_unique, (unsigned long long *)scalar(c, S_EXPORT));
         HIPCHK(hipMemcpyAsync(&flagged, scalar(c, S_EXPORT), 8, hipMemcpyDeviceToHost, c->stream));
-        HIPCHK(hipStreamSynchronize(c->stream));
+        HIPCHK(phi_stream_wait(c));
     }
     *n_distinct = in_set + flagged;
     return PHI_OK;
 }
 
+int phi_sp_flush(phi_ctx *c, uint64_t *n_in_set)
+{
+    if (!c->sp_trips) return sp_flush_trips0(c, n_in_set);
+    PhiSpectrumNow now;
+    PHICHK(sp_make_current(c, false, &now));
+    if (n_in_set) *n_in_set = now.in_set;
+    return PHI_OK;
+}
+
+int phi_spectrum_count(phi_ctx *c, uint64_t *n_distinct)
+{
+    if (!c->sp_trips) return spectrum_count_trips0(c, n_distinct);
+    PhiSpectrumNow now;
+    PHICHK(sp_make_current(c, true, &now));
+    *n_distinct = now.in_set + now.flagged;
+    return PHI_OK;
+}
+
 int phi_sync_check(phi_ctx *c)
 {
     PHICHK(phi_flush_reset(c));
-    HIPCHK(hipStreamSynchronize(c->stream));
-    uint64_t s[S_N];
-    HIPCHK(phi_copy_sync(c, s, c->d_scalars.p, sizeof s, hipMemcpyDeviceToHost));
-    const uint32_t err = (uint32_t)s[S_ERR];
-    if (err & PHI_KERR_TABLE_FULL) return phi_fail(c, PHI_ERR_OVERFLOW, "open-addressed table overflow (probe bound %d), or the overflow list of novel read hashes ran full under a batch handed over with phi_add_reads_device", PHI_MAX_PROBE);
-    if (err & PHI_KERR_SENTINEL) return phi_fail(c, PHI_ERR_UNSUPPORTED, "a minimiser hashes to UINT64_MAX (table sentinel)");
-    if (err & PHI_KERR_HASH_COLLISION) return phi_fail(c, PHI_ERR_UNSUPPORTED, "two different k-mers of the reads and walks share a MurmurHash3 value: the k-mer route cannot reproduce the reference's result for this read set (set PHI_SKETCH_KMER_KEYS=0 and run again)");
-    return PHI_OK;
+    if (!c->sp_trips) {
+        HIPCHK(phi_stream_wait(c));
+        uint64_t s[S_N];
+        HIPCHK(phi_copy_sync(c, s, c->d_scalars.p, sizeof s, hipMemcpyDeviceToHost));
+        return report_kernel_errors(c, (uint32_t)s[S_ERR]);
+    }
+    PHICHK(phi_host_block(c));
+    HIPCHK(hipMemcpyAsync(c->h_err + 16, scalar(c, S_ERR), 8, hipMemcpyDeviceToHost, c->stream));
+    HIPCHK(phi_stream_wait(c));
+    return report_kernel_errors(c, (uint32_t)host_totals(c)[S_ERR]);
 }
 
 extern "C" {
@@ -249,6 +361,7 @@
         c->prof_used++;
         c->prof_bases += n_bases;
     }
+    L.maybe_pending = true;
     phi_launch_sketch(c->stream, PHI_MODE_PROBE, A, t0, t1);
     HIPCHK(hipGetLastError());
     if (!replay) { c->reads_bases += n_bases; c->reads_count += n_reads; }
@@ -278,7 +391,7 @@
 {
     PHICHK(phi_add_reads_device_impl(c, d_bases, d_read_off, n_reads, n_bases, false));
     HIPCHK(hipMemcpyAsync(c->h_err, scalar(c, S_ERR), 4, hipMemcpyDeviceToHost, c->stream));
-    HIPCHK(hipStreamSynchronize(c->stream));
+    HIPCHK(phi_stream_wait(c));
     if (tm) tm->lap("H2D + sketch + probe");
     if (*c->h_err & PHI_KERR_TABLE_FULL) {
         PHICHK(replay_if_full(c, *c->h_err, d_bases, d_read_off, n_reads, n_bases));
@@ -290,7 +403,7 @@
 int phi_score_resident_batch(phi_ctx *c, const void *d_bases, const void *d_read_off, int64_t n_reads, int64_t n_bases)
 {
     if (c->rlog.async_batches) { PHICHK(phi_sync_check(c)); c->rlog.async_batches = false; }
-    if (!c->h_err) HIPCHK(hipHostMalloc((void **)&c->h_err, 64, hipHostMallocDefault));
+    PHICHK(phi_host_block(c));
     return score_wait_replay(c, d_bases, d_read_off, n_reads, n_bases, nullptr);
 }
 
@@ -312,7 +425,7 @@
     PhiStageTimer tm("add_reads");
     if (c->rlog.async_batches) { PHICHK(phi_sync_check(c)); c->rlog.async_batches = false; }
     PHICHK(phi_dev_ensure(c, c->d_roff, (size_t)(n_reads + 1) * 8));
-    if (!c->h_err) HIPCHK(hipHostMalloc((void **)&c->h_err, 64, hipHostMallocDefault));
+    PHICHK(phi_host_block(c));
     tm.lap("buffers");
     PHICHK(phi_dev_ensure(c, c->d_rbases, (size_t)std::max<int64_t>(n_bases, 1)));
     if (!uniform) HIPCHK(hipMemcpyAsync(c->d_roff.p, read_off, (size_t)(n_reads + 1) * 8, hipMemcpyHostToDevice, c->stream));
@@ -347,10 +460,16 @@
     if (!c) return PHI_ERR_INVALID;
     if (!c->have_graph) return phi_fail(c, PHI_ERR_STATE, "phi_reads_stats before phi_set_graph");
     HIPCHK(hipSetDevice(c->device));
-    PHICHK(phi_sync_check(c));
     uint64_t nd = 0, ne = 0;
-    PHICHK(phi_read_counts(c, nullptr, &ne));
-    PHICHK(phi_spectrum_count(c, &nd));
+    if (!c->sp_trips) {
+        PHICHK(phi_sync_check(c));
+        PHICHK(read_counts_trips0(c, nullptr, &ne));
+        PHICHK(spectrum_count_trips0(c, &nd));
+    } else {
+        PhiSpectrumNow now;
+        PHICHK(sp_make_current(c, true, &now));
+        ne = now.emitted; nd = now.in_set + now.flagged;
+    }
     if (n_reads) *n_reads = c->reads_count;
     if (n_bases) *n_bases = c->reads_bases;
     if (n_emitted) *n_emitted = (int64_t)ne;
@@ -391,7 +510,7 @@
         HIPCHK(hipMemsetAsync(scalar(c, S_EXPORT), 0, 8, c->stream));
         phi_launch_spectrum_export(c->stream, c->spset.d_sp_keys.as<uint64_t>(), (int64_t)c->spset.sp_cap, c->spset.d_export.as<uint64_t>(),
                                    (unsigned long long *)scalar(c, S_EXPORT));
-        HIPCHK(hipStreamSynchronize(c->stream));
+        HIPCHK(phi_stream_wait(c));
     }
     *d_hashes = c->spset.d_export.p;
     *n = (int64_t)cnt;
@@ -416,6 +535,28 @@
     return PHI_OK;
 }
 
+int phi_count_nonzero_bytes(phi_ctx *c, const void *d_bytes, int64_t n, int64_t *count)
+{
+    if (!c) return PHI_ERR_INVALID;
+    if (n < 0 || !count || (n > 0 && !d_bytes)) return phi_fail(c, PHI_ERR_INVALID, "phi_count_nonzero_bytes: bad argument");
+    HIPCHK(hipSetDevice(c->device));
+    PHICHK(phi_host_block(c));
+    phi_launch_count_nonzero(c->stream, static_cast<const uint8_t *>(d_bytes), n, byte_count_stripes(c));
+    phi_launch_totals(c->stream, c->d_scalars.as<uint64_t>(), S_N, S_OVCNT, c->d_stripes.as<unsigned long long>(), nullptr, byte_count_stripes(c), totals_block(c));
+    HIPCHK(hipGetLastError());
+    HIPCHK(hipMemcpyAsync(c->h_err + 16, totals_block(c), PHI_TOT_N * 8, hipMemcpyDeviceToHost, c->stream));
+    HIPCHK(phi_stream_wait(c));
+    *count = (int64_t)host_totals(c)[PHI_TOT_FLAGGED];
+    return PHI_OK;
+}
+
+int phi_host_waits(phi_ctx *c, int64_t *n_waits)
+{
+    if (!c || !n_waits) return PHI_ERR_INVALID;
+    *n_waits = c->n_waits;
+    return PHI_OK;
+}
+
 int phi_spectrum_set_size(phi_ctx *c, int64_t global_size)
 {
     if (!c || global_size < 0) return PHI_ERR_INVALID;
diff --git a/phi_amd/csrc/reads_host.h b/phi_amd/csrc/reads_host.h
--- a/phi_amd/csrc/reads_host.h
+++ b/phi_amd/csrc/reads_host.h
@@ -55,6 +55,41 @@
     return pow2_at_least(std::max<uint64_t>(1u << 16, 2 * (in_set + more)));
 }
 static inline bool phi_set_reusable(uint64_t cap, uint64_t need) { return cap >= need && cap <= 4 * need; }
+struct PhiSetRoom {
+    bool clear;
+    bool grow;
+    uint64_t cap;
+};
+static inline PhiSetRoom phi_set_room(uint64_t in_set, uint64_t more, uint64_t sp_cap, bool current)
+{
+    PhiSetRoom R{false, false, sp_cap};
+    current = current && sp_cap > 0;
+    const uint64_t need = phi_set_capacity(current ? in_set : 0, more);
+    if (!current) { R.clear = true; R.cap = phi_set_reusable(sp_cap, need) ? sp_cap : need; }
+    else if (need > sp_cap) { R.clear = R.grow = true; R.cap = need; }
+    return R;
+}
+struct PhiSetPlan {
+    bool pending;
+    PhiSetRoom room;
+    int64_t chunk_lo, chunk_hi;
+    int64_t ov_lo, ov_hi;
+    uint64_t more;
+};
+static inline PhiSetPlan phi_set_plan(int64_t log_chunks, int64_t log_done, uint64_t ov_now, int64_t ov_done, int64_t ov_cap, uint64_t logged,
+                                      int64_t logged_done, uint64_t in_set, uint64_t sp_cap, bool current)
+{
+    PhiSetPlan P{};
+    P.room = PhiSetRoom{false, false, sp_cap};
+    const int64_t ov = (int64_t)std::min<uint64_t>(ov_now, (uint64_t)std::max<int64_t>(ov_cap, 0));
+    P.chunk_lo = log_done; P.chunk_hi = std::max(log_chunks, log_done);
+    P.ov_lo = ov_done; P.ov_hi = std::max(ov, ov_done);
+    P.pending = P.chunk_hi > P.chunk_lo || P.ov_hi > P.ov_lo;
+    if (!P.pending) return P;
+    P.more = logged_done >= 0 && logged > (uint64_t)logged_done ? logged - (uint64_t)logged_done : 0;
+    P.room = phi_set_room(in_set, P.more, sp_cap, current);
+    return P;
+}
 
 template <bool ONE> static inline int phi_offsets_span_bad(const int64_t *off, int64_t lo, int64_t hi, int64_t len)
 {
diff --git a/phi_amd/csrc/table.hip b/phi_amd/csrc/table.hip
--- a/phi_amd/csrc/table.hip
+++ b/phi_amd/csrc/table.hip
@@ -358,6 +358,75 @@
         hipLaunchKernelGGL(phi_rt_overflowed_kernel, dim3(grid_for(n_buckets, 256)), dim3(256), 0, st, rt, n_buckets, n_out);
 }
 
+__device__ __forceinline__ int phi_nonzero_bytes(uint32_t x)
+{
+    return __popc((((x & 0x7F7F7F7Fu) + 0x7F7F7F7Fu) | x) & 0x80808080u);
+}
+__global__ void __launch_bounds__(256) phi_count_nonzero_kernel(const uint8_t *__restrict__ p, int64_t n, int64_t head, int64_t n_vec,
+                                                                unsigned long long *__restrict__ stripes)
+{
+    __shared__ int s_w[4];
+    int cnt = 0;
+    const uint4 *__restrict__ body = reinterpret_cast<const uint4 *>(p + head);
+    for (int64_t i = (int64_t)blockIdx.x * blockDim.x + threadIdx.x; i < n_vec; i += (int64_t)gridDim.x * blockDim.x) {
+        const uint4 v = body[i];
+        cnt += phi_nonzero_bytes(v.x) + phi_nonzero_bytes(v.y) + phi_nonzero_bytes(v.z) + phi_nonzero_bytes(v.w);
+    }
+    if (blockIdx.x == 0) {
+        const int64_t t = threadIdx.x, tail0 = head + 16 * n_vec;
+        if (t < head) cnt += p[t] != 0;
+        else if (t >= 64 && tail0 + (t - 64) < n) cnt += p[tail0 + (t - 64)] != 0;
+    }
+    cnt = phi_wave_sum(cnt);
+    if ((threadIdx.x & 63) == 0) s_w[threadIdx.x >> 6] = cnt;
+    __syncthreads();
+    if (threadIdx.x == 0) {
+        const int total = s_w[0] + s_w[1] + s_w[2] + s_w[3];
+        if (total) atomicAdd(stripes + (size_t)(blockIdx.x & (PHI_STRIPES - 1)) * 8, (unsigned long long)total);
+    }
+}
+void phi_launch_count_nonzero(hipStream_t st, const uint8_t *p, int64_t n, unsigned long long *stripes)
+{
+    if (n <= 0) return;
+    const int64_t head = std::min<int64_t>(n, (int64_t)((16 - ((uintptr_t)p & 15)) & 15)), n_vec = (n - head) / 16;
+    hipLaunchKernelGGL(phi_count_nonzero_kernel, dim3(grid_for(n_vec, 256)), dim3(256), 0, st, p, n, head, n_vec, stripes);
+}
+
+__global__ void __launch_bounds__(PHI_STRIPES) phi_totals_kernel(const uint64_t *__restrict__ scalars, int n_scalars, int ov_slot,
+                                                                 const unsigned long long *__restrict__ stripes,
+                                                                 const unsigned long long *__restrict__ sp_cnt,
+                                                                 unsigned long long *__restrict__ byte_cnt, uint64_t *__restrict__ out)
+{
+    __shared__ unsigned long long s_w[4][PHI_STRIPES / 64];
+    const size_t at = (size_t)threadIdx.x * 8;
+    unsigned long long v[4];
+    v[0] = stripes[at];
+    v[1] = stripes[(size_t)PHI_STRIPES * 8 + at];
+    v[2] = sp_cnt ? sp_cnt[at] : 0ull;
+    v[3] = byte_cnt[at];
+    if (v[3]) byte_cnt[at] = 0ull;
+#pragma unroll
+    for (int j = 0; j < 4; j++) {
+        v[j] = phi_wave_sum(v[j]);
+        if ((threadIdx.x & 63) == 0) s_w[j][threadIdx.x >> 6] = v[j];
+    }
+    __syncthreads();
+    if ((int)threadIdx.x < n_scalars) out[threadIdx.x] = scalars[threadIdx.x];
+    if (threadIdx.x >= 64 && threadIdx.x < 68) {
+        const int j = threadIdx.x - 64;
+        unsigned long long t = 0;
+#pragma unroll
+        for (int i = 0; i < PHI_STRIPES / 64; i++) t += s_w[j][i];
+        out[PHI_TOT_LOGGED + j] = t;
+    }
+    if (threadIdx.x == 68) out[PHI_TOT_OV] = scalars[ov_slot];
+}
+void phi_launch_totals(hipStream_t st, const uint64_t *scalars, int n_scalars, int ov_slot, const unsigned long long *stripes,
+                       const unsigned long long *sp_cnt, unsigned long long *byte_cnt, uint64_t *out)
+{
+    hipLaunchKernelGGL(phi_totals_kernel, dim3(1), dim3(PHI_STRIPES), 0, st, scalars, n_scalars, ov_slot, stripes, sp_cnt, byte_cnt, out);
+}
+
 __global__ void __launch_bounds__(256) phi_count_flags_kernel(const uint8_t *__restrict__ flags, int64_t n,
                                                               unsigned long long *__restrict__ n_out)
 {
```
